# jiangzhongshi/SurfaceNetworks

Hardware: AMD Instinct MI355X
Metric: meshes/sec fwd+bwd, Dirac temporal-predict (higher is better)
Workload: dtype f32; 1 GPU; as_rigid_as_possible Dirac temporal prediction: 64 grid-cloth meshes 71x71 (V=5041,F=9800) per GPU, C=128, 15 layers, fwd+loss+bwd+allreduce+Adam; meshes_per_gpu=64, global_batch=64, parallelism=dp1 (mesh sharding, flat-bucket RCCL all-reduce), world_size=1, rccl_ranks=1, collective_backend=nccl, devices_visible=1, operator_format=q3, operators=pool, grad_bucket_bytes=4075488

## Files before the change

### include/sn_spmm.h

```cpp
#ifndef SN_SPMM_H_
#define SN_SPMM_H_

#include <stddef.h>
#include <stdint.h>

#ifdef __cplusplus
extern "C" {
#endif

#define SN_ABI_VERSION 1

#define SN_OK            0
#define SN_E_NULL       -1
#define SN_E_SHAPE      -2
#define SN_E_RANGE      -3
#define SN_E_LD         -4
#define SN_E_ALIGN      -5
#define SN_E_WORKSPACE  -6
#define SN_E_UNSUPPORTED -7

int         sn_abi_version(void);
const char *sn_status_string(int status);

int sn_spmm_csr_f32(const int32_t *rowptr, const int32_t *colind, const float *vals,
// ... 122 lines not shown
                                   void *stream);

int sn_validate_csr_i32(const int32_t *rowptr, const int32_t *colind, const float *vals, int64_t M, int64_t K, int64_t nnz,
                        int32_t *flags, void *stream);

int sn_elu_into_f32(const float *src, int64_t lds, float *dst, int64_t ldd,
                    int64_t rows, int32_t C, void *stream);
int sn_elu_bwd_acc_f32(const float *gdst, int64_t ldg, const float *gdst2, int64_t ldg2, const float *gadd, int64_t ldga,
                       const float *out, int64_t ldo, float *gsrc, int64_t ldgs, int64_t rows, int32_t C,
                       int32_t accumulate, void *stream);


size_t sn_colstats_workspace_bytes(int64_t rows, int32_t C);
int sn_colstats_f32(const float *x, int64_t ld, int64_t rows, int32_t C, double *out,
                    void *workspace, size_t workspace_bytes, void *stream);
int sn_colstats_into_f32(const float *x, int64_t ld, int64_t rows, int32_t C, double *out, int64_t out_ld, int64_t out_off,
                         void *workspace, size_t workspace_bytes, void *stream);
int sn_colstats_merge_f64(const double *part, int32_t nblk, int32_t C, double *out, int64_t out_ld, int64_t out_off,
                          void *stream);
int sn_colstats_merge2_f64(const double *part_lo, int32_t nblk_lo, int32_t C_lo, int32_t ld_lo, const double *part_hi,
                           int32_t nblk_hi, int32_t C_hi, int32_t ld_hi, double *out, void *stream);
int32_t sn_linear_fwd_stats_blocks(int64_t rows);
size_t sn_wgrad_workspace_bytes(int64_t rows, int32_t J, int32_t C);
int sn_wgrad_f32(const float *dy, int64_t lddy, const float *x, int64_t ldx, const float *center, int64_t rows,
                 int32_t J, int32_t C, float *G, double *dysum, void *workspace, size_t workspace_bytes, void *stream);
size_t sn_wgrad_seg_workspace_bytes(int64_t rows, int64_t rows_per_seg, int32_t J, int32_t C);
int sn_wgrad_seg_f32(const float *dy, int64_t lddy, const float *x, int64_t ldx, const float *center, int64_t rows,
                     int64_t rows_per_seg, int32_t J, int32_t C, float *G, double *dysum, float *seg_dysum, void *workspace,
                     size_t workspace_bytes, void *stream);
int sn_wgrad_slabs_f32(const float *dy, int64_t lddy, const float *x, int64_t ldx, const float *center, int64_t rows,
                       const int64_t *slab_off, int32_t nslab, const int64_t *seg_slab_ptr, int32_t nseg, int32_t J, int32_t C,
                       float *G, double *dysum, float *seg_dysum, void *workspace, size_t workspace_bytes, void *stream);
int sn_wgrad_bounded_f32(const float *dy, int64_t lddy, const float *x, int64_t ldx, const float *center, int64_t rows,
                         int32_t J, int32_t C, float *G, double *dysum, void *workspace, size_t workspace_bytes,
                         const float *dybound, int64_t n_dybound, const float *xinvstd, int64_t stat_rows, void *stream);
int sn_wgrad_seg_bounded_f32(const float *dy, int64_t lddy, const float *x, int64_t ldx, const float *center, int64_t rows,
                             int64_t rows_per_seg, int32_t J, int32_t C, float *G, double *dysum, float *seg_dysum,
                             void *workspace, size_t workspace_bytes, const float *dybound, int64_t n_dybound,
                             const float *xinvstd, int64_t stat_rows, void *stream);
int sn_wgrad_slabs_bounded_f32(const float *dy, int64_t lddy, const float *x, int64_t ldx, const float *center, int64_t rows,
                               const int64_t *slab_off, int32_t nslab, const int64_t *seg_slab_ptr, int32_t nseg, int32_t J,
                               int32_t C, float *G, double *dysum, float *seg_dysum, void *workspace, size_t workspace_bytes,
                               const float *dybound, int64_t n_dybound, const float *xinvstd, int64_t stat_rows, void *stream);
size_t sn_wgrad_thin_workspace_bytes(int64_t rows, int32_t J, int32_t C);
int sn_wgrad_thin_f32(const float *dy, int64_t lddy, const float *x, int64_t ldx, int64_t rows, int32_t J, int32_t C,
                      float *G, float *db, void *workspace, size_t workspace_bytes, void *stream);
size_t sn_masked_smooth_l1_workspace_bytes(int64_t rows, int32_t C);
int sn_masked_smooth_l1_fwd_f32(const float *out, int64_t ldo, const float *target, int64_t ldt, const float *rowmask,
                                int64_t rows, int32_t C, double scale, float *loss, void *workspace, size_t workspace_bytes,
                                void *stream);
int sn_masked_smooth_l1_bwd_f32(const float *out, int64_t ldo, const float *target, int64_t ldt, const float *rowmask,
                                int64_t rows, int32_t C, double scale, const float *gloss, float *gout, int64_t ldg,
                                void *stream);
int sn_gather_segments_f32(const float *src, const int64_t *base, int64_t nitems, int64_t rows_per_item, int64_t row_stride,
                           int32_t len, float *out, void *stream);
int sn_gather_segments_ragged_f32(const float *src, const int64_t *base, const int64_t *item_off, int64_t nitems,
                                  int64_t total_rows, int64_t row_stride, int32_t len, float *out, void *stream);
int sn_pair_argmin_f32(const float *GA, int64_t ldA, int64_t colsA, const int64_t *pa, const float *GB, int64_t ldB,
                       const int64_t *pb, int64_t NA, int64_t NB, int64_t *out, void *stream);
int sn_pair_ce_fwd_f32(const float *S, int64_t ld, const int64_t *target, int64_t NA, int64_t NB, float *lse, float *rowloss,
                       void *stream);
int sn_pair_ce_bwd_f32(const float *S, int64_t ld, const int64_t *target, const float *lse, const float *gloss, int64_t NA,
                       int64_t NB, int64_t rows, int64_t cols, float *dS, int64_t ldd, void *stream);
size_t sn_pair_fused_workspace_bytes(int64_t rowsA, int64_t rowsB);
int sn_pair_fused_fwd_f32(const float *FA, int64_t lda, const float *FB, int64_t ldb, const int64_t *target, int64_t NA,
                          int64_t NB, int64_t rowsA, int64_t rowsB, int32_t K, float *lse, float *rowloss, void *workspace,
                          size_t workspace_bytes, void *stream);
int sn_pair_fused_bwd_f32(const int64_t *target, const float *lse, const float *gloss, int64_t NA, int64_t NB, int64_t rowsA,
                          int64_t rowsB, int32_t K, float *dFA, int64_t ldda, float *dFB, int64_t lddb, void *workspace,
                          size_t workspace_bytes, void *stream);
size_t sn_pair_loss_workspace_bytes(int64_t rowsA, int64_t rowsB);
int sn_pair_soft_fwd_f32(const float *FA, int64_t lda, const float *FB, int64_t ldb, const int64_t *mapA, const int64_t *mapB,
                         const float *const *geo, int64_t ldgA, int64_t ldgB, int64_t NA, int64_t NB, int64_t rowsA, int64_t rowsB,
                         int32_t K, float *stats, float *rowloss, void *workspace, size_t workspace_bytes, void *stream);
int sn_pair_soft_bwd_f32(const int64_t *mapA, const int64_t *mapB, const float *const *geo, int64_t ldgA, int64_t ldgB,
                         const float *stats, const float *gloss, int64_t NA, int64_t NB, int64_t rowsA, int64_t rowsB, int32_t K,
                         float *dFA, int64_t ldda, float *dFB, int64_t lddb, void *workspace, size_t workspace_bytes, void *stream);
int sn_pair_sl1_fwd_f32(const float *FA, int64_t lda, const float *FB, int64_t ldb, const int64_t *mapA, const int64_t *mapB,
                        const float *const *geo, int64_t ldgA, int64_t ldgB, int64_t NA, int64_t NB, int64_t rowsA, int64_t rowsB,
                        int32_t K, double *rowloss, void *workspace, size_t workspace_bytes, void *stream);
int sn_pair_sl1_bwd_f32(const int64_t *mapA, const int64_t *mapB, const float *const *geo, int64_t ldgA, int64_t ldgB,
                        const float *gloss, int64_t NA, int64_t NB, int64_t rowsA, int64_t rowsB, int32_t K, float *dFA, int64_t ldda,
                        float *dFB, int64_t lddb, void *workspace, size_t workspace_bytes, void *stream);
size_t sn_pair_match_workspace_bytes(int64_t rowsA, int64_t rowsB);
int sn_pair_match_f32(const float *FA, int64_t lda, const float *FB, int64_t ldb, int64_t NA, int64_t NB, int64_t rowsA,
                      int64_t rowsB, int32_t K, int64_t *colA, float *bestA, int64_t *rowB, float *bestB, const float *geoB,
                      int64_t ldgB, const int64_t *truthA, float *errA, void *workspace, size_t workspace_bytes, void *stream);
int sn_linear_thin_fwd_f32(const float *x, int64_t ldx, const float *W, int64_t ldw, const float *bias, int64_t rows,
                           int32_t C, int32_t J, float *y, int64_t ldy, float *y_elu, int64_t lde, void *stream);
int sn_affine_cols_acc_f32(float *dx, int64_t lddx, const float *x, int64_t ldx, const float *center, const float *B,
                           const float *Cc, int64_t rows, int32_t C, void *stream);
int sn_affine_cols_elu_bwd_f32(float *dx, int64_t lddx, const float *x, int64_t ldx, const float *center, const float *B,
                               const float *Cc, int64_t rows, int32_t C, void *stream);

int sn_bn_fold_f32(const double *stats, int64_t rows, const float *gamma, const float *beta, const float *W,
                   const float *b, int32_t J, int32_t C, double eps, double momentum, int32_t training,
                   float *running_mean, float *running_var, float *mean, float *invstd, float *s, float *t,
                   float *Wf, float *bf, int64_t *num_batches_tracked, void *stream);
int32_t sn_wgrad_bounded_enabled(void);
int32_t sn_gemm_variant(void);
int32_t sn_colstats_blocks(int64_t rows);
int sn_colstats_partial_f32(const float *x, int64_t ld, int64_t rows, int32_t C, double *partial, void *stream);
int sn_bn_bwd_coeffs_f32(const float *Gc, const double *dystats, const float *W, const float *s, const float *invstd,
                         const float *beta, int64_t rows, int32_t J, int32_t C, float *dW, float *db, float *dgamma,
                         float *dbeta, float *Bc, float *Cc, void *stream);

// ... 135 lines not shown
int sn_mesh_cot_laplacian_f32(const float *V, const int32_t *F, int64_t nV, int64_t nF, int32_t phase, int32_t mass, int32_t clamp,
                              double hack, int32_t *rowptr, int32_t *colind, float *vals, int32_t *status, void *workspace,
                              size_t workspace_bytes, void *stream);

#define SN_SPGEMM_MAX_WINDOW   131072
#define SN_SPGEMM_BAD_COLUMN   1
#define SN_SPGEMM_TOO_WIDE     2
#define SN_SPGEMM_TOO_LARGE    4
#define SN_CSR_NO_OFFDIAGONAL  8
int64_t sn_csr_spgemm_max_window(void);
size_t sn_csr_spgemm_workspace_bytes(int64_t M);
int sn_csr_spgemm_f32(const int32_t *a_rowptr, const int32_t *a_colind, const float *a_vals, const int32_t *b_rowptr,
                      const int32_t *b_colind, const float *b_vals, int64_t M, int64_t K, int64_t N, int32_t phase,
                      int32_t *s_rowptr, int32_t *s_colind, float *s_vals, int32_t *rowptr, int32_t *colind, float *vals,
                      int32_t *status, void *workspace, size_t workspace_bytes, void *stream);
int sn_csr_inv_sqrt_degree_f32(const int32_t *rowptr, int64_t M, float *d, int32_t *status, void *stream);
int sn_csr_scale_sym_f32(const int32_t *a_rowptr, const int32_t *a_colind, const float *a_vals, const float *d, int64_t M,
                         int32_t phase, float *s_vals, int32_t *rowptr, int32_t *colind, float *vals, int32_t *status,
                         void *workspace, size_t workspace_bytes, void *stream);

int64_t sn_linear_small_rows(void);
int32_t sn_linear_fwd_form(int64_t rows, int32_t K, int32_t J, int32_t has_residual, int32_t has_y, int32_t has_elu,
                           int32_t has_tile_sums);
int sn_linear_fwd_f32(const float *x, int64_t ldx, const float *W, int64_t ldw, const float *bias,
                      const float *residual, int64_t ldr, float *y, int64_t ldy, float *y_elu, int64_t lde,
                      int64_t rows, int32_t K, int32_t J, double *elu_stats_part ,
                      void *stream);
int sn_linear_dgrad_f32(const float *dy, int64_t lddy, const float *W, int64_t ldw, const float *x, int64_t ldx,
                        const float *center, const float *B, const float *Cc, float *dx, int64_t lddx,
                        int64_t rows, int32_t J, int32_t C, void *stream);
int sn_linear_dgrad_elu_f32(const float *dy, int64_t lddy, const float *W, int64_t ldw, const float *x, int64_t ldx,
                            const float *center, const float *B, const float *Cc, float *dx_hi, int64_t lddx,
                            float *gact, int64_t ldga, const float *gadd, int64_t ldgadd,
                            int64_t rows, int32_t J, int32_t C, void *stream);
int32_t sn_linear_dgrad_absmax_blocks(void);
int sn_linear_dgrad_elu_absmax_f32(const float *dy, int64_t lddy, const float *W, int64_t ldw, const float *x, int64_t ldx,
                                   const float *center, const float *B, const float *Cc, float *dx_hi, int64_t lddx,
                                   float *gact, int64_t ldga, const float *gadd, int64_t ldgadd,
                                   int64_t rows, int32_t J, int32_t C, float *gact_absmax, void *stream);
int sn_linear_dgrad_elu_rawlow_f32(const float *dy, int64_t lddy, const float *W, int64_t ldw, const float *x, int64_t ldx,
                                   const float *center, const float *B, const float *Cc, float *dx_hi, int64_t lddx,
                                   float *graw, int64_t ldgr, int64_t rows, int32_t J, int32_t C, void *stream);
int sn_linear_fwd_segbias_f32(const float *x, int64_t ldx, const float *W, int64_t ldw, const float *segbias,
                              int64_t rows_per_seg, const float *residual, int64_t ldr, float *y, int64_t ldy,
                              float *y_elu, int64_t lde, int64_t rows, int32_t K, int32_t J, double *elu_stats_part,
                              void *stream);
int sn_linear_dgrad_eluseg_f32(const float *dy, int64_t lddy, const float *W, int64_t ldw, const float *x, int64_t ldx,
                               const float *center, const float *B, const float *Cc, const float *segvec,
                               int64_t rows_per_seg, const float *rowmask, float *gact, int64_t ldga, const float *gadd,
                               int64_t ldgadd, int64_t rows, int32_t J, int32_t C, void *stream);
int sn_linear_fwd_tiles_f32(const float *x, int64_t ldx, const float *W, int64_t ldw, const float *bias, const float *residual,
                            int64_t ldr, float *y, int64_t ldy, float *y_elu, int64_t lde, int64_t rows, int32_t K, int32_t J,
                            double *elu_stats_part, float *tile_sums, void *stream);
int sn_linear_fwd_segbias_tiles_f32(const float *x, int64_t ldx, const float *W, int64_t ldw, const float *segbias,
                                    int64_t rows_per_seg, const float *residual, int64_t ldr, float *y, int64_t ldy, float *y_elu,
                                    int64_t lde, int64_t rows, int32_t K, int32_t J, double *elu_stats_part, float *tile_sums,
                                    void *stream);
int sn_avg_stats_from_tiles_f32(const float *tile_sums, const double *stats_part, int32_t nblk, const float *e, int64_t ld,
                                const float *mask, const float *inv_count, int64_t rows_per_seg, int64_t nseg, int32_t C,
                                float *m, double *stats, float *workspace, void *stream);
int sn_avg_stats_from_tiles_ragged_f32(const float *tile_sums, const double *stats_part, int32_t nblk, const float *e, int64_t ld,
                                       const int64_t *segoff, const float *inv_count, int64_t nseg, int32_t C, float *m,
                                       double *stats, float *workspace, void *stream);
int sn_linear_fwd_segbias_ragged_tiles_f32(const float *x, int64_t ldx, const float *W, int64_t ldw, const float *segbias,
                                           const int64_t *segoff, int32_t nseg, const float *residual, int64_t ldr, float *y,
                                           int64_t ldy, float *y_elu, int64_t lde, int64_t rows, int32_t K, int32_t J,
                                           double *elu_stats_part, float *tile_sums, void *stream);
int sn_linear_fwd_segbias_ragged_f32(const float *x, int64_t ldx, const float *W, int64_t ldw, const float *segbias,
                                     const int64_t *segoff, int32_t nseg, const float *residual, int64_t ldr, float *y,
                                     int64_t ldy, float *y_elu, int64_t lde, int64_t rows, int32_t K, int32_t J,
                                     double *elu_stats_part, void *stream);
int sn_linear_dgrad_eluseg_ragged_f32(const float *dy, int64_t lddy, const float *W, int64_t ldw, const float *x, int64_t ldx,
                                      const float *center, const float *B, const float *Cc, const float *segvec,
                                      const int64_t *segoff, int32_t nseg, float *gact, int64_t ldga, const float *gadd,
                                      int64_t ldgadd, int64_t rows, int32_t J, int32_t C, void *stream);
int sn_linear_dgrad_eluseg_absmax_f32(const float *dy, int64_t lddy, const float *W, int64_t ldw, const float *x, int64_t ldx,
                                      const float *center, const float *B, const float *Cc, const float *segvec,
                                      int64_t rows_per_seg, const float *rowmask, float *gact, int64_t ldga, const float *gadd,
                                      int64_t ldgadd, int64_t rows, int32_t J, int32_t C, float *gact_absmax, void *stream);
int sn_linear_dgrad_eluseg_ragged_absmax_f32(const float *dy, int64_t lddy, const float *W, int64_t ldw, const float *x,
                                             int64_t ldx, const float *center, const float *B, const float *Cc,
                                             const float *segvec, const int64_t *segoff, int32_t nseg, float *gact, int64_t ldga,
                                             const float *gadd, int64_t ldgadd, int64_t rows, int32_t J, int32_t C,
                                             float *gact_absmax, void *stream);

typedef struct sn_plan sn_plan;
int sn_plan_create(sn_plan **out);
int sn_plan_destroy(sn_plan *plan);
int32_t sn_plan_lookup(const char *entry_point_name);
int32_t sn_plan_entry_count(void);
const char *sn_plan_entry_name(int32_t fn);
const char *sn_plan_entry_signature(int32_t fn);
int64_t sn_plan_length(const sn_plan *plan);
int sn_plan_add_call(sn_plan *plan, int32_t fn, int32_t nargs, const int32_t *kind, const int32_t *slot, const int64_t *ival,
                     const double *dval);
int sn_plan_add_memset(sn_plan *plan, int32_t slot, int64_t offset, int32_t byte_value, int64_t pitch, int64_t width_bytes,
                       int64_t rows);
int sn_plan_add_copy(sn_plan *plan, int32_t dst_slot, int64_t dst_offset, int64_t dst_pitch, int32_t src_slot, int64_t src_offset,
                     int64_t src_pitch, int64_t width_bytes, int64_t rows);
int sn_plan_run(const sn_plan *plan, const uint64_t *slot_base, int32_t nslots, void *stream, int32_t *failed_node);

typedef struct sn_plan_exec sn_plan_exec;
int sn_plan_instantiate(const sn_plan *plan, const uint64_t *slot_base, int32_t nslots, sn_plan_exec **out, int32_t *failed_node);
int sn_plan_exec_launch(const sn_plan_exec *exec, const sn_plan *plan, const uint64_t *slot_base, int32_t nslots, void *stream,
                        int32_t *failed_node);
int sn_plan_exec_destroy(sn_plan_exec *exec);
// ... 6 lines not shown
```

### surfacenetworks_amd/_lib.py

```python
from __future__ import annotations

import ctypes as C
import os
import threading

_HERE = os.path.dirname(os.path.abspath(__file__))
LIB_PATH = os.path.join(_HERE, "libsn_hip.so")

_vp, _i64, _i32, _sz = C.c_void_p, C.c_int64, C.c_int32, C.c_size_t

SIGNATURES = {
    "sn_abi_version": (C.c_int, []),
    "sn_status_string": (C.c_char_p, [C.c_int]),
    "sn_spmm_csr_f32": (C.c_int, [_vp, _vp, _vp, _i64, _i64, _i64, _vp, _i64, _i32, _i32, _vp, _i64, _i32, _vp]),
    "sn_spmm_csr_stats_workspace_bytes": (_sz, [_i64]),
    "sn_spmm_csr_stats_f32": (C.c_int, [_vp, _vp, _vp, _i64, _i64, _i64, _vp, _i64, _i32, _i32, _vp, _i64, _i32, _vp, _vp, _sz, _vp]),
    "sn_spmm_bsr4_f32": (C.c_int, [_vp, _vp, _vp, _i64, _i64, _i64, _vp, _i64, _i32, _i32, _vp, _i64, _i32, _vp]),
    "sn_spmm_csr_elubwd_f32": (C.c_int, [_vp, _vp, _vp, _i64, _i64, _i64, _vp, _i64, _i32, _i32, _vp, _i64, _vp, _i64, _vp, _i64,
                                         _i32, _vp]),
    "sn_spmm_bsr4_elubwd_f32": (C.c_int, [_vp, _vp, _vp, _i64, _i64, _i64, _vp, _i64, _i32, _i32, _vp, _i64, _vp, _i64, _vp, _i64,
                                          _i32, _vp]),
    "sn_spmm_q3_f32": (C.c_int, [_vp, _vp, _i64, _i64, _i64, _vp, _i64, _i32, _i32, _vp, _i64, _i32, _vp]),
    "sn_spmm_q3_stats_workspace_bytes": (_sz, [_i64]),
    "sn_spmm_q3_stats_blocks": (_i32, []),
# ... 16 lines not shown
    "sn_spmm_rb4_stats_f32": (C.c_int, [_vp, _vp, _vp, _i64, _i64, _i64, _vp, _i64, _i32, _vp, _i64, _vp, _vp, _sz, _vp]),
    "sn_spmm_csr_ring_f32": (C.c_int, [_vp, _vp, _vp, _i64, _i64, _i64, _vp, _i64, _i32, _vp, _i64, _vp]),
    "sn_spmm_csr_ring_elubwd_f32": (C.c_int, [_vp, _vp, _vp, _i64, _i64, _i64, _vp, _i64, _i32, _vp, _i64, _vp, _i64, _vp, _i64, _vp]),
    "sn_spmm_csr_ring_absmax_blocks": (_i64, [_i64, _i32]),
    "sn_spmm_csr_ring_elubwd_absmax_f32": (C.c_int, [_vp, _vp, _vp, _i64, _i64, _i64, _vp, _i64, _i32, _vp, _i64, _vp, _i64, _vp, _i64, _vp,
                                                     _vp]),
    "sn_spmm_csr_ring_stats_workspace_bytes": (_sz, [_i64]),
    "sn_spmm_csr_ring_stats_f32": (C.c_int, [_vp, _vp, _vp, _i64, _i64, _i64, _vp, _i64, _i32, _vp, _i64, _vp, _vp, _sz, _vp]),
    "sn_spmm_csr_ring_half_window": (_i32, []),
    "sn_csr_band_i32": (C.c_int, [_vp, _vp, _i64, _i64, _vp, _vp]),
    "sn_blockdiag_concat_i32": (C.c_int, [_vp, _vp, _vp, _vp, _i64, _i64, _i64, _i64, _i32, _vp, _vp, _vp, _vp]),
    "sn_blockdiag_concat_ragged_i32": (C.c_int, [_vp, _vp, _vp, _vp, _i64, _i64, _i64, _i64, _i32, _vp, _vp, _vp, _vp]),
    "sn_validate_csr_i32": (C.c_int, [_vp, _vp, _vp, _i64, _i64, _i64, _vp, _vp]),
    "sn_elu_into_f32": (C.c_int, [_vp, _i64, _vp, _i64, _i64, _i32, _vp]),
    "sn_elu_bwd_acc_f32": (C.c_int, [_vp, _i64, _vp, _i64, _vp, _i64, _vp, _i64, _vp, _i64, _i64, _i32, _i32, _vp]),
    "sn_colstats_workspace_bytes": (_sz, [_i64, _i32]),
    "sn_colstats_f32": (C.c_int, [_vp, _i64, _i64, _i32, _vp, _vp, _sz, _vp]),
    "sn_wgrad_workspace_bytes": (_sz, [_i64, _i32, _i32]),
    "sn_wgrad_f32": (C.c_int, [_vp, _i64, _vp, _i64, _vp, _i64, _i32, _i32, _vp, _vp, _vp, _sz, _vp]),
    "sn_wgrad_seg_workspace_bytes": (_sz, [_i64, _i64, _i32, _i32]),
    "sn_wgrad_seg_f32": (C.c_int, [_vp, _i64, _vp, _i64, _vp, _i64, _i64, _i32, _i32, _vp, _vp, _vp, _vp, _sz, _vp]),
    "sn_wgrad_slabs_f32": (C.c_int, [_vp, _i64, _vp, _i64, _vp, _i64, _vp, _i32, _vp, _i32, _i32, _i32, _vp, _vp, _vp, _vp, _sz, _vp]),
    "sn_wgrad_bounded_f32": (C.c_int, [_vp, _i64, _vp, _i64, _vp, _i64, _i32, _i32, _vp, _vp, _vp, _sz, _vp, _i64, _vp, _i64, _vp]),
    "sn_wgrad_seg_bounded_f32": (C.c_int, [_vp, _i64, _vp, _i64, _vp, _i64, _i64, _i32, _i32, _vp, _vp, _vp, _vp, _sz, _vp, _i64, _vp,
                                           _i64, _vp]),
    "sn_wgrad_slabs_bounded_f32": (C.c_int, [_vp, _i64, _vp, _i64, _vp, _i64, _vp, _i32, _vp, _i32, _i32, _i32, _vp, _vp, _vp, _vp, _sz,
                                             _vp, _i64, _vp, _i64, _vp]),
    "sn_avg_prep_ragged_f32": (C.c_int, [_vp, _vp, _i64, _i32, _vp, _i32, _vp, _vp]),
    "sn_bn_fold_seg_f32": (C.c_int, [_vp, _i64, _vp, _vp, _vp, _vp, _i32, _i32, C.c_double, C.c_double, _vp, _vp, _vp, _vp, _vp, _vp, _vp,
                                     _vp, _vp, _vp, _i64, _vp, _vp]),
    "sn_avg_bn_bwd_f32": (C.c_int, [_vp, _vp, _vp, _vp, _vp, _vp, _vp, _vp, _vp, _i64, _i32, _i32, _i64, _vp, _i64, _vp, _i64, _vp, _vp,
                                    _vp, _vp, _vp, _vp, _vp, _vp, _vp]),
    "sn_linear_dgrad_absmax_blocks": (_i32, []),
    "sn_linear_dgrad_elu_absmax_f32": (C.c_int, [_vp, _i64, _vp, _i64, _vp, _i64, _vp, _vp, _vp, _vp, _i64, _vp, _i64, _vp, _i64, _i64,
                                                 _i32, _i32, _vp, _vp]),
    "sn_linear_dgrad_eluseg_absmax_f32": (C.c_int, [_vp, _i64, _vp, _i64, _vp, _i64, _vp, _vp, _vp, _vp, _i64, _vp, _vp, _i64, _vp,
                                                    _i64, _i64, _i32, _i32, _vp, _vp]),
    "sn_linear_dgrad_eluseg_ragged_absmax_f32": (C.c_int, [_vp, _i64, _vp, _i64, _vp, _i64, _vp, _vp, _vp, _vp, _vp, _i32, _vp, _i64,
                                                           _vp, _i64, _i64, _i32, _i32, _vp, _vp]),
    "sn_spmm_q3_absmax_blocks": (_i64, [_i64, _i32]),
    "sn_spmm_q3_elubwd_absmax_f32": (C.c_int, [_vp, _vp, _i64, _i64, _i64, _vp, _i64, _i32, _i32, _vp, _i64, _vp, _i64, _vp, _i64, _i32,
                                               _vp, _vp]),
    "sn_spmm_q3_tail_supported": (_i32, [_i32, _i32]),
    "sn_spmm_q3_elubwd_tail_absmax_f32": (C.c_int, [_vp, _vp, _i64, _i64, _i64, _vp, _i64, _i32, _i32, _vp, _i64, _vp, _i64, _vp, _vp, _vp,
                                                    _vp, _i64, _i32, _vp, _vp]),
    "sn_elu_tail_finish_f32": (C.c_int, [_vp, _i64, _vp, _i64, _vp, _vp, _vp, _i64, _i32, _vp]),
    "sn_linear_dgrad_elu_rawlow_f32": (C.c_int, [_vp, _i64, _vp, _i64, _vp, _i64, _vp, _vp, _vp, _vp, _i64, _vp, _i64, _i64, _i32, _i32,
                                                 _vp]),
    "sn_wgrad_thin_workspace_bytes": (_sz, [_i64, _i32, _i32]),
    "sn_wgrad_thin_f32": (C.c_int, [_vp, _i64, _vp, _i64, _i64, _i32, _i32, _vp, _vp, _vp, _sz, _vp]),
    "sn_masked_smooth_l1_workspace_bytes": (_sz, [_i64, _i32]),
    "sn_masked_smooth_l1_fwd_f32": (C.c_int, [_vp, _i64, _vp, _i64, _vp, _i64, _i32, C.c_double, _vp, _vp, _sz, _vp]),
    "sn_masked_smooth_l1_bwd_f32": (C.c_int, [_vp, _i64, _vp, _i64, _vp, _i64, _i32, C.c_double, _vp, _vp, _i64, _vp]),
    "sn_pair_argmin_f32": (C.c_int, [_vp, _i64, _i64, _vp, _vp, _i64, _vp, _i64, _i64, _vp, _vp]),
    "sn_pair_ce_fwd_f32": (C.c_int, [_vp, _i64, _vp, _i64, _i64, _vp, _vp, _vp]),
    "sn_pair_ce_bwd_f32": (C.c_int, [_vp, _i64, _vp, _vp, _vp, _i64, _i64, _i64, _i64, _vp, _i64, _vp]),
    "sn_pair_fused_workspace_bytes": (C.c_size_t, [_i64, _i64]),
    "sn_pair_fused_fwd_f32": (C.c_int, [_vp, _i64, _vp, _i64, _vp, _i64, _i64, _i64, _i64, C.c_int32, _vp, _vp, _vp, C.c_size_t, _vp]),
    "sn_pair_fused_bwd_f32": (C.c_int, [_vp, _vp, _vp, _i64, _i64, _i64, _i64, C.c_int32, _vp, _i64, _vp, _i64, _vp, C.c_size_t, _vp]),
    "sn_pair_loss_workspace_bytes": (C.c_size_t, [_i64, _i64]),
    "sn_pair_soft_fwd_f32": (C.c_int, [_vp, _i64, _vp, _i64, _vp, _vp, _vp, _i64, _i64, _i64, _i64, _i64, _i64, C.c_int32, _vp, _vp, _vp, C.c_size_t, _vp]),
    "sn_pair_soft_bwd_f32": (C.c_int, [_vp, _vp, _vp, _i64, _i64, _vp, _vp, _i64, _i64, _i64, _i64, C.c_int32, _vp, _i64, _vp, _i64, _vp, C.c_size_t, _vp]),
    "sn_pair_sl1_fwd_f32": (C.c_int, [_vp, _i64, _vp, _i64, _vp, _vp, _vp, _i64, _i64, _i64, _i64, _i64, _i64, C.c_int32, _vp, _vp, C.c_size_t, _vp]),
    "sn_pair_sl1_bwd_f32": (C.c_int, [_vp, _vp, _vp, _i64, _i64, _vp, _i64, _i64, _i64, _i64, C.c_int32, _vp, _i64, _vp, _i64, _vp, C.c_size_t, _vp]),
    "sn_pair_match_workspace_bytes": (C.c_size_t, [_i64, _i64]),
    "sn_pair_match_f32": (C.c_int, [_vp, _i64, _vp, _i64, _i64, _i64, _i64, _i64, C.c_int32, _vp, _vp, _vp, _vp, _vp, _i64, _vp, _vp, _vp,
                                    C.c_size_t, _vp]),
    "sn_gather_segments_f32": (C.c_int, [_vp, _vp, _i64, _i64, _i64, _i32, _vp, _vp]),
    "sn_gather_segments_ragged_f32": (C.c_int, [_vp, _vp, _vp, _i64, _i64, _i64, _i32, _vp, _vp]),
    "sn_linear_thin_fwd_f32": (C.c_int, [_vp, _i64, _vp, _i64, _vp, _i64, _i32, _i32, _vp, _i64, _vp, _i64, _vp]),
    "sn_bn_fold_f32": (C.c_int, [_vp, _i64, _vp, _vp, _vp, _vp, _i32, _i32, C.c_double, C.c_double, _i32, _vp, _vp, _vp,
                                 _vp, _vp, _vp, _vp, _vp, _vp, _vp]),
    "sn_colstats_blocks": (C.c_int32, [_i64]),
    "sn_wgrad_bounded_enabled": (C.c_int32, []),
    "sn_gemm_variant": (C.c_int32, []),
    "sn_colstats_merge2_f64": (C.c_int, [_vp, C.c_int32, C.c_int32, C.c_int32, _vp, C.c_int32, C.c_int32, C.c_int32, _vp, _vp]),
    "sn_colstats_partial_f32": (C.c_int, [_vp, _i64, _i64, C.c_int32, _vp, _vp]),
    "sn_bn_bwd_coeffs_f32": (C.c_int, [_vp, _vp, _vp, _vp, _vp, _vp, _i64, _i32, _i32, _vp, _vp, _vp, _vp, _vp, _vp, _vp]),
    "sn_segment_colsum_ragged_workspace_bytes": (_sz, [_i64, _i32]),
    "sn_segment_colsum_ragged_f32": (C.c_int, [_vp, _i64, _vp, _i64, _vp, _i64, _i32, _vp, _vp, _vp, _sz, _vp]),
    "sn_bcast_rows_ragged_f32": (C.c_int, [_vp, _vp, _i64, _vp, _i64, _i32, _vp]),
    "sn_segment_colsum_workspace_bytes": (_sz, [_i64, _i64, _i32]),
    "sn_segment_colsum_f32": (C.c_int, [_vp, _i64, _vp, _i64, _i64, _i32, _vp, _vp, _sz, _vp]),
    "sn_bcast_rows_f32": (C.c_int, [_vp, _vp, _i64, _i64, _i64, _i32, _vp]),
    "sn_elu_bwd_bcast_f32": (C.c_int, [_vp, _i64, _vp, _i64, _vp, _vp, _vp, _i64, _vp, _i64, _i64, _i64, _i32, _vp]),
    "sn_dirac_workspace_bytes": (_sz, [_i64, _i64]),
    "sn_dirac_bsr4_from_mesh": (C.c_int, [_vp, _vp, _i64, _i64, _vp, _vp, _vp, _vp, _vp, _vp, _vp, _vp, _vp, _sz, _vp]),
    "sn_timing_enable": (C.c_int, [_i32]),
    "sn_timing_count": (_i64, []),
    "sn_timing_drain": (C.c_int, [_vp, _vp, _i64, _vp]),
    "sn_laplacian_workspace_bytes": (_sz, [_i64, _i64]),
    "sn_laplacian_csr_from_mesh": (C.c_int, [_vp, _vp, _i64, _i64, _i32, _vp, _vp, _vp, _vp, _vp, _sz, _vp]),
    "sn_edge_lengths_csr_f32": (C.c_int, [_vp, _vp, _vp, _i64, _vp, _vp]),
    "sn_graph_apsp_max_vertices": (_i64, []),
    "sn_graph_apsp_group": (_i32, [_i64]),
    "sn_graph_apsp_threads": (_i32, [_i64]),
    "sn_graph_apsp_f32": (C.c_int, [_vp, _vp, _vp, _i64, _i64, _i64, _vp, _i64, _vp, _vp]),
    "sn_graph_apsp_sweeps_f32": (C.c_int, [_vp, _vp, _vp, _i64, _i64, _i64, _vp, _i64, _vp, _vp, _vp]),
    "sn_symmetrize_min_f32": (C.c_int, [_vp, _i64, _i64, _vp]),
    "sn_mesh_corners_workspace_bytes": (_sz, [_i64]),
    "sn_mesh_corners_f32": (C.c_int, [_vp, _vp, _i64, _i64, _vp, _vp, _vp, _vp, _sz, _vp]),
    "sn_mesh_geodesics_f32": (C.c_int, [_vp, _vp, _i64, _i64, _i64, _vp, _i64, _vp, _vp]),
    "sn_mesh_geodesics_sweeps_f32": (C.c_int, [_vp, _vp, _i64, _i64, _i64, _vp, _i64, _vp, _vp, _vp]),
    "sn_mesh_glue_workspace_bytes": (_sz, [_i64, _i64]),
    "sn_mesh_glue_i32": (C.c_int, [_vp, _vp, _i64, _i64, _vp, _vp, _vp, _vp, _sz, _vp]),
    "sn_mesh_idt_workspace_bytes": (_sz, [_i64]),
    "sn_mesh_idt_rounds_f64": (C.c_int, [_vp, _vp, _vp, _i64, _i32, _i32, _i32, _vp, _vp, _vp, _sz, _vp]),
    "sn_mesh_idt_laplacian_items": (_i64, [_i64, _i64]),
    "sn_mesh_idt_laplacian_workspace_bytes": (_sz, [_i64, _i64]),
    "sn_mesh_idt_laplacian_f32": (C.c_int, [_vp, _vp, _i64, _i64, _i32, _vp, _vp, _vp, _vp, _vp, _vp, _vp, _sz, _vp]),
    "sn_mesh_components_workspace_bytes": (_sz, [_i64, _i64, _i32]),
    "sn_mesh_components_i32": (C.c_int, [_vp, _i64, _i64, _i32, _vp, _vp, _vp, _vp, _vp, _vp, _sz, _vp]),
    "sn_mesh_label_mask_i32": (C.c_int, [_vp, _i64, _vp, _vp, _vp]),
    "sn_mesh_compact_workspace_bytes": (_sz, [_i64, _i64]),
    "sn_mesh_compact_i32": (C.c_int, [_vp, _vp, _vp, _i64, _i64, _vp, _vp, _vp, _vp, _vp, _vp, _vp, _sz, _vp]),
    "sn_mesh_weld_workspace_bytes": (_sz, [_i64]),
    "sn_mesh_weld_f32": (C.c_int, [_vp, _vp, _i64, _i64, C.c_double, _i32, _vp, _vp, _vp, _vp, _vp, _sz, _vp]),
    "sn_mesh_unique_faces_workspace_bytes": (_sz, [_i64]),
    "sn_mesh_unique_faces_i32": (C.c_int, [_vp, _vp, _i64, _i64, _i32, _vp, _vp, _vp, _vp, _sz, _vp]),
    "sn_mesh_orient_workspace_bytes": (_sz, [_i64, _i64]),
    "sn_mesh_orient_i32": (C.c_int, [_vp, _vp, _i64, _i64, _vp, _vp, _vp, _vp, _vp, _vp, _sz, _vp]),
    "sn_mesh_descriptors_workspace_bytes": (_sz, [_i64, _i64]),
    "sn_mesh_descriptors_f32": (C.c_int, [_vp, _vp, _i64, _i64, _vp, _vp, _vp, _vp, _vp, _vp, _vp, _vp, _vp, _vp, _vp, _sz, _vp]),
    "sn_mesh_cot_laplacian_workspace_bytes": (_sz, [_i64, _i64]),
    "sn_mesh_cot_laplacian_f32": (C.c_int, [_vp, _vp, _i64, _i64, _i32, _i32, _i32, C.c_double, _vp, _vp, _vp, _vp, _vp, _sz, _vp]),
    "sn_csr_spgemm_max_window": (_i64, []),
    "sn_csr_spgemm_workspace_bytes": (_sz, [_i64]),
    "sn_csr_spgemm_f32": (C.c_int, [_vp, _vp, _vp, _vp, _vp, _vp, _i64, _i64, _i64, _i32, _vp, _vp, _vp, _vp, _vp, _vp, _vp, _vp, _sz, _vp]),
    "sn_csr_inv_sqrt_degree_f32": (C.c_int, [_vp, _i64, _vp, _vp, _vp]),
    "sn_csr_scale_sym_f32": (C.c_int, [_vp, _vp, _vp, _vp, _i64, _i32, _vp, _vp, _vp, _vp, _vp, _vp, _sz, _vp]),
    "sn_linear_fwd_f32": (C.c_int, [_vp, _i64, _vp, _i64, _vp, _vp, _i64, _vp, _i64, _vp, _i64, _i64, _i32, _i32, _vp, _vp]),
    "sn_linear_fwd_stats_blocks": (_i32, [_i64]),
    "sn_linear_small_rows": (_i64, []),
    "sn_linear_fwd_form": (_i32, [_i64, _i32, _i32, _i32, _i32, _i32, _i32]),
    "sn_linear_fwd_tiles_f32": (C.c_int, [_vp, _i64, _vp, _i64, _vp, _vp, _i64, _vp, _i64, _vp, _i64, _i64, _i32, _i32, _vp, _vp, _vp]),
    "sn_linear_fwd_segbias_tiles_f32": (C.c_int, [_vp, _i64, _vp, _i64, _vp, _i64, _vp, _i64, _vp, _i64, _vp, _i64, _i64, _i32, _i32,
                                                  _vp, _vp, _vp]),
    "sn_avg_stats_from_tiles_ragged_f32": (C.c_int, [_vp, _vp, _i32, _vp, _i64, _vp, _vp, _i64, _i32, _vp, _vp, _vp, _vp]),
    "sn_linear_fwd_segbias_ragged_tiles_f32": (C.c_int, [_vp, _i64, _vp, _i64, _vp, _vp, _i32, _vp, _i64, _vp, _i64, _vp, _i64, _i64, _i32,
                                                         _i32, _vp, _vp, _vp]),
    "sn_avg_stats_from_tiles_f32": (C.c_int, [_vp, _vp, _i32, _vp, _i64, _vp, _vp, _i64, _i64, _i32, _vp, _vp, _vp, _vp]),
    "sn_colstats_into_f32": (C.c_int, [_vp, _i64, _i64, _i32, _vp, _i64, _i64, _vp, _sz, _vp]),
    "sn_colstats_merge_f64": (C.c_int, [_vp, _i32, _i32, _vp, _i64, _i64, _vp]),
    "sn_linear_dgrad_f32": (C.c_int, [_vp, _i64, _vp, _i64, _vp, _i64, _vp, _vp, _vp, _vp, _i64, _i64, _i32, _i32, _vp]),
    "sn_linear_dgrad_elu_f32": (C.c_int, [_vp, _i64, _vp, _i64, _vp, _i64, _vp, _vp, _vp, _vp, _i64, _vp, _i64, _vp, _i64, _i64,
                                          _i32, _i32, _vp]),
    "sn_linear_fwd_segbias_f32": (C.c_int, [_vp, _i64, _vp, _i64, _vp, _i64, _vp, _i64, _vp, _i64, _vp, _i64, _i64, _i32, _i32, _vp,
                                            _vp]),
    "sn_linear_dgrad_eluseg_f32": (C.c_int, [_vp, _i64, _vp, _i64, _vp, _i64, _vp, _vp, _vp, _vp, _i64, _vp, _vp, _i64, _vp, _i64,
                                             _i64, _i32, _i32, _vp]),
    "sn_avg_fwd_prep_f32": (C.c_int, [_vp, _vp, _i64, _i32, _i64, _vp, _vp, _vp, _vp]),
    "sn_avg_stats_workspace_bytes": (_sz, [_i64, _i64, _i32]),
    "sn_avg_stats_f32": (C.c_int, [_vp, _i64, _vp, _vp, _i64, _i64, _i32, _vp, _vp, _vp, _sz, _vp]),
    "sn_seg_affine_f32": (C.c_int, [_vp, _i64, _i32, _vp, _i64, _vp, _i32, _vp, _vp]),
    "sn_avg_bwd_gc_f32": (C.c_int, [_vp, _vp, _vp, _vp, _i64, _i32, _i32, _vp, _vp]),
    "sn_avg_bwd_segvec_f32": (C.c_int, [_vp, _vp, _i64, _vp, _vp, _vp, _vp, _vp, _i64, _i64, _i32, _i32, _vp, _vp]),
    "sn_avg_bwd_segvec_ragged_f32": (C.c_int, [_vp, _vp, _i64, _vp, _vp, _vp, _vp, _vp, _vp, _i64, _i32, _i32, _vp, _vp]),
    "sn_linear_fwd_segbias_ragged_f32": (C.c_int, [_vp, _i64, _vp, _i64, _vp, _vp, _i32, _vp, _i64, _vp, _i64, _vp, _i64, _i64, _i32,
                                                   _i32, _vp, _vp]),
    "sn_linear_dgrad_eluseg_ragged_f32": (C.c_int, [_vp, _i64, _vp, _i64, _vp, _i64, _vp, _vp, _vp, _vp, _vp, _i32, _vp, _i64, _vp,
                                                    _i64, _i64, _i32, _i32, _vp]),
    "sn_affine_cols_acc_f32": (C.c_int, [_vp, _i64, _vp, _i64, _vp, _vp, _vp, _i64, _i32, _vp]),
    "sn_affine_cols_elu_bwd_f32": (C.c_int, [_vp, _i64, _vp, _i64, _vp, _vp, _vp, _i64, _i32, _vp]),
    "sn_plan_create": (C.c_int, [C.POINTER(_vp)]),
    "sn_plan_destroy": (C.c_int, [_vp]),
    "sn_plan_lookup": (_i32, [C.c_char_p]),
    "sn_plan_entry_count": (_i32, []),
    "sn_plan_entry_name": (C.c_char_p, [_i32]),
    "sn_plan_entry_signature": (C.c_char_p, [_i32]),
    "sn_plan_length": (_i64, [_vp]),
    "sn_plan_add_call": (C.c_int, [_vp, _i32, _i32, _vp, _vp, _vp, _vp]),
    "sn_plan_add_memset": (C.c_int, [_vp, _i32, _i64, _i32, _i64, _i64, _i64]),
    "sn_plan_add_copy": (C.c_int, [_vp, _i32, _i64, _i64, _i32, _i64, _i64, _i64, _i64]),
    "sn_plan_run": (C.c_int, [_vp, _vp, _i32, _vp, _vp]),
    "sn_plan_instantiate": (C.c_int, [_vp, _vp, _i32, _vp, _vp]),
    "sn_plan_exec_launch": (C.c_int, [_vp, _vp, _vp, _i32, _vp, _vp]),
    "sn_plan_exec_destroy": (C.c_int, [_vp]),
}

_lib = None


class SnError(RuntimeError):
    """A C-ABI call returned non-zero (negative: SN_E_* argument error, positive: hipError_t)."""


def load() -> C.CDLL:
    global _lib
# ... 44 lines not shown
```

### surfacenetworks_amd/arap.py

```python
from __future__ import annotations

from dataclasses import dataclass
from typing import List, Optional

import numpy as np
import torch
import torch.nn as nn
import torch.nn.functional as F

from . import kernels, mesh_ops
from . import utils_pt as utils
from .operators import OperatorPool, PackedSegments, h2d_async

INPUT_FRAMES = 2
OUTPUT_FRAMES = 40


def _num_faces(Di, DiA, batch_size):
    return DiA.size(2) // 4 if len(Di.size()) == 3 else DiA.size(1) // 4 // batch_size



def _add_last_frame(x, inputs, frames):
    B, V, _ = x.shape
    return (x.reshape(B, V, frames, 3) + inputs[:, :, None, -3:]).reshape(B, V, 3 * frames)


class Model(nn.Module):

    def __init__(self, layer=15, dense=False):
        super().__init__()
        self.conv1 = utils.GraphConv1x1(6, 128, batch_norm=None)
        self.layer = layer
        for i in range(layer):
            if i % 2 == 0:
                blk = utils.DenseLapResNet2(128) if dense else utils.LapResNet2(128)
            else:
                blk = utils.AvgResNet2(128)
            self.add_module("rn{}".format(i), blk)
        self.conv2 = utils.GraphConv1x1(128, 120, batch_norm="pre")

    def forward(self, L, mask, inputs):
        x = self.conv1(inputs)
        for i in range(self.layer):
            blk = self._modules["rn{}".format(i)]
            if i % 2 == 0 and isinstance(blk, utils.LapResNet2):
                x = blk(L, mask, x, avg_next=i + 1 < self.layer)
            else:
                x = blk(L, mask, x)
        x = utils.elu_conv1x1(self.conv2, x)
        return _add_last_frame(x, inputs, OUTPUT_FRAMES)


class AvgModel(nn.Module):

    def __init__(self):
        super().__init__()
        self.conv1 = utils.GraphConv1x1(6, 128, batch_norm=None)
        for i in range(15):
            self.add_module("rn{}".format(i), utils.AvgResNet2(128))
        self.conv2 = utils.GraphConv1x1(128, 120, batch_norm="pre")

    def forward(self, L, mask, inputs):
        x = self.conv1(inputs)
        for i in range(15):
            x = self._modules["rn{}".format(i)](L, mask, x)
        x = utils.elu_conv1x1(self.conv2, x)
        return _add_last_frame(x, inputs, OUTPUT_FRAMES)


class MlpModel(nn.Module):

    def __init__(self):
        super().__init__()
        self.conv1 = utils.GraphConv1x1(6, 128, batch_norm=None)
        for i in range(15):
            self.add_module("rn{}".format(i), utils.MlpResNet2(128))
        self.bn = utils.GraphBatchNorm(128)
        self.conv2 = utils.GraphConv1x1(128, 120, batch_norm=None)

    def forward(self, L, mask, inputs):
        x = self.conv1(inputs)
        for i in range(15):
            x = self._modules["rn{}".format(i)](L, mask, x)
        x = self.conv2(F.elu(self.bn(x)))
        return _add_last_frame(x, inputs, OUTPUT_FRAMES)


class DirModel(nn.Module):

    def __init__(self):
        super().__init__()
        self.conv1 = utils.GraphConv1x1(6, 128, batch_norm=None)
        for i in range(15):
            self.add_module("rn{}".format(i), utils.DirResNet2(128) if i % 2 == 0 else utils.AvgResNet2(128))
        self.do = nn.Dropout2d()
        self.conv2 = utils.GraphConv1x1(128, 120, batch_norm="pre")

    def forward(self, Di, DiA, mask, inputs):
        batch_size = inputs.size(0)
        v = self.conv1(inputs)
        f = None
        nf = _num_faces(Di, DiA, batch_size)
        for i in range(15):
            blk = self._modules["rn{}".format(i)]
            if i % 2 == 0:
                v, f = blk(Di, DiA, v, f, f_out_needed=False, num_faces=nf,
                           avg_next=i + 1 < 15)
            else:
                v = blk(None, mask, v)
        x = utils.elu_conv1x1(self.conv2, v)
        return _add_last_frame(x, inputs, OUTPUT_FRAMES)


class _MaskedSmoothL1(torch.autograd.Function):

    @staticmethod
    def forward(ctx, out2d, tgt2d, rowmask, scale):
        ctx.save_for_backward(out2d, tgt2d, rowmask)
        ctx.scale = scale
        return kernels.masked_smooth_l1_fwd(out2d, tgt2d, rowmask, scale)

    @staticmethod
    def backward(ctx, gloss):
        out2d, tgt2d, rowmask = ctx.saved_tensors
        return kernels.masked_smooth_l1_bwd(out2d, tgt2d, rowmask, ctx.scale, gloss.contiguous()), None, None, None


def loss_fn(outputs, targets, mask, batch_size):
    if isinstance(mask, PackedSegments):
        mask = torch.ones(outputs.shape[0] * outputs.shape[1], dtype=torch.float32, device=outputs.device)
    if outputs.dim() == 3 and outputs.dtype == torch.float32 and targets.dtype == torch.float32 and \
            not targets.requires_grad and mask.numel() == outputs.shape[0] * outputs.shape[1]:
        C = outputs.shape[2]
        out = _MaskedSmoothL1.apply(outputs.reshape(-1, C), targets.reshape(-1, C).contiguous(),
                                    mask.reshape(-1).to(torch.float32).contiguous(), 1.0 / batch_size)
        return out
    outputs = outputs * mask.expand_as(outputs)
    return F.smooth_l1_loss(outputs, targets, reduction="sum") / batch_size


def make_adam(model):
    params = list(model.parameters())
    fused = len(params) > 0 and all(p.is_cuda and p.dtype == torch.float32 for p in params)
    return torch.optim.Adam(params, 1e-3, weight_decay=1e-5, fused=fused)


def make_optimizer(model):
    return make_adam(model)


def halve_lr(optimizer, epoch: int, after: int = 50, every: int = 10) -> bool:
    if not (epoch > after and epoch % every == 0):
        return False
    for group in optimizer.param_groups:
        group["lr"] *= 0.5
    return True


@dataclass
class Batch:
    inputs: torch.Tensor
    targets: torch.Tensor
    mask: torch.Tensor
    L: Optional[object]
    Di: Optional[object]
    DiA: Optional[object]
    num_meshes: int


class ClothSequences:

    def __init__(self, grids, frames=50, op_frames=2, seed=3, device="cuda", model="dir", permute=False,
                 operators="pool", reorder="auto"):
        rng = np.random.default_rng(seed)
        self.device = torch.device(device)
        self.frames, self.op_frames, self.kind = frames, op_frames, model
        self.operators = operators
        if operators not in ("pool", "device"):
            raise ValueError(operators)
        if operators == "device" and (model != "dir" or len(set(grids)) != 1):
            raise ValueError("on-device operator construction supports the Dirac model on equally sized meshes")
        assert frames >= INPUT_FRAMES + OUTPUT_FRAMES + 1 and 1 <= op_frames
        Vs, Fs, mats = [], [], {"L": [], "Di": [], "DiA": []}
        coords, faces_all, orders = [], [], []
        for (n, m) in grids:
            V0, F_ = mesh_ops.grid_cloth(n, m, rng, permute=permute)
            order = mesh_ops.MeshOrder.of_mesh(F_, V0.shape[0], reorder)
            V0, F_ = order.mesh(V0, F_)
# ... 165 lines not shown
```

### surfacenetworks_amd/blocks.py

```python
from __future__ import annotations

import weakref

import torch

from . import kernels, plans
from .functional import (SpmmTimer, _launch, _rows2d, product_form, avg_stage_backward, avg_stage_backward_ragged, avg_stage_forward,
                         avg_stage_forward_ragged, bn_prepare, bnlin_backward,
                         bnlin_backward_elu_input, bnlin_backward_zero_first, bnlin_forward, bnlin_forward_zero_first, stash, unstash,
                         zero_first_supported)
from .graphs import active_capture
from .operators import as_operator

__all__ = ["lap_block", "dirac_block", "avg_block", "avg_block_ragged", "avg_block_ragged_ok", "take_activated", "attach_activated", "zero_faces_ok", "elu_conv", "elu_conv_ok"]


DEFER_FACE_TAIL = True


def _version_of(t: torch.Tensor):
    return None if t.is_inference() else t._version


def attach_activated(t: torch.Tensor, cat: torch.Tensor) -> torch.Tensor:
    t._sn_cat = (cat, _version_of(t))
    return t


def take_activated(t: torch.Tensor, rows: int, C: int):
    d = getattr(t, "__dict__", None)
    entry = d.pop("_sn_cat", None) if d is not None else None
    if entry is None:
        return None
    cat, version = entry
    if version != _version_of(t) or tuple(cat.shape) != (rows, 2 * C) or cat.device != t.device or cat.dtype != torch.float32:
        return None
    return cat


def _new_cat(rows, C, device):
    return torch.empty((rows, 2 * C), dtype=torch.float32, device=device)


def _new_part(rows, C, device, narrow=False):
    if not (C == 128 or (narrow and C == 64 and kernels.linear_fwd_supported(2 * C, C))) or not kernels.elu_stats_supported():
        return None
    return kernels.new_elu_stats_part(rows, device)


def _attach_part(cat, part, tiles=None):
    if part is not None:
        cat._sn_part = part
        if tiles is not None:
            cat._sn_tiles = tiles


_TILE_SUMS_MIN_ROWS = 32768


def _new_tiles(rows, C, device, part, wanted):
    if not wanted or part is None or C != 128 or rows < _TILE_SUMS_MIN_ROWS or not kernels.tile_sums_supported():
        return None
    return kernels.new_tile_sums(rows, device)


def _wants_tiles(mod, avg_next) -> bool:
    if avg_next is None:
# ... 125 lines not shown
        g0 = 2 + len(kept)
        plan = plans.record(site, (id(fplan), key), impl, (saved, *[o for o, _ in ops], *grads, *consts), ext,
                            grads_device(grads, big, small), range(g0, g0 + len(grads)))
        fplan.bwd[key] = plan
        if plan is None:
            plans.renote(grads, maxima, tails)
            return impl(saved, *[o for o, _ in ops], *grads, *consts)
        for g in grads:
            if g is not None:
                kernels.take_absmax(g)
                kernels.take_tail(g)
    timer = SpmmTimer.active
    if timer is not None:
        if plan.tags is None:
            fext = [None] * fplan.n_ext
            for j, t in zip(fplan.saved_ext, kept):
                fext[j] = t
            plans.renote(grads, maxima, tails)
            return impl(plans._Builder(big, small, fext)(fplan.result[1]), *[o for o, _ in ops], *grads, *consts)
        timer.tags.extend(plan.tags)
    b2, s2 = plan.new_arenas(grads_device(grads, big, small))
    plan.run(b2, s2, ext)
    site.replayed += 1
    build = plans._Builder(b2, s2, ext)
    out = build(plan.result)
    if plan.effects or plan.tail_effects:
        plans.apply_effects(plan, build)
    return out


def grads_device(grads, *others):
    for t in (*grads, *others):
        if t is not None:
            return t.device
    raise ValueError("no tensor to take the device from")


_SITES = {name: plans.Site(name) for name in ("dirac_fwd", "dirac_bwd", "propagate_fwd", "propagate_bwd", "avg_fwd", "avg_bwd",
                                              "avg_ragged_fwd", "avg_ragged_bwd", "elu_conv_fwd", "elu_conv_bwd")}


_NAN = {}


def _nan_placeholder(device):
    t = _NAN.get(device)
    if t is None:
        t = torch.full((1, 1), float("nan"), dtype=torch.float32, device=device)
        if device.type != "cuda" or not torch.cuda.is_current_stream_capturing():
            _NAN[device] = t
    return t


def _dirac_fwd(v, f, pre_v, pre_f, g0, b0, W0, c0, rm0, rv0, g1, b1, W1, c1, rm1, rv1, opDi, opDiA, need_f, avg_next, tr0, mo0,
               ep0, tr1, mo1, ep1):
    rv, C = v.shape
    rf = opDi.shape[0] // 4
    cat1 = _activated(v, pre_v)
    nxt_f = _new_cat(rf, C, v.device)
    pf = _new_part(rf, C, v.device, narrow=True)
    if f is None:
        cat0 = torch.empty((rf, C), dtype=torch.float32, device=v.device)
        _attach_hi(cat0, _launch(opDi, cat1[:, :C], cat0, 4, "fwd", stats=tr0))
        f_out, st0 = bnlin_forward_zero_first(cat0, g0, b0, W0, c0, rm0, rv0, tr0, mo0, ep0, nxt_f[:, :C], need_f, pf)
    else:
        cat0 = pre_f if pre_f is not None else _activated(f, None)
        _attach_hi(cat0, _launch(opDi, cat1[:, :C], cat0[:, C:], 4, "fwd", stats=tr0))
        f_out, st0 = bnlin_forward(cat0, g0, b0, W0, c0, rm0, rv0, tr0, mo0, ep0, None, nxt_f[:, :C], want_y=need_f,
                                   elu_stats=pf)
    _attach_part(nxt_f, pf)
    _attach_hi(cat1, _launch(opDiA, nxt_f[:, :C], cat1[:, C:], 4, "fwd", stats=tr1))
    nxt_v = _new_cat(rv, C, v.device)
    pv = _new_part(rv, C, v.device, narrow=True)
    tv = _new_tiles(rv, C, v.device, pv, avg_next)
    v_new, st1 = bnlin_forward(cat1, g1, b1, W1, c1, rm1, rv1, tr1, mo1, ep1, v, nxt_v[:, :C], elu_stats=pv, tile_sums=tv)
    _attach_part(nxt_v, pv, tv)
    return (v_new, f_out, nxt_v, nxt_f), ((cat0, cat1, nxt_f), st0, st1)


def _dirac_bwd(saved, opDi, opDiA, g_vnew, g_fo, f_zero, need_gv, need_gf, defer=False, expect_raw=False):
    (cat0, cat1, nxt_f), st0, st1 = saved
    C = cat1.shape[1] // 2
    dev = cat1.device
    tail = kernels.take_tail(g_fo) if g_fo is not None else None
    if expect_raw and g_fo is not None and tail is None:
        raise RuntimeError("dirac_block: a raw face gradient without its tail")
    gp1 = (None,) * 4
    h1 = None
    if g_vnew is not None:
        (dx1_hi, h1), dg1, db1, dW1, dc1 = bnlin_backward(st1, g_vnew, through_elu=(g_vnew,))
        gp1 = (dg1, db1, dW1, dc1)
        g_sum = torch.empty((nxt_f.shape[0], C), dtype=torch.float32, device=dev)
        _launch(opDiA.t(), dx1_hi, g_sum, 4, "bwd", elubwd=(nxt_f[:, :C], g_fo) if tail is None else (nxt_f[:, :C], g_fo, tail))
        g_fo = g_sum
    elif tail is not None:
        kernels.elu_tail_finish(g_fo, nxt_f[:, :C], tail)
    gp0 = (None,) * 4
    g_v = g_f = None
    dx0_hi = None
    if g_fo is not None and f_zero:
        dx0_hi, dg0, db0, dW0, dc0 = bnlin_backward_zero_first(st0, g_fo)
        gp0 = (dg0, db0, dW0, dc0)
    elif g_fo is not None and defer and need_gf:
        (dx0_hi, g_f), dg0, db0, dW0, dc0, tail_f = bnlin_backward(st0, g_fo, through_elu=(None,), raw_low=True)
        kernels.note_tail(g_f, tail_f)
        gp0 = (dg0, db0, dW0, dc0)
    elif g_fo is not None:
        (dx0_hi, g_f), dg0, db0, dW0, dc0 = bnlin_backward(st0, g_fo, through_elu=(None,))
        gp0 = (dg0, db0, dW0, dc0)
    if need_gv:
        if dx0_hi is not None:
            g_v = torch.empty((cat1.shape[0], C), dtype=torch.float32, device=dev)
            _launch(opDi.t(), dx0_hi, g_v, 4, "bwd", elubwd=(cat1[:, :C], h1))
        else:
            g_v = h1
    if f_zero or not need_gf:
        g_f = None
    return (g_v, g_f) + gp0 + gp1


class _DiracBlock(torch.autograd.Function):

    @staticmethod
    def forward(ctx, v, f, opDi, opDiA, pre_v, pre_f, need_f, avg_next, g0, b0, W0, c0, rm0, rv0, tr0, mo0, ep0, g1, b1, W1, c1,
                rm1, rv1, tr1, mo1, ep1):
        v = _rows2d(v)
        if f is not None and pre_f is None:
            f = _rows2d(f)
        ctx.f_zero = f is None
        ctx.ops = (opDi, opDiA)
        box = pre_f.__dict__.get("_sn_rawbox") if pre_f is not None else None
        ctx.defer = bool(DEFER_FACE_TAIL and box is not None and tr0 and v.is_cuda and
                         kernels.linear_dgrad_elu_supported(W0.shape[0], W0.shape[1]) and W0.shape[1] == 2 * v.shape[1])
        if ctx.defer:
            box[0] = True
        ctx.rawbox = [False] if not need_f else None
        tensors = (v, f, pre_v, pre_f, g0, b0, W0, c0, rm0, rv0, g1, b1, W1, c1, rm1, rv1)
        consts = (need_f, avg_next, tr0, mo0, ep0, tr1, mo1, ep1)
        outs = None
        ctx._sn_plan = None
        if plans.usable(v):
            outs = _plan_forward(ctx, _SITES["dirac_fwd"], _dirac_fwd, tensors, ((opDi, 4), (opDiA, 4)), consts, v.shape[1], 4, (2, 3, 8, 14))
            if outs is not None:
                _drop_counters(rm0, rm1)
        ctx._sn_planned = outs is not None
        if outs is None:
            outs, saved = _dirac_fwd(*tensors, opDi, opDiA, *consts)
            stash(ctx, *saved)
        v_new, f_out, nxt_v, nxt_f = outs
        if f_out is None:
            f_out = _nan_placeholder(v.device).expand(nxt_f.shape[0], v.shape[1])
            if ctx.rawbox is not None:
                nxt_f._sn_rawbox = ctx.rawbox
        ctx.mark_non_differentiable(nxt_v, nxt_f)
        ctx.set_materialize_grads(False)
        return v_new, f_out, nxt_v, nxt_f

    @staticmethod
    def backward(ctx, g_vnew, g_fout, _gv, _gf):
        if g_vnew is None and g_fout is None:
            return (None,) * 26
        opDi, opDiA = ctx.ops
        g_vnew = g_vnew.contiguous() if g_vnew is not None else None
        g_fout = g_fout.contiguous() if g_fout is not None else None
        consts = (ctx.f_zero, bool(ctx.needs_input_grad[0]), bool(ctx.needs_input_grad[1]), ctx.defer,
                  bool(ctx.rawbox is not None and ctx.rawbox[0]))
        if consts[4] and g_fout is not None and not kernels.has_tail(g_fout):
            raise RuntimeError("dirac_block: the gradient of the face output was left raw by the next Dirac block (DEFER_FACE_TAIL), but "
                               "what finishes it is gone — the gradient was copied, edited in place, or kernels.clear_absmax() ran "
                               "between the two backward calls")
        if ctx._sn_planned:
            r = _plan_backward(ctx, _SITES["dirac_bwd"], _dirac_bwd, (g_vnew, g_fout), consts)
        else:
            r = _dirac_bwd(unstash(ctx), opDi, opDiA, g_vnew, g_fout, *consts)
        none5 = (None,) * 5
        return (r[0], r[1], None, None, None, None, None, None) + r[2:6] + none5 + r[6:10] + none5


def _drop_counters(*running_means) -> None:
    for rm in running_means:
        d = getattr(rm, "__dict__", None)
        if d is not None:
            d.pop("_sn_nbt", None)


def dirac_block(mod, Di, DiA, v, f, need_f=True, num_faces=None, avg_next=None):
    B, V, C = v.shape
    F_ = f.shape[1] if f is not None else int(num_faces)
    rv, rf = B * V, B * F_
    opDi, opDiA = as_operator(Di), as_operator(DiA)
    if opDi.shape != (4 * rf, 4 * rv) or opDiA.shape != (4 * rv, 4 * rf):
        raise ValueError(f"DirResNet2: Di {tuple(opDi.shape)} / DiA {tuple(opDiA.shape)} do not match v rows {rv}, f rows {rf}")
    v_new, f_out, nxt_v, nxt_f = _DiracBlock.apply(v.reshape(rv, C), f.reshape(rf, C) if f is not None else None, opDi, opDiA,
                                                  take_activated(v, rv, C),
                                                  take_activated(f, rf, C) if f is not None else None, bool(need_f),
                                                  _wants_tiles(mod, avg_next), *_bn_args(mod._modules["bn_fc0"]), *_bn_args(mod._modules["bn_fc1"]))
    _mark_producer(nxt_v, mod, avg_next)
    return attach_activated(v_new.view(B, V, C), nxt_v), attach_activated(f_out.view(B, F_, C), nxt_f)


def zero_faces_ok(mod, C: int) -> bool:
    return zero_first_supported(C, mod.bn_fc0.fc.weight.shape[0]) and mod.bn_fc0.fc.weight.shape[1] == 2 * C


def _propagate_fwd(x, pre, mask_rows, inv_count, g0, b0, W0, c0, rm0, rv0, g1, b1, W1, c1, rm1, rv1, op, nseg, avg_next, tr0, mo0,
                   ep0, tr1, mo1, ep1):
    rows, C = x.shape
    per = rows // nseg if nseg else 0

    def propagate(cat, training):
        if op is not None:
            _attach_hi(cat, _launch(op, cat[:, :C], cat[:, C:], 1, "fwd", stats=training))
        else:
            mean = kernels.segment_colsum(cat[:, :C], mask_rows, per, nseg) * inv_count
            kernels.bcast_rows(mean, cat[:, C:], per)

    cat_a = _activated(x, pre)
    propagate(cat_a, tr0)
    cat_b = _new_cat(rows, C, x.device)
    pb = _new_part(rows, C, x.device)
    _, st0 = bnlin_forward(cat_a, g0, b0, W0, c0, rm0, rv0, tr0, mo0, ep0, None, cat_b[:, :C],
                           want_y=False, elu_stats=pb)
    _attach_part(cat_b, pb)
    propagate(cat_b, tr1)
    nxt = _new_cat(rows, C, x.device)
    pn = _new_part(rows, C, x.device)
    tn = _new_tiles(rows, C, x.device, pn, avg_next)
    out, st1 = bnlin_forward(cat_b, g1, b1, W1, c1, rm1, rv1, tr1, mo1, ep1, x, nxt[:, :C], elu_stats=pn, tile_sums=tn)
    _attach_part(nxt, pn, tn)
    return (out, nxt), ((cat_a, cat_b), st0, st1, (mask_rows, inv_count))


def _propagate_bwd(saved, op, g_out, nseg, need_gx):
    (cat_a, cat_b), st0, st1, (mask_rows, inv_count) = saved
    C = cat_a.shape[1] // 2
    per = cat_a.shape[0] // nseg if nseg else 0

    def stage_backward(st, g_in, cat, gadd):
        if op is not None:
            (d_hi, h), dg, db, dW, dc = bnlin_backward(st, g_in, through_elu=(gadd,))
            g = torch.empty((cat.shape[0], C), dtype=torch.float32, device=cat.device)
            _launch(op.t(), d_hi, g, 1, "bwd", elubwd=(cat[:, :C], h))
        else:
            dcat, dg, db, dW, dc = bnlin_backward(st, g_in)
            g = torch.empty((cat.shape[0], C), dtype=torch.float32, device=cat.device)
            gm = (kernels.segment_colsum(dcat[:, C:], None, per, nseg) * inv_count).contiguous()
            kernels.elu_bwd_bcast(dcat[:, :C], cat[:, :C], gm, mask_rows, g, per, gadd)
        return g, dg, db, dW, dc
# ... 165 lines not shown
        if g_out is None:
            return (None,) * 21
        g_out = g_out.contiguous()
        seg = ctx.seg
        seg_t, seg_key = _seg_tensors(seg)
        need = bool(ctx.needs_input_grad[0])
        if ctx._sn_planned:
            r = _plan_backward(ctx, _SITES["avg_ragged_bwd"], _avg_ragged_bwd_u, (g_out, *seg_t), (_Opaque(seg), seg_key, need))
        else:
            r = _avg_ragged_bwd(unstash(ctx), g_out, *seg_t, seg, seg_key, need)
        none5 = (None,) * 5
        return (r[0], None, None) + r[1:5] + none5 + r[5:9] + none5


class _Opaque:
    __slots__ = ("v",)

    def __init__(self, v):
        self.v = v

    def __hash__(self):
        return 0

    def __eq__(self, other):
        return isinstance(other, _Opaque)


def _avg_ragged_fwd_u(*a):
    return _avg_ragged_fwd(*a[:21], a[21].v, *a[22:])


def _avg_ragged_bwd_u(saved, g_out, *a):
    return _avg_ragged_bwd(saved, g_out, *a[:7], a[7].v, *a[8:])


def avg_block_ragged_ok(mod, seg, inputs) -> bool:
    C = inputs.shape[-1]
    a0, a1 = _bn_args(mod._modules["bn_fc0"]), _bn_args(mod._modules["bn_fc1"])
    return bool(a0[6] and a1[6]) and inputs.dtype == torch.float32 and mod.bn_fc0.fc.weight.shape == (C, 2 * C) and \
        mod.bn_fc1.fc.weight.shape == (C, 2 * C) and kernels.avg_stage_ragged_supported(C, C, seg) and \
        seg.rows == inputs.shape[0] * inputs.shape[1]


def avg_block_ragged(mod, seg, inputs):
    B, V, C = inputs.shape
    rows = B * V
    pre = take_activated(inputs, rows, C)
    _learn_avg_next(pre, rows)
    out, nxt = _AvgBlockRagged.apply(inputs.reshape(rows, C), seg, pre, *_bn_args(mod.bn_fc0),
                                     *_bn_args(mod.bn_fc1))
    return attach_activated(out.view(B, V, C), nxt)


def _elu_conv_fwd(v, pre, g0, b0, W0, c0, rm0, rv0, tr0, mo0, ep0):
    C = v.shape[1]
    cat = _activated(v, pre)
    part = getattr(cat, "_sn_part", None)
    pre_stats = kernels.colstats_from_part(part, v.shape[0]) if (part is not None and tr0 and C == 128) else None
    y, st = bnlin_forward(cat[:, :C], g0, b0, W0, c0, rm0, rv0, tr0, mo0, ep0, pre_stats=pre_stats)
    return (y,), (st,)


def _elu_conv_bwd(saved, dy, need_gv):
    (st,) = saved
    g_v, dg, db, dW, dc = bnlin_backward_elu_input(st, dy)
    return (g_v if need_gv else None, dg, db, dW, dc)


class _EluConv(torch.autograd.Function):

    @staticmethod
    def forward(ctx, v, pre, g0, b0, W0, c0, rm0, rv0, tr0, mo0, ep0):
        v = _rows2d(v)
        tensors = (v, pre, g0, b0, W0, c0, rm0, rv0)
        consts = (tr0, mo0, ep0)
        ctx._sn_plan = None
        outs = None
        if plans.usable(v):
            outs = _plan_forward(ctx, _SITES["elu_conv_fwd"], _elu_conv_fwd, tensors, (), consts, v.shape[1], 2, (1, 6))
            if outs is not None:
                _drop_counters(rm0)
        ctx._sn_planned = outs is not None
        if outs is None:
            outs, saved = _elu_conv_fwd(*tensors, *consts)
            stash(ctx, *saved)
        return outs[0]

    @staticmethod
    def backward(ctx, dy):
        dy = dy.contiguous()
        need = bool(ctx.needs_input_grad[0])
        if ctx._sn_planned:
            r = _plan_backward(ctx, _SITES["elu_conv_bwd"], _elu_conv_bwd, (dy,), (need,))
        else:
            r = _elu_conv_bwd(unstash(ctx), dy, need)
        return (r[0], None) + r[1:5] + (None,) * 5


def elu_conv(conv, v):
    B, N, C = v.shape
    rows = B * N
    y = _EluConv.apply(v.reshape(rows, C), take_activated(v, rows, C), *_bn_args(conv))
    return y.view(B, N, conv.num_outputs)


def elu_conv_ok(conv, v) -> bool:
    c = v.shape[-1]
    return getattr(conv, "batch_norm", None) == "pre" and v.dtype == torch.float32 and c % 4 == 0 and 256 % (c // 4) == 0 and \
        conv.bn.affine and conv.bn.momentum is not None and conv.bn.track_running_stats


def lap_block(mod, L, inputs, avg_next=None):
    B, V, C = inputs.shape
    rows = B * V
    op = as_operator(L)
    if op.shape != (rows, rows):
        raise ValueError(f"LapResNet2: operator {tuple(op.shape)} vs {rows} rows")
    out, nxt = _PropagateBlock.apply(inputs.reshape(rows, C), op, None, None, 0, take_activated(inputs, rows, C),
                                     _wants_tiles(mod, avg_next), *_bn_args(mod._modules["bn_fc0"]), *_bn_args(mod._modules["bn_fc1"]))
    _mark_producer(nxt, mod, avg_next)
    return attach_activated(out.view(B, V, C), nxt)


def avg_block(mod, mask, inputs):
    B, V, C = inputs.shape
    rows = B * V
    capturing = mask.is_cuda and torch.cuda.is_current_stream_capturing()
    gen = active_capture() if capturing else None
    slot = "_sn_avg" if not capturing else ("_sn_avg_cap" if gen is not None else None)
    cached = getattr(mask, slot, None) if slot else None
    key = (B, V, _version_of(mask), gen)
    if cached is None or cached[0] != key:
        cached = (key, mask.reshape(rows).contiguous(), 1.0 / mask.reshape(B, V).sum(1, keepdim=True))
        if slot:
            try:
                setattr(mask, slot, cached)
            except AttributeError:
                pass
    _, mask_rows, inv_count = cached
    a0, a1 = _bn_args(mod._modules["bn_fc0"]), _bn_args(mod._modules["bn_fc1"])
    if a0[6] and a1[6] and kernels.avg_stage_supported(C, a0[2].shape[0], V) and a0[2].shape[1] == 2 * C and a1[2].shape[0] == C:
        pre = take_activated(inputs, rows, C)
        _learn_avg_next(pre, rows)
        out, nxt = _AvgBlock.apply(inputs.reshape(rows, C), mask_rows, inv_count, B, pre, *a0, *a1)
    else:
        out, nxt = _PropagateBlock.apply(inputs.reshape(rows, C), None, mask_rows, inv_count, B, take_activated(inputs, rows, C),
                                         False, *a0, *a1)
    return attach_activated(out.view(B, V, C), nxt)
```

### surfacenetworks_amd/csrc/sn_dense.hip

```cpp

#include <hip/hip_runtime.h>
#include <hip/hip_ext.h>
#include <limits.h>
#include <stdint.h>
#include <stdlib.h>

#include "sn_dense_common.h"

namespace {

#define kCUs sn_internal_cu_count()

__device__ __forceinline__ f4 ld4_s(const float *p, int nt) {
  return nt ? __builtin_nontemporal_load(reinterpret_cast<const f4 *>(p)) : *reinterpret_cast<const f4 *>(p);
}
__device__ __forceinline__ void st4_s(float *p, f4 v, int nt) {
  if (nt) __builtin_nontemporal_store(v, reinterpret_cast<f4 *>(p));
  else *reinterpret_cast<f4 *>(p) = v;
}
__device__ __forceinline__ f4 ld4_stat(const float *p) { return ld4_s(p, 0); }

constexpr int kStreamNT = 1;

constexpr int kStatBlocks = 512;

template <bool VEC>
__global__ __launch_bounds__(kWG) void colstats_k(const float *__restrict__ x, int64_t ld, int64_t rows, int C,
                                                  double *__restrict__ partial ) {
  extern __shared__ double sm[];
  const int cw = VEC ? C / 4 : C;
  const int lanes_r = kWG / cw;
  const int cg = threadIdx.x % cw, rl = threadIdx.x / cw;
  const int64_t per = (rows + gridDim.x - 1) / gridDim.x;
  const int64_t r0 = (int64_t)blockIdx.x * per;
  const int64_t r1 = r0 + per < rows ? r0 + per : rows;
  if constexpr (VEC) {
    double s0 = 0, s1 = 0, s2 = 0, s3 = 0, q0 = 0, q1 = 0, q2 = 0, q3 = 0;
    if (rl < lanes_r) {
      const float *p = x + cg * 4;
      int64_t r = r0 + rl;
      for (; r + 3 * lanes_r < r1; r += 4 * lanes_r) {
        const f4 a = ld4_stat(p + r * ld);
        const f4 b = ld4_stat(p + (r + lanes_r) * ld);
        const f4 c = ld4_stat(p + (r + 2 * lanes_r) * ld);
        const f4 d = ld4_stat(p + (r + 3 * lanes_r) * ld);
#define SN_ACC(v)                                                                    \
  s0 += (double)v.x; s1 += (double)v.y; s2 += (double)v.z; s3 += (double)v.w;        \
  q0 += (double)v.x * v.x; q1 += (double)v.y * v.y; q2 += (double)v.z * v.z; q3 += (double)v.w * v.w;
        SN_ACC(a) SN_ACC(b) SN_ACC(c) SN_ACC(d)
      }
      for (; r < r1; r += lanes_r) {
        const f4 a = ld4_stat(p + r * ld);
        SN_ACC(a)
#undef SN_ACC
      }
      double *o = sm + (int64_t)rl * 2 * C;
      o[cg * 4] = s0; o[cg * 4 + 1] = s1; o[cg * 4 + 2] = s2; o[cg * 4 + 3] = s3;
      o[C + cg * 4] = q0; o[C + cg * 4 + 1] = q1; o[C + cg * 4 + 2] = q2; o[C + cg * 4 + 3] = q3;
// ... 525 lines not shown
constexpr int kLossBlocks = 1024;

__device__ __forceinline__ double sl1(float d) {
  const float a = fabsf(d);
  return a < 1.f ? 0.5 * (double)d * (double)d : (double)a - 0.5;
}

template <bool VEC>
__global__ __launch_bounds__(kWG) void masked_sl1_fwd_k(const float *__restrict__ o, int64_t ldo,
                                                        const float *__restrict__ t, int64_t ldt,
                                                        const float *__restrict__ mask, int64_t rows, int C,
                                                        double *__restrict__ partial) {
  __shared__ double red[kWG];
  constexpr int W = VEC ? 4 : 1;
  const int cw = C / W;
  const int64_t total = rows * cw;
  double acc = 0;
  for (int64_t i = (int64_t)blockIdx.x * kWG + threadIdx.x; i < total; i += (int64_t)gridDim.x * kWG) {
    const int64_t r = i / cw;
    const int c = (int)(i - r * cw) * W;
    const float m = mask ? mask[r] : 1.f;
    if constexpr (VEC) {
      const f4 ov = ld4_s(o + r * ldo + c, 1), tv = ld4_s(t + r * ldt + c, 1);
      acc += sl1(ov.x * m - tv.x) + sl1(ov.y * m - tv.y) + sl1(ov.z * m - tv.z) + sl1(ov.w * m - tv.w);
    } else {
      acc += sl1(o[r * ldo + c] * m - t[r * ldt + c]);
    }
  }
  red[threadIdx.x] = acc;
  __syncthreads();
  for (int s = kWG / 2; s > 0; s >>= 1) {
    if (threadIdx.x < s) red[threadIdx.x] += red[threadIdx.x + s];
    __syncthreads();
  }
  if (threadIdx.x == 0) partial[blockIdx.x] = red[0];
}

__global__ __launch_bounds__(kWG) void masked_sl1_final_k(const double *__restrict__ partial, int nblk, double scale,
                                                          float *__restrict__ loss) {
  __shared__ double red[kWG];
  double acc = 0;
  for (int i = threadIdx.x; i < nblk; i += kWG) acc += partial[i];
  red[threadIdx.x] = acc;
  __syncthreads();
  for (int s = kWG / 2; s > 0; s >>= 1) {
    if (threadIdx.x < s) red[threadIdx.x] += red[threadIdx.x + s];
    __syncthreads();
  }
  if (threadIdx.x == 0) loss[0] = (float)(red[0] * scale);
}

__device__ __forceinline__ float sl1_grad(float d) { return d < -1.f ? -1.f : (d > 1.f ? 1.f : d); }

template <bool VEC>
__global__ __launch_bounds__(kWG) void masked_sl1_bwd_k(const float *__restrict__ o, int64_t ldo,
                                                        const float *__restrict__ t, int64_t ldt,
                                                        const float *__restrict__ mask, int64_t rows, int C, float scale,
                                                        const float *__restrict__ gloss, float *__restrict__ g,
                                                        int64_t ldg) {
  constexpr int W = VEC ? 4 : 1;
  const int cw = C / W;
  const int64_t total = rows * cw;
  const float gs = gloss[0] * scale;
  for (int64_t i = (int64_t)blockIdx.x * kWG + threadIdx.x; i < total; i += (int64_t)gridDim.x * kWG) {
    const int64_t r = i / cw;
    const int c = (int)(i - r * cw) * W;
    const float m = mask ? mask[r] : 1.f;
    const float gm = gs * m;
    if constexpr (VEC) {
      const f4 ov = ld4_s(o + r * ldo + c, 1), tv = ld4_s(t + r * ldt + c, 1);
      st4_s(g + r * ldg + c, f4{gm * sl1_grad(ov.x * m - tv.x), gm * sl1_grad(ov.y * m - tv.y),
                                gm * sl1_grad(ov.z * m - tv.z), gm * sl1_grad(ov.w * m - tv.w)}, 1);
    } else {
      g[r * ldg + c] = gm * sl1_grad(o[r * ldo + c] * m - t[r * ldt + c]);
    }
  }
}

template <int W>
__global__ __launch_bounds__(kWG) void gather_segments_k(const float *__restrict__ src, const int64_t *__restrict__ base,
                                                         int64_t rows_per_item, int64_t row_stride, int len,
                                                         int64_t total, float *__restrict__ out) {
  const int lw = len / W;
  const int64_t per_item = rows_per_item * lw;
  for (int64_t i = (int64_t)blockIdx.x * kWG + threadIdx.x; i < total; i += (int64_t)gridDim.x * kWG) {
    const int64_t item = i / per_item, w = i - item * per_item;
    const int64_t r = w / lw;
    const int c = (int)(w - r * lw) * W;
    const float *p = src + base[item] + r * row_stride + c;
    if constexpr (W == 4) {
      __builtin_nontemporal_store(f4{p[0], p[1], p[2], p[3]}, reinterpret_cast<f4 *>(out) + i);
    } else {
      __builtin_nontemporal_store(p[0], out + i);
    }
  }
}

template <int W>
__global__ __launch_bounds__(kWG) void gather_segments_ragged_k(const float *__restrict__ src, const int64_t *__restrict__ base,
                                                                const int64_t *__restrict__ item_off, int nitems,
                                                                int64_t row_stride, int len, int64_t total,
                                                                float *__restrict__ out) {
  const int lw = len / W;
  for (int64_t i = (int64_t)blockIdx.x * kWG + threadIdx.x; i < total; i += (int64_t)gridDim.x * kWG) {
    const int64_t row = i / lw;
    const int c = (int)(i - row * lw) * W;
    int lo = 0, hi = nitems - 1;
    while (lo < hi) {
      const int mid = (lo + hi + 1) >> 1;
      if (item_off[mid] <= row) lo = mid;
      else hi = mid - 1;
    }
    const float *p = src + base[lo] + (row - item_off[lo]) * row_stride + c;
    if constexpr (W == 4) {
      __builtin_nontemporal_store(f4{p[0], p[1], p[2], p[3]}, reinterpret_cast<f4 *>(out) + i);
    } else {
      __builtin_nontemporal_store(p[0], out + i);
    }
  }
}

template <int C>
__global__ __launch_bounds__(kWG) void linear_thin_fwd_k(const float *__restrict__ x, int64_t ldx,
                                                         const float *__restrict__ W, int64_t ldw,
                                                         const float *__restrict__ b, int64_t rows, int J,
                                                         float *__restrict__ y, int64_t ldy, float *__restrict__ ye,
                                                         int64_t lde) {
  const int cw = J / 4, lanes_r = kWG / cw;
  const int cg = threadIdx.x % cw, rl = threadIdx.x / cw;
// ... 1705 lines not shown
  return launch_status();
}

int sn_elu_bwd_bcast_f32(const float *gdst, int64_t ldg, const float *out, int64_t ldo, const float *bias,
                         const float *mask, const float *gadd, int64_t ldga, float *gsrc, int64_t ldgs,
                         int64_t rows_per_seg, int64_t nseg, int32_t C, void *stream) {
  (void)hipGetLastError();
  if (rows_per_seg < 0 || nseg < 0 || C < 1 || ldg < C || ldo < C || ldgs < C || (gadd && ldga < C)) return SN_E_SHAPE;
  if ((C % 4) || (ldg % 4) || (ldo % 4) || (ldgs % 4) || (gadd && (ldga % 4))) return SN_E_UNSUPPORTED;
  const int64_t rows = rows_per_seg * nseg;
  if (rows == 0) return SN_OK;
  if (!gdst || !out || !bias || !gsrc) return SN_E_NULL;
  if (!aligned16(gdst) || !aligned16(out) || !aligned16(bias) || !aligned16(gsrc) || (gadd && !aligned16(gadd))) return SN_E_ALIGN;
  hipLaunchKernelGGL(elu_bwd_bcast_k, dim3(ew_grid(rows * (C / 4))), dim3(kWG), 0, static_cast<hipStream_t>(stream), gdst,
                     ldg, out, ldo, bias, mask, gadd, ldga, gsrc, ldgs, rows_per_seg, rows, (int)C, kStreamNT);
  return launch_status();
}

static int loss_blocks(int64_t items) {
  int64_t b = (items + kWG - 1) / kWG;
  if (b > kLossBlocks) b = kLossBlocks;
  return b < 1 ? 1 : (int)b;
}

size_t sn_masked_smooth_l1_workspace_bytes(int64_t rows, int32_t C) {
  (void)rows; (void)C;
  return (size_t)kLossBlocks * sizeof(double);
}

int sn_masked_smooth_l1_fwd_f32(const float *out, int64_t ldo, const float *target, int64_t ldt, const float *rowmask,
                                int64_t rows, int32_t C, double scale, float *loss, void *workspace, size_t workspace_bytes,
                                void *stream) {
  (void)hipGetLastError();
  if (rows < 0 || C < 1 || ldo < C || ldt < C) return SN_E_SHAPE;
  if (!loss) return SN_E_NULL;
  hipStream_t s = static_cast<hipStream_t>(stream);
  if (rows == 0) {
    const hipError_t e = sn_internal_fill(loss, 0, sizeof(float), s);
    return e == hipSuccess ? SN_OK : (int)e;
  }
  if (!out || !target || !workspace) return SN_E_NULL;
  if (workspace_bytes < (size_t)kLossBlocks * sizeof(double)) return SN_E_WORKSPACE;
  const bool vec = (C % 4 == 0) && (ldo % 4 == 0) && (ldt % 4 == 0) && aligned16(out) && aligned16(target);
  const int nblk = loss_blocks(rows * (vec ? C / 4 : C));
  double *partial = static_cast<double *>(workspace);
  if (vec)
    hipLaunchKernelGGL((masked_sl1_fwd_k<true>), dim3(nblk), dim3(kWG), 0, s, out, ldo, target, ldt, rowmask, rows, (int)C, partial);
  else
    hipLaunchKernelGGL((masked_sl1_fwd_k<false>), dim3(nblk), dim3(kWG), 0, s, out, ldo, target, ldt, rowmask, rows, (int)C, partial);
  hipLaunchKernelGGL(masked_sl1_final_k, dim3(1), dim3(kWG), 0, s, partial, nblk, scale, loss);
  return launch_status();
}

int sn_masked_smooth_l1_bwd_f32(const float *out, int64_t ldo, const float *target, int64_t ldt, const float *rowmask,
                                int64_t rows, int32_t C, double scale, const float *gloss, float *gout, int64_t ldg,
                                void *stream) {
  (void)hipGetLastError();
  if (rows < 0 || C < 1 || ldo < C || ldt < C || ldg < C) return SN_E_SHAPE;
  if (rows == 0) return SN_OK;
  if (!out || !target || !gloss || !gout) return SN_E_NULL;
  hipStream_t s = static_cast<hipStream_t>(stream);
  const bool vec = (C % 4 == 0) && (ldo % 4 == 0) && (ldt % 4 == 0) && (ldg % 4 == 0) && aligned16(out) &&
                   aligned16(target) && aligned16(gout);
  const int64_t items = rows * (vec ? C / 4 : C);
  int64_t blocks = (items + kWG - 1) / kWG;
  if (blocks > 16 * 1024) blocks = 16 * 1024;
  if (vec)
    hipLaunchKernelGGL((masked_sl1_bwd_k<true>), dim3((unsigned)blocks), dim3(kWG), 0, s, out, ldo, target, ldt, rowmask, rows, (int)C,
                       (float)scale, gloss, gout, ldg);
  else
    hipLaunchKernelGGL((masked_sl1_bwd_k<false>), dim3((unsigned)blocks), dim3(kWG), 0, s, out, ldo, target, ldt, rowmask, rows, (int)C,
                       (float)scale, gloss, gout, ldg);
  return launch_status();
}

int sn_gather_segments_f32(const float *src, const int64_t *base, int64_t nitems, int64_t rows_per_item, int64_t row_stride,
                           int32_t len, float *out, void *stream) {
  (void)hipGetLastError();
  if (nitems < 0 || rows_per_item < 0 || len < 1 || row_stride < 0) return SN_E_SHAPE;
  if (nitems * rows_per_item * len == 0) return SN_OK;
  if (!src || !base || !out) return SN_E_NULL;
  const bool vec = (len % 4 == 0) && aligned16(out);
  const int64_t total = nitems * rows_per_item * (vec ? len / 4 : len);
  int64_t blocks = (total + kWG - 1) / kWG;
  if (blocks > 64 * 1024) blocks = 64 * 1024;
  if (vec)
    hipLaunchKernelGGL((gather_segments_k<4>), dim3((unsigned)blocks), dim3(kWG), 0, static_cast<hipStream_t>(stream), src, base,
                       rows_per_item, row_stride, (int)len, total, out);
  else
    hipLaunchKernelGGL((gather_segments_k<1>), dim3((unsigned)blocks), dim3(kWG), 0, static_cast<hipStream_t>(stream), src, base,
                       rows_per_item, row_stride, (int)len, total, out);
  return launch_status();
}

int sn_gather_segments_ragged_f32(const float *src, const int64_t *base, const int64_t *item_off, int64_t nitems,
                                  int64_t total_rows, int64_t row_stride, int32_t len, float *out, void *stream) {
  (void)hipGetLastError();
  if (nitems < 0 || nitems > INT_MAX || total_rows < 0 || len < 1 || row_stride < 0) return SN_E_SHAPE;
  if (nitems == 0 || total_rows == 0) return SN_OK;
  if (!src || !base || !item_off || !out) return SN_E_NULL;
  const bool vec = (len % 4 == 0) && aligned16(out);
  const int64_t total = total_rows * (vec ? len / 4 : len);
  int64_t blocks = (total + kWG - 1) / kWG;
  if (blocks > 64 * 1024) blocks = 64 * 1024;
  if (vec)
    hipLaunchKernelGGL((gather_segments_ragged_k<4>), dim3((unsigned)blocks), dim3(kWG), 0, static_cast<hipStream_t>(stream), src,
                       base, item_off, (int)nitems, row_stride, (int)len, total, out);
  else
    hipLaunchKernelGGL((gather_segments_ragged_k<1>), dim3((unsigned)blocks), dim3(kWG), 0, static_cast<hipStream_t>(stream), src,
                       base, item_off, (int)nitems, row_stride, (int)len, total, out);
  return launch_status();
}

int sn_pair_ce_fwd_f32(const float *S, int64_t ld, const int64_t *target, int64_t NA, int64_t NB, float *lse, float *rowloss,
                       void *stream) {
  (void)hipGetLastError();
  if (NA < 0 || NB < 1 || ld < NB) return SN_E_SHAPE;
  if (NA > INT_MAX || NB > INT_MAX) return SN_E_RANGE;
  if (NA == 0) return SN_OK;
  if (!S || !target || !lse || !rowloss) return SN_E_NULL;
  hipStream_t s = static_cast<hipStream_t>(stream);
  if (aligned16(S) && (ld % 4) == 0)
    hipLaunchKernelGGL((pair_ce_fwd_k<true>), dim3((unsigned)NA), dim3(kWG), 0, s, S, ld, target, (int)NB, lse, rowloss);
  else
    hipLaunchKernelGGL((pair_ce_fwd_k<false>), dim3((unsigned)NA), dim3(kWG), 0, s, S, ld, target, (int)NB, lse, rowloss);
  return launch_status();
// ... 66 lines not shown
```

### surfacenetworks_amd/csrc/sn_gemm.hip

```cpp
#include <hip/hip_runtime.h>
#include <hip/hip_ext.h>
#include <stdint.h>
#include <stdlib.h>

#include "sn_spmm.h"

int sn_internal_cu_count();
hipError_t sn_internal_fill(void *dst, int value, size_t bytes, hipStream_t s);
hipError_t sn_internal_copy2d(void *dst, int64_t dpitch, const void *src, int64_t spitch, int64_t width, int64_t rows, hipStream_t s);
bool sn_internal_timing_slot(int kind, int64_t rows, int64_t width, int64_t bytes, int outw, hipEvent_t *s, hipEvent_t *e);

namespace {

constexpr int kWG = 256;
#define kCUs sn_internal_cu_count()
typedef float f4 __attribute__((ext_vector_type(4)));
typedef float f16v __attribute__((ext_vector_type(16)));

inline int launch_status() {
  const hipError_t e = hipGetLastError();
  return e == hipSuccess ? SN_OK : (int)e;
}
inline bool aligned16(const void *p) { return (reinterpret_cast<uintptr_t>(p) & 15u) == 0; }
inline bool ld32(int64_t a, int64_t b = 0, int64_t c = 0, int64_t d = 0, int64_t e = 0) {
  const int64_t lim = (int64_t)1 << 24;
  return a < lim && b < lim && c < lim && d < lim && e < lim;
}
__device__ __forceinline__ float elu1(float x) { return x > 0.f ? x : __expf(x) - 1.0f; }

enum { EPI_FWD = 0, EPI_DGRAD = 1, EPI_DGRAD_ELU = 2 };

struct EpiArgs {
  const float *v0, *v1, *v2, *v3;
  float *o2;
  int64_t ld1, ld2;
  const float *v4;
  int64_t ld3;
  int half;
  const float *segv;
  int64_t period, ldseg;
  const float *rowmask;
  double *stats;
  int stats_blocks;
  int jv;
  const int64_t *segoff;
  int nseg;
  float *absmax;
  int interleave;
  float *tile_sums;
};
constexpr int kAbsmaxBlocks = 512;

template <int K, int NT, bool TRANSW, int EPI>
__global__ __launch_bounds__(kWG, 1) void gemm_rows_k(const float *__restrict__ In, int64_t ldi,
                                                      const float *__restrict__ W, int64_t ldw,
                                                      float *__restrict__ Out, int64_t ldo, int64_t rows, EpiArgs ep) {
  constexpr int STEPS = K / 2;
  constexpr int LOADS = K / 8;
  const int wave = threadIdx.x >> 6, lane = threadIdx.x & 63;
  const int n = lane & 31, h = lane >> 5;
  float a[NT][STEPS];
#pragma unroll
  for (int t = 0; t < NT; ++t) {
    const int col = 32 * (wave * NT + t) + n;
#pragma unroll
    for (int t8 = 0; t8 < LOADS; ++t8) {
      if constexpr (!TRANSW) {
        const f4 w4 = *reinterpret_cast<const f4 *>(W + (int64_t)col * ldw + 8 * t8 + 4 * h);
        a[t][4 * t8 + 0] = w4.x; a[t][4 * t8 + 1] = w4.y; a[t][4 * t8 + 2] = w4.z; a[t][4 * t8 + 3] = w4.w;
      } else {
#pragma unroll
        for (int s = 0; s < 4; ++s) a[t][4 * t8 + s] = W[(int64_t)(8 * t8 + 4 * h + s) * ldw + col];
      }
    }
  }
  const int64_t ntiles = (rows + 31) / 32;
  const int64_t per = (ntiles + gridDim.x - 1) / gridDim.x;
  int64_t tile = (int64_t)blockIdx.x * per;
  const int64_t tend = tile + per < ntiles ? tile + per : ntiles;
  if (tile >= tend) return;
  f4 e0[NT][4], e1[NT][4], e2[NT][4];
  const bool affine = (EPI == EPI_DGRAD) && ep.v2 != nullptr;
#pragma unroll
  for (int t = 0; t < NT; ++t)
#pragma unroll
    for (int g = 0; g < 4; ++g) {
      const int c = 32 * (wave * NT + t) + 4 * h + 8 * g;
      const f4 z = {0.f, 0.f, 0.f, 0.f};
      if constexpr (EPI == EPI_FWD) {
        e0[t][g] = *reinterpret_cast<const f4 *>(ep.v0 + c);
        e1[t][g] = z;
        e2[t][g] = z;
      } else {
        e0[t][g] = (affine && ep.v1) ? *reinterpret_cast<const f4 *>(ep.v1 + c) : z;
        e1[t][g] = affine ? *reinterpret_cast<const f4 *>(ep.v2 + c) : z;
        e2[t][g] = affine ? *reinterpret_cast<const f4 *>(ep.v3 + c) : z;
      }
    }
  const bool side = (EPI == EPI_FWD) ? (ep.v1 != nullptr) : affine;
  const float *side_p = (EPI == EPI_FWD) ? ep.v1 : ep.v0;

  f4 b0[LOADS], b1[LOADS];
// ... 115 lines not shown
}
__device__ __forceinline__ unsigned row16_umax(unsigned v) {
  v = dpp_umax<0xB1>(v);
  v = dpp_umax<0x4E>(v);
  v = dpp_umax<0x141>(v);
  v = dpp_umax<0x140>(v);
  return v;
}

template <int I>
struct IC {
  static constexpr int value = I;
};
template <int I, int N, class F>
__device__ __forceinline__ void static_for(F &&f) {
  if constexpr (I < N) {
    f(IC<I>{});
    static_for<I + 1, N>(f);
  }
}

#define SN_LDS_BARRIER() asm volatile("s_waitcnt lgkmcnt(0)\n\ts_barrier" ::: "memory")

typedef __amdgpu_buffer_rsrc_t rsrc_t;
struct RowWindow {
  const char *p;
  int step;
  int n_full, n_last;
  __device__ __forceinline__ void init(const float *base, int64_t ld, int64_t row0, int last_rows, int span) {
    step = 128 * (int)ld;
    p = reinterpret_cast<const char *>(base + row0 * ld);
    n_full = 4 * (31 * (int)ld + span);
    n_last = 4 * ((last_rows - 1) * (int)ld + span);
  }
  __device__ __forceinline__ void init_empty() {
    step = 0;
    p = nullptr;
    n_full = n_last = 0;
  }
  __device__ __forceinline__ void next() { p += step; }
  __device__ __forceinline__ void stride(int g) { step *= g; }
  __device__ __forceinline__ rsrc_t rsrc(int to_last) const {
    const int n = to_last > 0 ? n_full : (to_last == 0 ? n_last : 0);
    return __builtin_amdgcn_make_buffer_rsrc(const_cast<char *>(p), 0, n, 0x00020000);
  }
};
__device__ __forceinline__ f4 bld4(rsrc_t r, int voff) {
  return __builtin_bit_cast(f4, __builtin_amdgcn_raw_buffer_load_b128(r, voff, 0, 0));
}
__device__ __forceinline__ void bst4(rsrc_t r, int voff, const f4 &v) {
  __builtin_amdgcn_raw_buffer_store_b128(__builtin_bit_cast(u4, v), r, voff, 0, 2);
}

template <int PC, int K, int NT, bool TRANSW, int EPI, bool SIDE, bool ELU, bool SMALL = false, int WV = 4, bool RAWLOW = false>
__global__ __launch_bounds__(64 * WV, (PC == 2 && K == 128 && NT == 1 && WV == 4) ? 2 : 1) void gemm_rows_split_k(const float *__restrict__ In, int64_t ldi,
                                                         const float *__restrict__ W, int64_t ldw,
                                                         float *__restrict__ Out, int64_t ldo, int64_t rows, EpiArgs ep) {
  constexpr int KS = K / 16;
  constexpr int RS = 2 * K + 16;
  constexpr int PART = 32 * RS;
  constexpr int SEG = K / 64;
  constexpr int NCH = 8 / WV;
  constexpr int NL = NCH * SEG;
  constexpr int CSTEP = KS / 2;
  constexpr int NOUT = 32 * WV * NT;
  constexpr int CPR = 8 * NT;
  constexpr int SROW = 16 * CPR + 16;
  constexpr int RPI = 64 / CPR;
  constexpr int NST = 32 / RPI;
  static_assert(PC == 2, "two fp16 pieces");
  __shared__ __attribute__((aligned(16))) unsigned char img[2][PC][PART];
  __shared__ __attribute__((aligned(16))) unsigned char stg[WV][32 * SROW];
  __shared__ float s_rs[2][32];
  __shared__ float s_amax[WV];
  __shared__ __attribute__((aligned(16))) float s_cs[NOUT];
  const int wave = __builtin_amdgcn_readfirstlane(threadIdx.x >> 6), lane = threadIdx.x & 63;
  const int n = lane & 31, h = lane >> 5;
  u4 wh[NT][KS], wl[NT][KS];
  constexpr int kOob = 0x7fffff00;
  const f4 zero4 = {0.f, 0.f, 0.f, 0.f};
  auto load_w = [&](int col, int ks, f4 &p, f4 &q) {
    if constexpr (!TRANSW) {
      p = q = zero4;
      if (col < ep.jv) {
        p = *reinterpret_cast<const f4 *>(W + (int64_t)col * ldw + 16 * ks + 8 * h);
        q = *reinterpret_cast<const f4 *>(W + (int64_t)col * ldw + 16 * ks + 8 * h + 4);
      }
    } else {
      const int k0w = 16 * ks + 8 * h;
      const float *w0 = W + (int64_t)k0w * ldw + col;
      p = q = zero4;
      if (k0w < ep.jv) p = f4{w0[0], w0[ldw], w0[2 * ldw], w0[3 * ldw]};
      if (k0w + 4 < ep.jv) q = f4{w0[4 * ldw], w0[5 * ldw], w0[6 * ldw], w0[7 * ldw]};
    }
  };
#pragma unroll
  for (int t = 0; t < NT; ++t) {
    const int col = 32 * (wave * NT + t) + n;
    float cup = 1.f;
    constexpr bool ONEPASS = SMALL && !(PC == 2 && K == 128 && NT == 1 && !TRANSW && !SIDE);
    f4 wp[ONEPASS ? KS : 1], wq[ONEPASS ? KS : 1];
    if constexpr (ONEPASS) {
#pragma unroll
      for (int ks = 0; ks < KS; ++ks) load_w(col, ks, wp[ks], wq[ks]);
    }
    {
      float cm = 0.f;
#pragma unroll
      for (int ks = 0; ks < KS; ++ks) {
        f4 p, q;
        if constexpr (ONEPASS) p = wp[ks], q = wq[ks];
        else load_w(col, ks, p, q);
        cm = fmaxf(cm, fmaxf(absmax4(p), absmax4(q)));
      }
      cm = fmaxf(cm, __shfl_xor(cm, 32));
      float cdown;
      pow2_scales(cm, cup, cdown);
      if (h == 0) s_cs[col] = cdown;
    }
#pragma unroll
    for (int ks = 0; ks < KS; ++ks) {
      f4 p, q;
      if constexpr (ONEPASS) p = wp[ks], q = wq[ks];
      else load_w(col, ks, p, q);
      split8_h2(p, q, cup, wh[t][ks], wl[t][ks]);
    }
  }
  __syncthreads();
  const int64_t ntiles = (rows + 31) / 32;
  const int64_t per = (ntiles + gridDim.x - 1) / gridDim.x;
  const int G = ep.interleave ? (int)gridDim.x : 1;
  int64_t tile = G > 1 ? (int64_t)blockIdx.x : (int64_t)blockIdx.x * per;
  const int64_t tend = G > 1 ? ntiles : (tile + per < ntiles ? tile + per : ntiles);
  constexpr bool STATS = (EPI == EPI_FWD) && ELU && NT == 1;
  if (tile >= tend) {
    if constexpr (STATS)
      if (ep.stats)
        for (int64_t b = blockIdx.x; b < ep.stats_blocks; b += gridDim.x) ep.stats[b * 256 + threadIdx.x] = 0.0;
    if constexpr (EPI == EPI_DGRAD_ELU)
      if (ep.absmax && threadIdx.x == 0)
        for (int b = blockIdx.x; b < kAbsmaxBlocks; b += gridDim.x) ep.absmax[b] = 0.f;
    return;
  }
  float amax = 0.f;
  double ssum[STATS ? 4 : 1], ssq[STATS ? 4 : 1];
#pragma unroll
  for (int i = 0; i < (STATS ? 4 : 1); ++i) ssum[i] = ssq[i] = 0.0;
  const int erow = lane / CPR;
  const int ecol = 32 * NT * wave + 4 * (lane % CPR);
  f4 k0 = {0.f, 0.f, 0.f, 0.f}, k1 = k0, k2 = k0;
  constexpr bool DGE = (EPI == EPI_DGRAD_ELU);
  static_assert(!DGE || SIDE, "the ELU variant needs the BatchNorm tail operand");
  static_assert(!RAWLOW || DGE, "the raw low half is a form of the input gradient through the activation");
  const bool lowhalf = DGE && 32 * NT * wave < ep.half;
  const bool colv = EPI != EPI_FWD || ecol < ep.jv;
  if constexpr (EPI == EPI_FWD) {
    if (colv) k0 = *reinterpret_cast<const f4 *>(ep.v0 + ecol);
  } else if constexpr (SIDE) {
    if (!(RAWLOW && lowhalf)) {
      if (ep.v1) k0 = *reinterpret_cast<const f4 *>(ep.v1 + ecol);
      k1 = *reinterpret_cast<const f4 *>(ep.v2 + ecol);
      k2 = *reinterpret_cast<const f4 *>(ep.v3 + ecol);
    }
  }
  const f4 kcs = *reinterpret_cast<const f4 *>(s_cs + ecol);
  unsigned char *const sw = &stg[wave][0] + n * SROW + 16 * h;
  const unsigned char *const sr = &stg[wave][0] + erow * SROW + 16 * (lane % CPR);
  const float *side_p = (EPI == EPI_FWD) ? ep.v1 : ep.v0;
  const bool has_out = (EPI != EPI_FWD && !DGE) || Out != nullptr;
  const bool has_ga = DGE && !RAWLOW && lowhalf && ep.v4 != nullptr;
  const int scol = RAWLOW ? ecol - ep.half : ecol;
  const int vo_side = (colv && (!RAWLOW || scol >= 0)) ? 4 * (erow * (int)ep.ld1 + scol) : kOob, js_side = 4 * RPI * (int)ep.ld1;
  const int vo_out = colv ? 4 * (erow * (int)ldo + ecol) : kOob, js_out = 4 * RPI * (int)ldo;
  const int vo_o2 = colv ? 4 * (erow * (int)ep.ld2 + ecol) : kOob, js_o2 = 4 * RPI * (int)ep.ld2;
  const int vo_ga = 4 * (erow * (int)ep.ld3 + ecol), js_ga = 4 * RPI * (int)ep.ld3;
  RowWindow w_in, w_side, w_out, w_o2, w_ga;
  const int64_t row0 = tile * 32;
  const int last_nrt = (int)(rows - (ntiles - 1) * 32);
  int to_last = (int)(ntiles - 1 - tile);
  const int ispan = EPI == EPI_FWD ? K : ep.jv;
  const int ospan = EPI == EPI_FWD ? ep.jv : NOUT;
  w_in.init(In, ldi, row0, last_nrt, ispan);
  if constexpr (SIDE) {
    if (RAWLOW && lowhalf) w_side.init_empty();
    else w_side.init(side_p, ep.ld1, row0, last_nrt, RAWLOW ? NOUT - ep.half : ospan);
  }
  if (has_out) w_out.init(Out, ldo, row0, last_nrt, ospan);
  else w_out.init_empty();
  if constexpr (DGE || (EPI == EPI_FWD && ELU)) w_o2.init(ep.o2, ep.ld2, row0, last_nrt, DGE ? ep.half : ospan);
  if constexpr (DGE) {
    if (has_ga) w_ga.init(ep.v4, ep.ld3, row0, last_nrt, ep.half);
    else w_ga.init_empty();
  }
  if (G > 1) {
    w_in.stride(G);
    if constexpr (SIDE) w_side.stride(G);
    w_out.stride(G);
    if constexpr (DGE || (EPI == EPI_FWD && ELU)) w_o2.stride(G);
    if constexpr (DGE) w_ga.stride(G);
  }
  const bool useseg = (ep.period > 0 || ep.segoff != nullptr) && (EPI == EPI_FWD || (DGE && lowhalf));
  int64_t seg_m = 0;
  int seg_left = 0;
  if (useseg) {
    if (ep.segoff) {
      int lo = 0, hi = ep.nseg - 1;
      while (lo < hi) {
        const int mid = (lo + hi + 1) >> 1;
        if (ep.segoff[mid] <= row0) lo = mid;
        else hi = mid - 1;
      }
      seg_m = lo;
      seg_left = (int)(ep.segoff[lo + 1] - row0);
    } else {
      seg_m = row0 / ep.period;
      seg_left = (int)((seg_m + 1) * ep.period - row0);
    }
  }

  const int lr = lane >> 4, lc = lane & 15;
  const int lrow = 4 * NCH * wave + lr;
  int lvo[SEG];
#pragma unroll
  for (int s = 0; s < SEG; ++s)
    lvo[s] = (EPI == EPI_FWD || 64 * s + 4 * lc < ep.jv) ? 4 * (lrow * (int)ldi + 4 * lc) + 256 * s : kOob;
  const int lps = 16 * (int)ldi;
  f4 raw[NL];
  auto load_chunk = [&](rsrc_t r, int p) {
#pragma unroll
    for (int s = 0; s < SEG; ++s) raw[p * SEG + s] = bld4(r, lvo[s] + p * lps);
  };
  auto convert_chunk = [&](int buf, int p) {
    unsigned char *d = &img[buf][0][0] + (lrow + 4 * p) * RS + 8 * lc;
    float m = absmax4(raw[p * SEG]);
#pragma unroll
    for (int s = 1; s < SEG; ++s) m = fmaxf(m, absmax4(raw[p * SEG + s]));
    float up, down;
    pow2_scales(__uint_as_float(row16_umax(__float_as_uint(m))), up, down);
#pragma unroll
    for (int s = 0; s < SEG; ++s) {
      u2 H, L;
      split4_h2(raw[p * SEG + s], up, H, L);
      *reinterpret_cast<u2 *>(d + 128 * s) = H;
      *reinterpret_cast<u2 *>(d + 128 * s + PART) = L;
    }
    if (lc == 0) s_rs[buf][lrow + 4 * p] = down;
  };
  {
    const rsrc_t r0 = w_in.rsrc(to_last);
#pragma unroll
    for (int p = 0; p < NCH; ++p) load_chunk(r0, p);
    w_in.next();
    const rsrc_t r1 = w_in.rsrc(to_last - G);
#pragma unroll
    for (int p = 0; p < NCH; ++p) {
      convert_chunk(0, p);
      load_chunk(r1, p);
    }
    w_in.next();
  }

  auto do_tile = [&](auto bufc, int64_t tl) {
    constexpr int buf = decltype(bufc)::value;
    SN_LDS_BARRIER();
    const rsrc_t r_in = w_in.rsrc(to_last - 2 * G);
    const int nrt = to_last == 0 ? last_nrt : 32;
    f4 sd[NST];
    if constexpr (SIDE) {
      if (!(RAWLOW && lowhalf)) {
        const rsrc_t r_side = w_side.rsrc(to_last);
#pragma unroll
        for (int j = 0; j < NST; ++j) sd[j] = bld4(r_side, vo_side + j * js_side);
      }
    }
    f4 sg0 = {0.f, 0.f, 0.f, 0.f}, sg1 = sg0;
    float smk[NST];
    int nb = 32;
    const bool usemask = DGE && useseg && ep.rowmask != nullptr;
    if (useseg) {
      while (seg_left <= 0) {
        ++seg_m;
        seg_left += ep.segoff ? (int)(ep.segoff[seg_m + 1] - ep.segoff[seg_m]) : (int)ep.period;
      }
      nb = seg_left < nrt ? seg_left : nrt;
      const float *s0 = ep.segv + seg_m * ep.ldseg + (colv ? ecol : 0);
      const float *s1 = nb < nrt ? s0 + ep.ldseg : s0;
      sg0 = *reinterpret_cast<const f4 *>(s0);
      sg1 = *reinterpret_cast<const f4 *>(s1);
      if constexpr (DGE) {
        if (usemask) {
          const float *mrow = ep.rowmask + tl * 32;
#pragma unroll
          for (int j = 0; j < NST; ++j) {
            const int rt = erow + RPI * j;
            smk[j] = mrow[rt < nrt ? rt : nrt - 1];
          }
        }
      }
    }
    f4 ga[NST];
    if constexpr (DGE && !RAWLOW) {
      if (lowhalf) {
        const rsrc_t r_ga = w_ga.rsrc(to_last);
#pragma unroll
        for (int j = 0; j < NST; ++j) ga[j] = bld4(r_ga, vo_ga + j * js_ga);
      }
    }
    f16v acc0[NT], acc1[NT];
    const f16v zero = {0.f, 0.f, 0.f, 0.f, 0.f, 0.f, 0.f, 0.f, 0.f, 0.f, 0.f, 0.f, 0.f, 0.f, 0.f, 0.f};
    const unsigned char *fp = &img[buf][0][0] + n * RS + 16 * h;
    constexpr int LOWP = PART;
    const float rs = s_rs[buf][n];
    u4 dh = *reinterpret_cast<const u4 *>(fp), dl = *reinterpret_cast<const u4 *>(fp + LOWP);
    static_for<0, KS>([&](auto ic) {
      constexpr int ks = decltype(ic)::value;
      __builtin_amdgcn_sched_barrier(0);
      u4 nh, nl;
      if constexpr (ks + 1 < KS) {
        nh = *reinterpret_cast<const u4 *>(fp + 32 * (ks + 1));
        nl = *reinterpret_cast<const u4 *>(fp + LOWP + 32 * (ks + 1));
      }
      if constexpr (ks % CSTEP == 0 && ks / CSTEP < NCH) {
        constexpr int p = ks / CSTEP;
        convert_chunk(buf ^ 1, p);
        load_chunk(r_in, p);
      }
#pragma unroll
      for (int t = 0; t < NT; ++t) acc1[t] = mfma_f16(wl[t][ks], dh, ks == 0 ? zero : acc1[t]);
#pragma unroll
      for (int t = 0; t < NT; ++t) acc0[t] = mfma_f16(wh[t][ks], dh, ks == 0 ? zero : acc0[t]);
#pragma unroll
      for (int t = 0; t < NT; ++t) acc1[t] = mfma_f16(wh[t][ks], dl, acc1[t]);
      if constexpr (ks + 1 < KS) {
        dh = nh; dl = nl;
      }
    });
    __builtin_amdgcn_sched_barrier(0);
#pragma unroll
    for (int t = 0; t < NT; ++t)
#pragma unroll
      for (int g = 0; g < 4; ++g)
        *reinterpret_cast<f4 *>(sw + 128 * t + 32 * g) =
            f4{__builtin_fmaf(acc1[t][4 * g], kLowDown, acc0[t][4 * g]) * rs,
               __builtin_fmaf(acc1[t][4 * g + 1], kLowDown, acc0[t][4 * g + 1]) * rs,
               __builtin_fmaf(acc1[t][4 * g + 2], kLowDown, acc0[t][4 * g + 2]) * rs,
               __builtin_fmaf(acc1[t][4 * g + 3], kLowDown, acc0[t][4 * g + 3]) * rs};
    const rsrc_t r_out = w_out.rsrc(to_last);
    rsrc_t r_o2 = r_out;
    if constexpr (DGE || (EPI == EPI_FWD && ELU)) r_o2 = w_o2.rsrc(to_last);
    auto out_row = [&](int j) {
      f4 v = *reinterpret_cast<const f4 *>(sr + RPI * j * SROW);
      v *= kcs;
      if constexpr (EPI == EPI_FWD) {
        if (useseg) v += (erow + RPI * j < nb ? sg0 : sg1);
        else v += k0;
        if constexpr (SIDE) v += sd[j];
      } else if constexpr (SIDE) {
        const f4 xv = sd[j] - k0;
        v.x += __builtin_fmaf(xv.x, k1.x, k2.x);
        v.y += __builtin_fmaf(xv.y, k1.y, k2.y);
        v.z += __builtin_fmaf(xv.z, k1.z, k2.z);
        v.w += __builtin_fmaf(xv.w, k1.w, k2.w);
      }
      return v;
    };
    if constexpr (RAWLOW) {
      if (lowhalf) {
#pragma unroll
        for (int j = 0; j < NST; ++j) {
          f4 v = *reinterpret_cast<const f4 *>(sr + RPI * j * SROW);
          v *= kcs;
          bst4(r_o2, vo_o2 + j * js_o2, v);
        }
      } else {
#pragma unroll
        for (int j = 0; j < NST; ++j) bst4(r_out, vo_out + j * js_out, out_row(j));
      }
    } else if constexpr (DGE) {
      if (lowhalf) {
#pragma unroll
        for (int j = 0; j < NST; ++j) {
          f4 v = out_row(j);
          const f4 o = sd[j];
          if (useseg) {
            f4 sv = erow + RPI * j < nb ? sg0 : sg1;
            if (usemask) sv *= smk[j];
            v += sv;
          }
          v = f4{__builtin_fmaf(v.x, fminf(o.x, 0.f), v.x), __builtin_fmaf(v.y, fminf(o.y, 0.f), v.y),
                 __builtin_fmaf(v.z, fminf(o.z, 0.f), v.z), __builtin_fmaf(v.w, fminf(o.w, 0.f), v.w)};
          v += ga[j];
          bst4(r_o2, vo_o2 + j * js_o2, v);
          const float m4 = fmaxf(fmaxf(__builtin_fabsf(v.x), __builtin_fabsf(v.y)), fmaxf(__builtin_fabsf(v.z), __builtin_fabsf(v.w)));
          amax = (erow + RPI * j < nrt) ? fmaxf(amax, m4) : amax;
        }
      } else {
#pragma unroll
        for (int j = 0; j < NST; ++j) bst4(r_out, vo_out + j * js_out, out_row(j));
      }
    } else {
      f4 tsum = {0.f, 0.f, 0.f, 0.f};
#pragma unroll
      for (int j = 0; j < NST; ++j) {
        const f4 v = out_row(j);
        bst4(r_out, vo_out + j * js_out, v);
        if constexpr (EPI == EPI_FWD && ELU) {
          const f4 ev = f4{elu1(v.x), elu1(v.y), elu1(v.z), elu1(v.w)};
          bst4(r_o2, vo_o2 + j * js_o2, ev);
          if constexpr (STATS) {
            if (erow + RPI * j < nrt) {
              const double e0 = ev.x, e1 = ev.y, e2 = ev.z, e3 = ev.w;
              ssum[0] += e0; ssum[1] += e1; ssum[2] += e2; ssum[3] += e3;
              ssq[0] = __builtin_fma(e0, e0, ssq[0]); ssq[1] = __builtin_fma(e1, e1, ssq[1]);
              ssq[2] = __builtin_fma(e2, e2, ssq[2]); ssq[3] = __builtin_fma(e3, e3, ssq[3]);
              tsum += ev;
            }
          }
        }
      }
      if constexpr (STATS) {
        if (ep.tile_sums) {
#pragma unroll
          for (int o = CPR; o < 64; o <<= 1) {
            tsum.x += __shfl_xor(tsum.x, o); tsum.y += __shfl_xor(tsum.y, o);
            tsum.z += __shfl_xor(tsum.z, o); tsum.w += __shfl_xor(tsum.w, o);
          }
          if (erow == 0) *reinterpret_cast<f4 *>(ep.tile_sums + tl * 128 + ecol) = tsum;
        }
      }
    }
    w_in.next();
    to_last -= G;
    seg_left -= 32 * G;
    if constexpr (SIDE) w_side.next();
    w_out.next();
    if constexpr (DGE || (EPI == EPI_FWD && ELU)) w_o2.next();
    if constexpr (DGE) w_ga.next();
  };
  while (true) {
    do_tile(IC<0>{}, tile);
    if ((tile += G) >= tend) break;
    do_tile(IC<1>{}, tile);
    if ((tile += G) >= tend) break;
  }
  if constexpr (EPI == EPI_DGRAD_ELU) {
    if (ep.absmax) {
      unsigned mb = __float_as_uint(amax);
#pragma unroll
      for (int o = 32; o > 0; o >>= 1) {
        const unsigned other = (unsigned)__shfl_xor((int)mb, o);
        mb = other > mb ? other : mb;
      }
      if (lane == 0) s_amax[wave] = __uint_as_float(mb);
      __syncthreads();
      if (threadIdx.x == 0) {
        float m = s_amax[0];
#pragma unroll
        for (int w = 1; w < WV; ++w) m = fmaxf(m, s_amax[w]);
        ep.absmax[blockIdx.x] = m;
        for (int b = blockIdx.x + gridDim.x; b < kAbsmaxBlocks; b += gridDim.x) ep.absmax[b] = 0.f;
      }
    }
  }
  if constexpr (STATS) {
    if (ep.stats) {
      static_assert(CPR == 8 && 32 * SROW >= 64 * 64, "statistics staging assumes the NT == 1 epilogue geometry");
      double *sl = reinterpret_cast<double *>(&stg[wave][0]);
#pragma unroll
      for (int i = 0; i < 4; ++i) {
        sl[lane * 8 + i] = ssum[i];
        sl[lane * 8 + 4 + i] = ssq[i];
      }
      const int chunk = lane >> 3, val = lane & 7;
      double tot = 0.0;
#pragma unroll
      for (int er = 0; er < 8; ++er) tot += sl[(er * 8 + chunk) * 8 + val];
      ep.stats[(int64_t)blockIdx.x * 256 + (val >> 2) * 128 + 32 * wave + 4 * chunk + (val & 3)] = tot;
      for (int64_t b = blockIdx.x + gridDim.x; b < ep.stats_blocks; b += gridDim.x) ep.stats[b * 256 + threadIdx.x] = 0.0;
    }
  }
}

typedef float f4v __attribute__((ext_vector_type(4)));
__device__ __forceinline__ f4 mfma16_f16(const u4 &a, const u4 &b, const f4 &c) {
  return __builtin_amdgcn_mfma_f32_16x16x32_f16(__builtin_bit_cast(h8v, a), __builtin_bit_cast(h8v, b), c, 0, 0, 0);
}

template <int K, bool SIDE, bool ELU>
__global__ __launch_bounds__(512, 1) void gemm_fwd_w8_k(const float *__restrict__ In, int64_t ldi, const float *__restrict__ W,
                                                        int64_t ldw, float *__restrict__ Out, int64_t ldo, int64_t rows,
// ... 279 lines not shown
}

int sn_linear_fwd_tiles_f32(const float *x, int64_t ldx, const float *W, int64_t ldw, const float *bias,
                            const float *residual, int64_t ldr, float *y, int64_t ldy, float *y_elu, int64_t lde,
                            int64_t rows, int32_t K, int32_t J, double *elu_stats_part, float *tile_sums, void *stream) {
  (void)hipGetLastError();
  if (tile_sums && (!elu_stats_part || J != 128)) return SN_E_UNSUPPORTED;
  if (rows < 0 || K < 1 || J < 1 || ldx < K || ldw < K || (y && ldy < J)) return SN_E_SHAPE;
  if (J > 128 || (J % 4) || (J != 128 && gemm_variant() == 0) || (K != 128 && K != 256) || !ld32(ldx, ldy, ldr, lde))
    return SN_E_UNSUPPORTED;
  if (rows == 0) return SN_OK;
  if (!x || !W || !bias || (!y && !(y_elu && gemm_variant() != 0))) return SN_E_NULL;
  if (!aligned16(x) || !aligned16(W) || !aligned16(bias) || (y && (!aligned16(y) || (ldy % 4))) || (ldx % 4) || (ldw % 4) ||
      (residual && (!aligned16(residual) || (ldr % 4) || ldr < J)) || (y_elu && (!aligned16(y_elu) || (lde % 4) || lde < J)))
    return SN_E_ALIGN;
  if (elu_stats_part && (!y_elu || gemm_variant() == 0)) return SN_E_UNSUPPORTED;
  EpiArgs ep{bias, residual, nullptr, nullptr, y_elu, ldr, lde, nullptr, 0, 0, nullptr, 0, 0, nullptr, elu_stats_part,
             sn_linear_fwd_stats_blocks(rows), (int)J, nullptr, 0, nullptr, 1, tile_sums};
  hipStream_t s = static_cast<hipStream_t>(stream);
  const unsigned grid = gemm_grid(rows, gemm_wgs(K, 1));
  const bool x3 = gemm_variant() != 0;
  hipEvent_t t_start = nullptr, t_stop = nullptr;
  if (x3)
    sn_internal_timing_slot(0x100 | (residual ? 2 : 0) | (y_elu ? 1 : 0) | (y ? 4 : 0), rows, K,
                            rows * 4 * ((int64_t)K + (y ? J : 0) + (residual ? J : 0) + (y_elu ? J : 0)), J, &t_start, &t_stop);
#define SN_X3_FWD(KK, RES, EL) SN_SPLIT_LAUNCH((KK, 1, false, EPI_FWD, RES, EL), x, ldx, W, ldw, y, ldy, rows, ep)
#define SN_W8_FWD(KK, RES, EL)                                                                                         \
  do {                                                                                                                 \
    if (t_start) hipExtLaunchKernelGGL((gemm_fwd_w8_k<KK, RES, EL>), dim3(grid8), dim3(512), 0, s, t_start, t_stop, 0, x, ldx, W, ldw, y, ldy, rows, ep); \
    else hipLaunchKernelGGL((gemm_fwd_w8_k<KK, RES, EL>), dim3(grid8), dim3(512), 0, s, x, ldx, W, ldw, y, ldy, rows, ep); \
  } while (0)
  if (linear_fwd_form(rows, K, J, residual != nullptr, y != nullptr, y_elu != nullptr, tile_sums != nullptr) == FWD_FORM_W8) {
    const unsigned grid8 = gemm_grid(rows, 1);
    SN_W8_FWD(256, false, true);
    return launch_status();
  }
  if (x3) {
    const int sel = (K == 256 ? 4 : 0) + (residual ? 2 : 0) + (y_elu ? 1 : 0);
    switch (sel) {
      case 0: SN_X3_FWD(128, false, false); break;
      case 1: SN_X3_FWD(128, false, true); break;
      case 2: SN_X3_FWD(128, true, false); break;
      case 3: SN_X3_FWD(128, true, true); break;
      case 4: SN_X3_FWD(256, false, false); break;
      case 5: SN_X3_FWD(256, false, true); break;
      case 6: SN_X3_FWD(256, true, false); break;
      default: SN_X3_FWD(256, true, true); break;
    }
  }
  else if (K == 256)
    hipLaunchKernelGGL((gemm_rows_k<256, 1, false, EPI_FWD>), dim3(grid), dim3(kWG), 0, s, x, ldx, W, ldw, y, ldy, rows, ep);
  else
    hipLaunchKernelGGL((gemm_rows_k<128, 1, false, EPI_FWD>), dim3(grid), dim3(kWG), 0, s, x, ldx, W, ldw, y, ldy, rows, ep);
  return launch_status();
}

int sn_linear_dgrad_f32(const float *dy, int64_t lddy, const float *W, int64_t ldw, const float *x, int64_t ldx,
                        const float *center, const float *B, const float *Cc, float *dx, int64_t lddx, int64_t rows,
                        int32_t J, int32_t C, void *stream) {
  (void)hipGetLastError();
  if (rows < 0 || J < 1 || C < 1 || lddy < J || ldw < C || lddx < C) return SN_E_SHAPE;
  if (J > 128 || (J % 4) || (J != 128 && gemm_variant() == 0) || (C != 128 && C != 256) || !ld32(lddy, ldx, lddx))
    return SN_E_UNSUPPORTED;
  if (rows == 0) return SN_OK;
  if (!dy || !W || !dx) return SN_E_NULL;
  if (B && (!x || !Cc)) return SN_E_NULL;
  if (!aligned16(dy) || !aligned16(W) || !aligned16(dx) || (lddy % 4) || (ldw % 4) || (lddx % 4)) return SN_E_ALIGN;
  if (B && (!aligned16(x) || !aligned16(B) || !aligned16(Cc) || (center && !aligned16(center)) || (ldx % 4) || ldx < C))
    return SN_E_ALIGN;
  EpiArgs ep{x, center, B, Cc, nullptr, ldx, 0, nullptr, 0, 0, nullptr, 0, 0, nullptr, nullptr, 0, (int)J, nullptr, 0, nullptr, 1, nullptr};
  hipStream_t s = static_cast<hipStream_t>(stream);
  const unsigned grid = gemm_grid(rows, gemm_wgs(128, C / 128));
  const bool x3 = gemm_variant() != 0;
  hipEvent_t t_start = nullptr, t_stop = nullptr;
  if (x3) sn_internal_timing_slot(0x200 | (B ? 1 : 0), rows, C, rows * 4 * ((int64_t)J + C + (B ? C : 0)), J, &t_start, &t_stop);
  if (C == 256 && x3 && B)
    SN_SPLIT_LAUNCH_NT2(128, EPI_DGRAD, true, dy, lddy, W, ldw, dx, lddx, rows, ep);
  else if (C == 256 && x3)
    SN_SPLIT_LAUNCH_NT2(128, EPI_DGRAD, false, dy, lddy, W, ldw, dx, lddx, rows, ep);
  else if (C == 256)
    hipLaunchKernelGGL((gemm_rows_k<128, 2, true, EPI_DGRAD>), dim3(grid), dim3(kWG), 0, s, dy, lddy, W, ldw, dx, lddx, rows, ep);
  else if (x3 && B)
    SN_SPLIT_LAUNCH((128, 1, true, EPI_DGRAD, true, false), dy, lddy, W, ldw, dx, lddx, rows, ep);
  else if (x3)
    SN_SPLIT_LAUNCH((128, 1, true, EPI_DGRAD, false, false), dy, lddy, W, ldw, dx, lddx, rows, ep);
  else
    hipLaunchKernelGGL((gemm_rows_k<128, 1, true, EPI_DGRAD>), dim3(grid), dim3(kWG), 0, s, dy, lddy, W, ldw, dx, lddx, rows, ep);
  return launch_status();
}

int32_t sn_linear_dgrad_absmax_blocks(void) { return kAbsmaxBlocks; }

int sn_linear_dgrad_elu_f32(const float *dy, int64_t lddy, const float *W, int64_t ldw, const float *x, int64_t ldx,
                            const float *center, const float *B, const float *Cc, float *dx_hi, int64_t lddx, float *gact,
                            int64_t ldga, const float *gadd, int64_t ldgadd, int64_t rows, int32_t J, int32_t C,
                            void *stream) {
  return sn_linear_dgrad_elu_absmax_f32(dy, lddy, W, ldw, x, ldx, center, B, Cc, dx_hi, lddx, gact, ldga, gadd, ldgadd, rows, J, C,
                                        nullptr, stream);
}

int sn_linear_dgrad_elu_absmax_f32(const float *dy, int64_t lddy, const float *W, int64_t ldw, const float *x, int64_t ldx,
                                   const float *center, const float *B, const float *Cc, float *dx_hi, int64_t lddx, float *gact,
                                   int64_t ldga, const float *gadd, int64_t ldgadd, int64_t rows, int32_t J, int32_t C,
                                   float *gact_absmax, void *stream) {
  (void)hipGetLastError();
  if (rows < 0 || J < 1 || C < 2 || lddy < J || ldw < C || lddx < C / 2 || ldga < C / 2 || ldx < C) return SN_E_SHAPE;
// ... 199 lines not shown
```

### surfacenetworks_amd/csrc/sn_plan_table.inc

```
SN_PLAN_FN(sn_spmm_csr_f32)
SN_PLAN_FN(sn_spmm_csr_stats_f32)
SN_PLAN_FN(sn_spmm_bsr4_f32)
SN_PLAN_FN(sn_spmm_csr_elubwd_f32)
SN_PLAN_FN(sn_spmm_bsr4_elubwd_f32)
SN_PLAN_FN(sn_spmm_q3_f32)
SN_PLAN_FN(sn_spmm_q3_stats_f32)
SN_PLAN_FN(sn_spmm_q3_elubwd_f32)
SN_PLAN_FN(sn_bsr4_to_q3_f32)
SN_PLAN_FN(sn_coo_to_csr_i32)
SN_PLAN_FN(sn_csr_transpose_f32)
SN_PLAN_FN(sn_bsr4_count)
SN_PLAN_FN(sn_bsr4_fill)
SN_PLAN_FN(sn_rb4_count)
SN_PLAN_FN(sn_rb4_fill)
SN_PLAN_FN(sn_spmm_rb4_f32)
SN_PLAN_FN(sn_spmm_rb4_elubwd_f32)
SN_PLAN_FN(sn_spmm_rb4_elubwd_absmax_f32)
SN_PLAN_FN(sn_spmm_rb4_stats_f32)
SN_PLAN_FN(sn_spmm_csr_ring_f32)
SN_PLAN_FN(sn_spmm_csr_ring_elubwd_f32)
SN_PLAN_FN(sn_spmm_csr_ring_elubwd_absmax_f32)
SN_PLAN_FN(sn_spmm_csr_ring_stats_f32)
SN_PLAN_FN(sn_csr_band_i32)
SN_PLAN_FN(sn_blockdiag_concat_i32)
SN_PLAN_FN(sn_blockdiag_concat_ragged_i32)
SN_PLAN_FN(sn_validate_csr_i32)
SN_PLAN_FN(sn_elu_into_f32)
SN_PLAN_FN(sn_elu_bwd_acc_f32)
SN_PLAN_FN(sn_colstats_f32)
SN_PLAN_FN(sn_wgrad_f32)
SN_PLAN_FN(sn_wgrad_seg_f32)
SN_PLAN_FN(sn_wgrad_slabs_f32)
SN_PLAN_FN(sn_wgrad_bounded_f32)
SN_PLAN_FN(sn_wgrad_seg_bounded_f32)
SN_PLAN_FN(sn_wgrad_slabs_bounded_f32)
SN_PLAN_FN(sn_avg_prep_ragged_f32)
SN_PLAN_FN(sn_bn_fold_seg_f32)
SN_PLAN_FN(sn_avg_bn_bwd_f32)
SN_PLAN_FN(sn_linear_dgrad_elu_absmax_f32)
SN_PLAN_FN(sn_linear_dgrad_eluseg_absmax_f32)
SN_PLAN_FN(sn_linear_dgrad_eluseg_ragged_absmax_f32)
SN_PLAN_FN(sn_spmm_q3_elubwd_absmax_f32)
SN_PLAN_FN(sn_spmm_q3_elubwd_tail_absmax_f32)
SN_PLAN_FN(sn_elu_tail_finish_f32)
SN_PLAN_FN(sn_linear_dgrad_elu_rawlow_f32)
SN_PLAN_FN(sn_wgrad_thin_f32)
SN_PLAN_FN(sn_masked_smooth_l1_fwd_f32)
SN_PLAN_FN(sn_masked_smooth_l1_bwd_f32)
SN_PLAN_FN(sn_pair_argmin_f32)
SN_PLAN_FN(sn_pair_ce_fwd_f32)
SN_PLAN_FN(sn_pair_ce_bwd_f32)
SN_PLAN_FN(sn_pair_fused_fwd_f32)
SN_PLAN_FN(sn_pair_fused_bwd_f32)
SN_PLAN_FN(sn_pair_soft_fwd_f32)
SN_PLAN_FN(sn_pair_soft_bwd_f32)
SN_PLAN_FN(sn_pair_sl1_fwd_f32)
SN_PLAN_FN(sn_pair_sl1_bwd_f32)
SN_PLAN_FN(sn_pair_match_f32)
SN_PLAN_FN(sn_gather_segments_f32)
SN_PLAN_FN(sn_gather_segments_ragged_f32)
SN_PLAN_FN(sn_linear_thin_fwd_f32)
SN_PLAN_FN(sn_bn_fold_f32)
SN_PLAN_FN(sn_colstats_merge2_f64)
SN_PLAN_FN(sn_colstats_partial_f32)
SN_PLAN_FN(sn_bn_bwd_coeffs_f32)
SN_PLAN_FN(sn_segment_colsum_ragged_f32)
SN_PLAN_FN(sn_bcast_rows_ragged_f32)
SN_PLAN_FN(sn_segment_colsum_f32)
SN_PLAN_FN(sn_bcast_rows_f32)
SN_PLAN_FN(sn_elu_bwd_bcast_f32)
SN_PLAN_FN(sn_dirac_bsr4_from_mesh)
SN_PLAN_FN(sn_laplacian_csr_from_mesh)
SN_PLAN_FN(sn_edge_lengths_csr_f32)
SN_PLAN_FN(sn_graph_apsp_f32)
SN_PLAN_FN(sn_graph_apsp_sweeps_f32)
SN_PLAN_FN(sn_symmetrize_min_f32)
SN_PLAN_FN(sn_mesh_corners_f32)
SN_PLAN_FN(sn_mesh_geodesics_f32)
SN_PLAN_FN(sn_mesh_geodesics_sweeps_f32)
SN_PLAN_FN(sn_mesh_glue_i32)
SN_PLAN_FN(sn_mesh_idt_rounds_f64)
SN_PLAN_FN(sn_mesh_idt_laplacian_f32)
SN_PLAN_FN(sn_mesh_components_i32)
SN_PLAN_FN(sn_mesh_label_mask_i32)
SN_PLAN_FN(sn_mesh_compact_i32)
SN_PLAN_FN(sn_mesh_weld_f32)
SN_PLAN_FN(sn_mesh_unique_faces_i32)
SN_PLAN_FN(sn_mesh_orient_i32)
SN_PLAN_FN(sn_mesh_descriptors_f32)
SN_PLAN_FN(sn_mesh_cot_laplacian_f32)
SN_PLAN_FN(sn_csr_spgemm_f32)
SN_PLAN_FN(sn_csr_inv_sqrt_degree_f32)
SN_PLAN_FN(sn_csr_scale_sym_f32)
SN_PLAN_FN(sn_linear_fwd_f32)
SN_PLAN_FN(sn_linear_fwd_tiles_f32)
SN_PLAN_FN(sn_linear_fwd_segbias_tiles_f32)
SN_PLAN_FN(sn_avg_stats_from_tiles_ragged_f32)
SN_PLAN_FN(sn_linear_fwd_segbias_ragged_tiles_f32)
SN_PLAN_FN(sn_avg_stats_from_tiles_f32)
SN_PLAN_FN(sn_colstats_into_f32)
SN_PLAN_FN(sn_colstats_merge_f64)
SN_PLAN_FN(sn_linear_dgrad_f32)
SN_PLAN_FN(sn_linear_dgrad_elu_f32)
SN_PLAN_FN(sn_linear_fwd_segbias_f32)
SN_PLAN_FN(sn_linear_dgrad_eluseg_f32)
SN_PLAN_FN(sn_avg_fwd_prep_f32)
SN_PLAN_FN(sn_avg_stats_f32)
SN_PLAN_FN(sn_seg_affine_f32)
SN_PLAN_FN(sn_avg_bwd_gc_f32)
SN_PLAN_FN(sn_avg_bwd_segvec_f32)
SN_PLAN_FN(sn_avg_bwd_segvec_ragged_f32)
SN_PLAN_FN(sn_linear_fwd_segbias_ragged_f32)
SN_PLAN_FN(sn_linear_dgrad_eluseg_ragged_f32)
SN_PLAN_FN(sn_affine_cols_acc_f32)
SN_PLAN_FN(sn_affine_cols_elu_bwd_f32)
```

### surfacenetworks_amd/functional.py

```python
from __future__ import annotations

import os

import torch

from . import _lib as _lib_mod
from . import kernels
from .operators import SparseOperator, as_operator

__all__ = ["spmm", "lap_propagate", "dirac_face_stage", "dirac_vert_stage", "avg_propagate", "avg_propagate_ragged", "bn_linear", "bnlin_forward",
           "bnlin_backward", "bn_prepare", "avg_stage_forward_ragged", "avg_stage_backward_ragged", "set_dirac_format", "set_laplacian_format", "SpmmTimer", "thin_linear", "thin_linear_supported"]

_DIRAC_FORMAT = "q3"
_LAPLACIAN_FORMAT = "ring"


def set_laplacian_format(fmt: str) -> None:
    global _LAPLACIAN_FORMAT
    if fmt not in ("ring", "rb4", "csr"):
        raise ValueError(fmt)
    _LAPLACIAN_FORMAT = fmt


def set_dirac_format(fmt: str) -> None:
# ... 353 lines not shown
    return buf[:k].view_as(stats).contiguous(), int(round(float(buf[k].item())))


def _sync_grad_stats(Gc, sdy):
    grp, n = _sync_world()
    if n == 1:
        return Gc, sdy, 1.0
    import torch.distributed as dist

    Gc = Gc.contiguous()
    dist.all_reduce(Gc, group=grp)
    sdy = sdy.contiguous()
    dist.all_reduce(sdy, group=grp)
    return Gc, sdy, 1.0 / n


def _scale_param_grads(scale, *grads):
    return grads if scale == 1.0 else tuple(None if g is None else g * scale for g in grads)


class _Const:
    __slots__ = ("v",)

    def __init__(self, v):
        self.v = v


def stash(ctx, *groups) -> None:
    tensors, spec = [], []
    for g in groups:
        gs = []
        for item in g:
            if isinstance(item, torch.Tensor):
                gs.append(len(tensors))
                tensors.append(item)
            else:
                gs.append(_Const(item))
        spec.append(gs)
    ctx.save_for_backward(*tensors)
    ctx._sn_spec = spec


def unstash(ctx):
    t = ctx.saved_tensors
    return [tuple(t[i] if isinstance(i, int) else i.v for i in gs) for gs in ctx._sn_spec]


def _take_counter(running_mean):
    d = getattr(running_mean, "__dict__", None)
    return d.pop("_sn_nbt", None) if d is not None else None


def bnlin_forward(x, gamma, beta, W, b, running_mean, running_var, training, momentum, eps, residual=None, elu_out=None,
                  want_y=True, elu_stats=None, pre_stats=None, tile_sums=None):
    part, part_hi = getattr(x, "_sn_part", None), getattr(x, "_sn_part_hi", None)
    x = _rows2d(x)
    rows = x.shape[0]
    nbt = _take_counter(running_mean)
    if not training:
        stats = None
    elif pre_stats is not None:
        stats = pre_stats
    elif ((part is not None or part_hi is not None) and x.shape[1] == 256) or \
            (part is not None and part_hi is not None and x.shape[1] == 128):
        stats = kernels.colstats_halves(x, part, part_hi)
    else:
        stats = kernels.colstats(x)
    rows_g = rows
    if training:
        stats, rows_g = _sync_stats(stats, rows)
    mean, invstd, s, t, Wf, bf = kernels.bn_fold(stats, rows_g, gamma, beta, W, b, eps, momentum, training, running_mean,
                                                 running_var, nbt)
    if residual is not None:
        residual = _rows2d(residual)
    if kernels.linear_fwd_supported(x.shape[1], W.shape[0]):
        y = kernels.linear_fwd(x, Wf, bf, residual, elu_out, want_y, elu_stats, tile_sums)
    else:
        if elu_stats is not None:
            raise ValueError("bnlin_forward: elu_stats needs a shape the fused GEMM covers")
        _library_gemm("the forward", x.shape[1], W.shape[0])
        y = torch.addmm(bf, x, Wf.t())
        if residual is not None:
            y += residual
        if elu_out is not None:
            kernels.elu_into(y, elu_out)
    return y, (x, W, Wf, s, mean, invstd, beta, training, b is not None, rows_g)


_STRICT = os.environ.get("SN_STRICT", "0") == "1"


def _library_gemm(what: str, K: int, J: int) -> None:
    if _STRICT:
        raise RuntimeError(f"SN_STRICT: {what} of a {K} -> {J} Linear would run on the library GEMM (no hand-written kernel for this shape)")


def _dy_bounds(dy, invstd, rows_g, training):
    if not training or not kernels.absmax_wanted():
        return None
    am = kernels.take_absmax(dy)
    if am is None:
        return None
    return am, invstd, rows_g


def _centered_wgrad(dy, x, mean, bounds=None):
    rows, C = x.shape
    J = dy.shape[1]
    if kernels.wgrad_supported(J, C):
        return kernels.wgrad(dy, x, mean, want_colsum=True, bounds=bounds)
    if C == 64 and rows % 2 == 0 and rows > 0 and x.is_contiguous() and dy.is_contiguous() and kernels.wgrad_supported(2 * J, 2 * C):
        if bounds is not None:
            bounds = (bounds[0], torch.cat([bounds[1], bounds[1]]), bounds[2])
        G2, s2 = kernels.wgrad(dy.view(rows // 2, 2 * J), x.view(rows // 2, 2 * C), torch.cat([mean, mean]), want_colsum=True,
                               bounds=bounds)
        return G2[:J, :C] + G2[J:, C:], s2[:J] + s2[J:]
    _library_gemm("the weight gradient", C, J)
    return dy.t().mm(x - mean), kernels.colstats(dy)


def _wgrad_and_coeffs(dy, x, W, s, mean, invstd, beta, training, has_bias, rows_g):
    bounds = _dy_bounds(dy, invstd, rows_g, training)
    Gc, sdy = _centered_wgrad(dy, x, mean, bounds)
    scale = 1.0
    if training:
        Gc, sdy, scale = _sync_grad_stats(Gc, sdy)
    dW, db, dgamma, dbeta, Bc, Cc = kernels.bn_bwd_coeffs(Gc, sdy, W, s, invstd, beta, rows_g, has_bias)
    dW, db, dgamma, dbeta = _scale_param_grads(scale, dW, db, dgamma, dbeta)
# ... 324 lines not shown
```

### surfacenetworks_amd/kernels.py

```python
from __future__ import annotations

import collections

import torch

from . import _lib

__all__ = [
    "note_absmax", "take_absmax", "absmax_wanted", "clear_absmax", "tile_sums_supported", "new_tile_sums", "avg_stats_from_tiles", "spmm_csr", "spmm_bsr4", "spmm_csr_elubwd", "spmm_bsr4_elubwd", "spmm_q3", "spmm_q3_stats", "spmm_q3_stats_supported", "spmm_csr_stats", "spmm_csr_stats_supported", "csr_to_rb4", "spmm_rb4", "spmm_rb4_stats", "spmm_rb4_supported", "spmm_ring", "spmm_ring_stats", "spmm_ring_supported", "ring_half_window", "csr_band", "bsr4_to_q3", "coo_to_csr", "csr_transpose", "csr_to_bsr4", "blockdiag_concat", "blockdiag_concat_ragged", "validate_csr",
    "elu_into", "elu_bwd", "colstats", "wgrad", "wgrad_supported", "affine_cols_acc", "affine_cols_elu_bwd",
    "bn_fold", "bn_bwd_coeffs", "segment_colsum", "bcast_rows", "segment_colsum_ragged", "bcast_rows_ragged", "elu_bwd_bcast", "dirac_from_mesh", "laplacian_from_mesh", "linear_fwd", "linear_fwd_supported", "linear_dgrad",
    "linear_dgrad_supported", "linear_dgrad_elu", "linear_dgrad_elu_supported",
    "avg_stage_supported", "avg_fwd_prep", "avg_stats", "seg_affine", "avg_bwd_gc", "avg_bwd_segvec", "linear_fwd_segbias", "linear_dgrad_eluseg", "wgrad_seg", "wgrad_slabs", "avg_bwd_segvec_ragged", "linear_fwd_segbias_ragged", "linear_dgrad_eluseg_ragged", "avg_stage_ragged_supported", "wgrad_thin", "wgrad_thin_supported", "linear_thin_fwd", "masked_smooth_l1_fwd", "masked_smooth_l1_bwd", "gather_segments", "pair_argmin", "pair_ce_fwd", "pair_ce_bwd", "pair_fused_fwd", "pair_fused_bwd", "colstats_partial", "linear_fwd_stats_blocks", "elu_stats_supported", "new_elu_stats_part", "colstats_halves", "colstats_into", "colstats_from_part", "colstats_merge_into",
    "avg_merged_supported", "avg_stats_ragged", "avg_stats_from_tiles_ragged", "gather_segments_ragged",
]


def _dev(*tensors) -> None:
    if _lib._recorder is not None and _lib.recorder() is not None and _lib._recorder.allow_cpu:
        return
    for t in tensors:
        if t is not None and not t.is_cuda:
            raise RuntimeError(
                "surfacenetworks_amd kernels run on the MI355X only: got a CPU tensor. There is no CPU/eager "
# ... 1176 lines not shown
_gemm_variant = None


def _split_gemm() -> bool:
    global _gemm_variant
    if _gemm_variant is None:
        _gemm_variant = int(_lib.load().sn_gemm_variant())
    return _gemm_variant != 0


def linear_fwd_supported(K: int, J: int) -> bool:
    return K in (128, 256) and (J == 128 or (_split_gemm() and 0 < J < 128 and J % 4 == 0))


def elu_stats_supported() -> bool:
    return _split_gemm()


def new_elu_stats_part(rows: int, device):
    nblk = int(_lib.load().sn_linear_fwd_stats_blocks(rows))
    return torch.empty((max(nblk, 1), 2, 128), dtype=torch.float64, device=device)


def tile_sums_supported() -> bool:
    return elu_stats_supported()


def new_tile_sums(rows: int, device):
    return torch.empty(((rows + 31) // 32, 128), dtype=torch.float32, device=device)


def linear_small_rows() -> int:
    return int(_lib.load().sn_linear_small_rows())


def linear_fwd_form(rows: int, K: int, J: int, residual: bool = False, want_y: bool = True, y_elu: bool = False,
                    tile_sums: bool = False) -> int:
    return int(_lib.load().sn_linear_fwd_form(rows, K, J, int(bool(residual)), int(bool(want_y)), int(bool(y_elu)),
                                              int(bool(tile_sums))))


def linear_fwd(x, W, bias, residual=None, y_elu=None, want_y: bool = True, elu_stats=None, tile_sums=None):
    _dev(x, W, bias, residual, y_elu, elu_stats, tile_sums)
    rows, K = x.shape
    J = W.shape[0]
    keep = want_y or y_elu is None
    y = torch.empty((rows, J), dtype=torch.float32, device=x.device) if (keep or not elu_stats_supported()) else None
    _lib.call("sn_linear_fwd_tiles_f32", _p(x), _ld(x), _p(W), _ld(W), _p(bias), _p(residual),
              _ld(residual) if residual is not None else 0, _p(y), J, _p(y_elu), _ld(y_elu) if y_elu is not None else 0,
              rows, K, J, _p(elu_stats), _p(tile_sums), _stream())
    return y if keep else None


def avg_stats_from_tiles(tile_sums, part, e, mask, inv_count, rows_per_seg: int, nseg: int):
    _dev(tile_sums, part, e, mask, inv_count)
    rows, C = e.shape
    if tile_sums.shape != ((rows + 31) // 32, 128) or part.dim() != 3 or part.shape[1:] != (2, 128) or part.dtype != torch.float64:
        raise ValueError("avg_stats_from_tiles: tile sums / statistics partials of another operand")
    nblk = int(_lib.load().sn_linear_fwd_stats_blocks(rows))
    if part.shape[0] < nblk:
        raise ValueError("avg_stats_from_tiles: partial buffer smaller than the producing launch's grid")
    m = torch.empty((nseg, C), dtype=torch.float32, device=e.device)
    stats = torch.empty((2, 2 * C), dtype=torch.float64, device=e.device)
    ws = torch.empty((nseg, C), dtype=torch.float32, device=e.device)
    _lib.call("sn_avg_stats_from_tiles_f32", _p(tile_sums), _p(part), nblk, _p(e), _ld(e), _p(mask), _p(inv_count.contiguous()),
              rows_per_seg, nseg, C, _p(m), _p(stats), _p(ws), _stream())
    return m, stats


def avg_stats_from_tiles_ragged(tile_sums, part, e, seg):
    _dev(tile_sums, part, e)
    rows, C = e.shape
    if tile_sums.shape != ((rows + 31) // 32, 128) or part.dim() != 3 or part.shape[1:] != (2, 128) or part.dtype != torch.float64:
        raise ValueError("avg_stats_from_tiles_ragged: tile sums / statistics partials of another operand")
    nblk = int(_lib.load().sn_linear_fwd_stats_blocks(rows))
    if part.shape[0] < nblk or seg.rows != rows:
        raise ValueError("avg_stats_from_tiles_ragged: partial buffer smaller than the producing launch's grid / another batch")
    m = torch.empty((seg.nseg, C), dtype=torch.float32, device=e.device)
    stats = torch.empty((2, 2 * C), dtype=torch.float64, device=e.device)
    ws = torch.empty((seg.nseg, C), dtype=torch.float32, device=e.device)
    _lib.call("sn_avg_stats_from_tiles_ragged_f32", _p(tile_sums), _p(part), nblk, _p(e), _ld(e), _p(seg.off_dev), _p(seg.inv_count),
              seg.nseg, C, _p(m), _p(stats), _p(ws), _stream())
    return m, stats


def colstats_from_part(part, rows: int):
    _dev(part)
    if part.dim() != 3 or part.shape[1:] != (2, 128) or part.dtype != torch.float64:
        raise ValueError("colstats_from_part: expected (nblk, 2, 128) float64 partials")
    nblk = int(_lib.load().sn_linear_fwd_stats_blocks(rows))
    if part.shape[0] < nblk:
        raise ValueError("colstats_from_part: partial buffer smaller than the producing launch's grid")
    out = torch.empty((2, 128), dtype=torch.float64, device=part.device)
    _lib.call("sn_colstats_merge_f64", _p(part), nblk, 128, _p(out), 128, 0, _stream())
    return out


def colstats_merge_into(part, out, offset: int) -> None:
    _dev(part, out)
    C = part.shape[2]
    if part.dim() != 3 or part.shape[1] != 2 or part.dtype != torch.float64 or out.dtype != torch.float64 or \
            not out.is_contiguous() or offset + C > out.shape[1]:
        raise ValueError("colstats_merge_into: (nblk, 2, C) float64 partials into a contiguous (2, width >= offset + C) tensor")
    _lib.call("sn_colstats_merge_f64", _p(part), int(part.shape[0]), C, _p(out), out.shape[1], offset, _stream())


# ... 437 lines not shown


def pair_match(FA, FB, NA: int, NB: int, both: bool = True, geoB=None, truthA=None):
    _dev(FA, FB, geoB, truthA)
    for t in (FA, FB):
        if t.dtype != torch.float32 or t.dim() != 2 or t.stride(1) != 1:
            raise TypeError("pair_match: row-major float32 feature matrices expected")
    if FA.shape[1] != FB.shape[1]:
        raise TypeError("pair_match: features of one width expected")
    if not (0 < NA <= FA.shape[0] and 0 < NB <= FB.shape[0]):
        raise ValueError("pair_match: NA / NB do not fit the feature matrices")
    if (geoB is None) != (truthA is None):
        raise ValueError("pair_match: geoB and truthA come together")
    if geoB is not None:
        if geoB.dtype != torch.float32 or geoB.dim() != 2 or geoB.stride(1) != 1 or truthA.dtype != torch.int64:
            raise TypeError("pair_match: a row-major float32 geodesic matrix and int64 true matches expected")
        if geoB.shape[0] < NB or geoB.shape[1] < NB or truthA.numel() != NA:
            raise ValueError("pair_match: geoB holds fewer than NB x NB entries, or truthA not NA")
        truthA = truthA.contiguous()
    dev = FA.device
    nbytes = _lib.load().sn_pair_match_workspace_bytes(FA.shape[0], FB.shape[0])
    ws = torch.empty(nbytes, dtype=torch.uint8, device=dev)
    colA = torch.empty(NA, dtype=torch.int64, device=dev)
    bestA = torch.empty(NA, dtype=torch.float32, device=dev)
    rowB = torch.empty(NB, dtype=torch.int64, device=dev) if both else None
    bestB = torch.empty(NB, dtype=torch.float32, device=dev) if both else None
    errA = torch.empty(NA, dtype=torch.float32, device=dev) if geoB is not None else None
    _lib.call("sn_pair_match_f32", _p(FA), FA.stride(0), _p(FB), FB.stride(0), NA, NB, FA.shape[0], FB.shape[0], FA.shape[1], _p(colA),
              _p(bestA), _p(rowB), _p(bestB), _p(geoB), geoB.stride(0) if geoB is not None else 0, _p(truthA), _p(errA), _p(ws), nbytes,
              _stream())
    return colA, bestA, rowB, bestB, errA


def masked_smooth_l1_fwd(out2d, target2d, rowmask, scale: float):
    _dev(out2d, target2d, rowmask)
    rows, C = out2d.shape
    loss = torch.empty((), dtype=torch.float32, device=out2d.device)
    ws_bytes = int(_lib.load().sn_masked_smooth_l1_workspace_bytes(rows, C))
    ws = torch.empty(ws_bytes, dtype=torch.uint8, device=out2d.device)
    _lib.call("sn_masked_smooth_l1_fwd_f32", _p(out2d), _ld(out2d), _p(target2d), _ld(target2d), _p(rowmask), rows, C,
              float(scale), _p(loss), _p(ws), ws_bytes, _stream())
    return loss


def masked_smooth_l1_bwd(out2d, target2d, rowmask, scale: float, gloss):
    _dev(out2d, target2d, rowmask, gloss)
    rows, C = out2d.shape
    g = torch.empty((rows, C), dtype=torch.float32, device=out2d.device)
    _lib.call("sn_masked_smooth_l1_bwd_f32", _p(out2d), _ld(out2d), _p(target2d), _ld(target2d), _p(rowmask), rows, C,
              float(scale), _p(gloss), _p(g), C, _stream())
    return g


def linear_fwd_segbias(x, W, segbias, rows_per_seg: int, residual=None, y_elu=None, want_y: bool = True, elu_stats=None,
                       tile_sums=None):
    _dev(x, W, segbias, residual, y_elu, tile_sums)
    rows, K = x.shape
    J = W.shape[0]
    y = torch.empty((rows, J), dtype=torch.float32, device=x.device) if want_y else None
    _lib.call("sn_linear_fwd_segbias_tiles_f32", _p(x), _ld(x), _p(W), _ld(W), _p(segbias), rows_per_seg, _p(residual),
              _ld(residual) if residual is not None else 0, _p(y), J, _p(y_elu), _ld(y_elu) if y_elu is not None else 0,
              rows, K, J, _p(elu_stats), _p(tile_sums), _stream())
    return y


def linear_dgrad_eluseg(dy, W, x, center, B, Cc, segvec, rows_per_seg: int, rowmask=None, gadd=None):
    _dev(dy, W, x, center, B, Cc, segvec, rowmask, gadd)
    rows, J = dy.shape
    C = x.shape[1]
    gact = torch.empty((rows, C), dtype=torch.float32, device=dy.device)
    am = _new_dgrad_absmax(dy.device)
    _lib.call("sn_linear_dgrad_eluseg_absmax_f32", _p(dy), _ld(dy), _p(W), _ld(W), _p(x), _ld(x), _p(center), _p(B), _p(Cc),
              _p(segvec), rows_per_seg, _p(rowmask), _p(gact), C, _p(gadd), _ld(gadd) if gadd is not None else 0, rows, J, C,
              _p(am), _stream())
    note_absmax(gact, am)
    return gact
```

### surfacenetworks_amd/utils_pt.py

```python
from __future__ import annotations

import numpy as np
import torch
import torch.nn as nn
import torch.nn.functional as F

from . import blocks as snB
from . import functional as snF
from .operators import PackedSegments, SparseOperator, as_operator
from .resident import LazySparse, batch_operator, reference_cat, reference_diag_cat

__all__ = [
    "sparse_cat", "sparse_diag_cat", "sp_sparse_to_pt_sparse", "to_dense_batched", "GraphConv1x1",
    "GraphBatchNorm", "global_average", "DenseLapResNet2", "LapResNet2", "DirResNet2", "AvgResNet2",
    "MlpResNet2", "SparseBMMFunc", "PackedSegments",
]


def sp_sparse_to_pt_sparse(L):
    return LazySparse.of_scipy(L)


def sparse_diag_cat(tensors, size0, size1):
    if len(tensors) and all(isinstance(t, LazySparse) for t in tensors):
# ... 17 lines not shown

def global_average(x, mask):
    if isinstance(mask, PackedSegments):
        return mask.mean(x.reshape(-1, x.shape[-1])).unsqueeze(1)
    m = mask.expand_as(x)
    return (x * m).sum(1, keepdim=True) / m.sum(1, keepdim=True)


class SparseBMMFunc:

    def __call__(self, matrix1, matrix2):
        op = as_operator(matrix1)
        B, _, N = matrix2.shape
        y = snF.spmm(op, matrix2.reshape(-1, N), 1)
        return y.view(B, -1, N)


class GraphConv1x1(nn.Module):

    def __init__(self, num_inputs, num_outputs, batch_norm=None):
        super().__init__()
        self.num_inputs, self.num_outputs, self.batch_norm = num_inputs, num_outputs, batch_norm
        if batch_norm == "pre":
            self.bn = nn.BatchNorm1d(num_inputs)
        if batch_norm == "post":
            self.bn = nn.BatchNorm1d(num_outputs)
        self.fc = nn.Linear(num_inputs, num_outputs)

    def forward2d(self, x2d, residual=None):
        if self.batch_norm == "pre":
            if x2d.dtype == torch.float32 and self.bn.affine and self.bn.momentum is not None:
                return snF.bn_linear(x2d, self.bn, self.fc, residual)
            x2d = self.bn(x2d)
        if self.batch_norm is None and snF.thin_linear_supported(x2d, self.fc):
            want_elu = residual is None and self.num_outputs % 4 == 0 and 256 % (self.num_outputs // 4) == 0
            x2d, cat = snF.thin_linear(x2d, self.fc, want_elu)
            if cat is not None:
                snB.attach_activated(x2d, cat)
        else:
            x2d = self.fc(x2d)
        if self.batch_norm == "post":
            x2d = self.bn(x2d)
        return x2d if residual is None else x2d + residual

    def forward(self, x):
        batch_size, num_nodes, num_inputs = x.size()
        assert num_inputs == self.num_inputs
        y2d = self.forward2d(x.reshape(-1, num_inputs))
        cat = snB.take_activated(y2d, y2d.shape[0], self.num_outputs)
        y = y2d.view(batch_size, num_nodes, self.num_outputs)
        return y if cat is None else snB.attach_activated(y, cat)


def elu_conv1x1(conv: GraphConv1x1, x: torch.Tensor) -> torch.Tensor:
    if USE_WHOLE_BLOCKS and snB.elu_conv_ok(conv, x):
        return snB.elu_conv(conv, x)
    return conv(F.elu(x))


class GraphBatchNorm(nn.Module):

    def __init__(self, num_inputs):
        super().__init__()
        self.bn = nn.BatchNorm1d(num_inputs)

    def forward(self, x):
        self.bn.train()
        b, n, c = x.size()
        return self.bn(x.reshape(b * n, c)).view(b, n, c)


def _blocks_ok(mod, x) -> bool:
    c = x.shape[-1]
    if not USE_WHOLE_BLOCKS or x.dtype != torch.float32 or c % 4 or 256 % (c // 4):
        return False
    mods = mod.__dict__["_modules"]
    for name in ("bn_fc0", "bn_fc1"):
        bn = mods[name].__dict__["_modules"]["bn"].__dict__
        if not (bn["affine"] and bn["momentum"] is not None and bn["track_running_stats"]):
            return False
    return True


USE_WHOLE_BLOCKS = True


class _TwoStage(nn.Module):

    def __init__(self, num_outputs):
        super().__init__()
        self.num_outputs = num_outputs
        self.bn_fc0 = GraphConv1x1(2 * num_outputs, num_outputs, batch_norm="pre")
        self.bn_fc1 = GraphConv1x1(2 * num_outputs, num_outputs, batch_norm="pre")


class DenseLapResNet2(_TwoStage):

    def forward(self, L, mask, inputs):
        x = F.elu(inputs)
        x = self.bn_fc0(torch.cat([x, torch.bmm(L, x)], 2))
        x = F.elu(x)
        x = self.bn_fc1(torch.cat([x, torch.bmm(L, x)], 2))
        return x + inputs


class LapResNet2(_TwoStage):

    def forward(self, L, mask, inputs, avg_next=None):
        if isinstance(L, torch.Tensor) and L.layout == torch.strided:
            return DenseLapResNet2.forward(self, L, mask, inputs)
        batch, node, feat = inputs.size()
        op = as_operator(L)
        if _blocks_ok(self, inputs):
            return snB.lap_block(self, op, inputs, avg_next)
        x2d = inputs.reshape(batch * node, feat)
        h = self.bn_fc0.forward2d(snF.lap_propagate(op, x2d))
        h = self.bn_fc1.forward2d(snF.lap_propagate(op, h), residual=x2d)
        return h.view(batch, node, feat)


class DirResNet2(_TwoStage):

    def __init__(self, num_outputs, res_f=False):
        super().__init__(num_outputs)
        self.res_f = res_f

    def forward(self, Di, DiA, v, f, f_out_needed=True, num_faces=None, avg_next=None):
        batch_size, num_nodes, num_inputs = v.size()
        if f is None:
            if num_faces is None:
                raise ValueError("DirResNet2: f=None needs num_faces")
            if _blocks_ok(self, v) and snB.zero_faces_ok(self, num_inputs):
                return snB.dirac_block(self, Di, DiA, v, None, f_out_needed, num_faces, avg_next)
            f = torch.zeros(batch_size, int(num_faces), num_inputs, dtype=v.dtype, device=v.device)
        _, num_faces, _ = f.size()
        if _blocks_ok(self, v):
            return snB.dirac_block(self, Di, DiA, v, f, f_out_needed, None, avg_next)
        v2d = v.reshape(batch_size * num_nodes, num_inputs)
        cat0, e_v = snF.dirac_face_stage(as_operator(Di), v2d, f.reshape(batch_size * num_faces, num_inputs))
        f_out = self.bn_fc0.forward2d(cat0)
        cat1 = snF.dirac_vert_stage(as_operator(DiA), f_out, e_v)
        v_new = self.bn_fc1.forward2d(cat1, residual=v2d)
        return v_new.view(batch_size, num_nodes, num_inputs), f_out.view(batch_size, num_faces, num_inputs)


class AvgResNet2(_TwoStage):

    def forward(self, L, mask, inputs):
        b, n, c = inputs.size()
        if isinstance(mask, PackedSegments):
            if self.training and snB.avg_block_ragged_ok(self, mask, inputs):
                return snB.avg_block_ragged(self, mask, inputs)
            x2d = inputs.reshape(b * n, c)
            h = self.bn_fc0.forward2d(snF.avg_propagate_ragged(x2d, mask))
            h = self.bn_fc1.forward2d(snF.avg_propagate_ragged(h, mask), residual=x2d)
            return h.view(b, n, c)
        if c % 4 or 256 % (c // 4) or inputs.dtype != torch.float32:
            x = F.elu(inputs)
            x = self.bn_fc0(torch.cat([x, global_average(x, mask).expand_as(x)], 2))
            x = F.elu(x)
            x = self.bn_fc1(torch.cat([x, global_average(x, mask).expand_as(x)], 2))
            return x + inputs
        if _blocks_ok(self, inputs):
            return snB.avg_block(self, mask, inputs)
        h = self.bn_fc0.forward2d(snF.avg_propagate(inputs, mask))
        h = self.bn_fc1.forward2d(snF.avg_propagate(h.view(b, n, c), mask), residual=inputs.reshape(b * n, c))
        return h.view(b, n, c)


class MlpResNet2(nn.Module):

    def __init__(self, num_outputs):
        super().__init__()
        self.num_outputs = num_outputs
        self.bn0 = GraphBatchNorm(num_outputs)
        self.fc0 = GraphConv1x1(num_outputs, num_outputs, batch_norm=None)
        self.bn1 = GraphBatchNorm(num_outputs)
        self.fc1 = GraphConv1x1(num_outputs, num_outputs, batch_norm=None)

    def forward(self, L, mask, inputs):
        x = self.fc0(F.elu(self.bn0(inputs)))
        x = self.fc1(F.elu(self.bn1(x)))
        return x + inputs
```

Before: 3427 meshes/s.

## Fuse prediction tail: frame-add epilogue, skip last-block v store, loss computes grad

Adds a GEMM epilogue that adds the last input frame to the final 1x1 conv output, removing a separate broadcast-add pass. The last Dirac block no longer writes its raw vertex output when only the activated hand-off is consumed. The smooth-L1 loss forward also writes the gradient buffer, so backward only rescales it by gloss. This saves several memory passes over the tail, at the cost of more code paths and placeholder tensors that break if a consumer reads them.

```diff
diff --git a/include/sn_spmm.h b/include/sn_spmm.h
--- a/include/sn_spmm.h
+++ b/include/sn_spmm.h
@@ -198,6 +198,12 @@
 int sn_masked_smooth_l1_bwd_f32(const float *out, int64_t ldo, const float *target, int64_t ldt, const float *rowmask,
                                 int64_t rows, int32_t C, double scale, const float *gloss, float *gout, int64_t ldg,
                                 void *stream);
+int sn_masked_smooth_l1_fwdg_f32(const float *out, int64_t ldo, const float *target, int64_t ldt, const float *rowmask,
+                                 int64_t rows, int32_t C, double scale, float *loss, float *gout, int64_t ldg, void *workspace,
+                                 size_t workspace_bytes, void *stream);
+int sn_masked_smooth_l1_bwdg_f32(const float *out, int64_t ldo, const float *target, int64_t ldt, const float *rowmask,
+                                 int64_t rows, int32_t C, double scale, const float *gloss, float *gout, int64_t ldg,
+                                 void *stream);
 int sn_gather_segments_f32(const float *src, const int64_t *base, int64_t nitems, int64_t rows_per_item, int64_t row_stride,
                            int32_t len, float *out, void *stream);
 int sn_gather_segments_ragged_f32(const float *src, const int64_t *base, const int64_t *item_off, int64_t nitems,
@@ -439,6 +445,9 @@
 int sn_linear_fwd_tiles_f32(const float *x, int64_t ldx, const float *W, int64_t ldw, const float *bias, const float *residual,
                             int64_t ldr, float *y, int64_t ldy, float *y_elu, int64_t lde, int64_t rows, int32_t K, int32_t J,
                             double *elu_stats_part, float *tile_sums, void *stream);
+int32_t sn_linear_fwd_frame_supported(int32_t K, int32_t J);
+int sn_linear_fwd_frame_f32(const float *x, int64_t ldx, const float *W, int64_t ldw, const float *bias, const float *frame,
+                            int64_t ldf, float *y, int64_t ldy, int64_t rows, int32_t K, int32_t J, void *stream);
 int sn_linear_fwd_segbias_tiles_f32(const float *x, int64_t ldx, const float *W, int64_t ldw, const float *segbias,
                                     int64_t rows_per_seg, const float *residual, int64_t ldr, float *y, int64_t ldy, float *y_elu,
                                     int64_t lde, int64_t rows, int32_t K, int32_t J, double *elu_stats_part, float *tile_sums,
diff --git a/surfacenetworks_amd/_lib.py b/surfacenetworks_amd/_lib.py
--- a/surfacenetworks_amd/_lib.py
+++ b/surfacenetworks_amd/_lib.py
@@ -92,6 +92,8 @@
     "sn_masked_smooth_l1_workspace_bytes": (_sz, [_i64, _i32]),
     "sn_masked_smooth_l1_fwd_f32": (C.c_int, [_vp, _i64, _vp, _i64, _vp, _i64, _i32, C.c_double, _vp, _vp, _sz, _vp]),
     "sn_masked_smooth_l1_bwd_f32": (C.c_int, [_vp, _i64, _vp, _i64, _vp, _i64, _i32, C.c_double, _vp, _vp, _i64, _vp]),
+    "sn_masked_smooth_l1_fwdg_f32": (C.c_int, [_vp, _i64, _vp, _i64, _vp, _i64, _i32, C.c_double, _vp, _vp, _i64, _vp, _sz, _vp]),
+    "sn_masked_smooth_l1_bwdg_f32": (C.c_int, [_vp, _i64, _vp, _i64, _vp, _i64, _i32, C.c_double, _vp, _vp, _i64, _vp]),
     "sn_pair_argmin_f32": (C.c_int, [_vp, _i64, _i64, _vp, _vp, _i64, _vp, _i64, _i64, _vp, _vp]),
     "sn_pair_ce_fwd_f32": (C.c_int, [_vp, _i64, _vp, _i64, _i64, _vp, _vp, _vp]),
     "sn_pair_ce_bwd_f32": (C.c_int, [_vp, _i64, _vp, _vp, _vp, _i64, _i64, _i64, _i64, _vp, _i64, _vp]),
@@ -174,6 +176,8 @@
     "sn_linear_small_rows": (_i64, []),
     "sn_linear_fwd_form": (_i32, [_i64, _i32, _i32, _i32, _i32, _i32, _i32]),
     "sn_linear_fwd_tiles_f32": (C.c_int, [_vp, _i64, _vp, _i64, _vp, _vp, _i64, _vp, _i64, _vp, _i64, _i64, _i32, _i32, _vp, _vp, _vp]),
+    "sn_linear_fwd_frame_supported": (_i32, [_i32, _i32]),
+    "sn_linear_fwd_frame_f32": (C.c_int, [_vp, _i64, _vp, _i64, _vp, _vp, _i64, _vp, _i64, _i64, _i32, _i32, _vp]),
     "sn_linear_fwd_segbias_tiles_f32": (C.c_int, [_vp, _i64, _vp, _i64, _vp, _i64, _vp, _i64, _vp, _i64, _vp, _i64, _i64, _i32, _i32,
                                                   _vp, _vp, _vp]),
     "sn_avg_stats_from_tiles_ragged_f32": (C.c_int, [_vp, _vp, _i32, _vp, _i64, _vp, _vp, _i64, _i32, _vp, _vp, _vp, _vp]),
diff --git a/surfacenetworks_amd/arap.py b/surfacenetworks_amd/arap.py
--- a/surfacenetworks_amd/arap.py
+++ b/surfacenetworks_amd/arap.py
@@ -15,6 +15,8 @@
 INPUT_FRAMES = 2
 OUTPUT_FRAMES = 40
 
+FUSED_TAIL = True
+
 
 def _num_faces(Di, DiA, batch_size):
     return DiA.size(2) // 4 if len(Di.size()) == 3 else DiA.size(1) // 4 // batch_size
@@ -24,6 +26,13 @@
 def _add_last_frame(x, inputs, frames):
     B, V, _ = x.shape
     return (x.reshape(B, V, frames, 3) + inputs[:, :, None, -3:]).reshape(B, V, 3 * frames)
+
+
+def _predict(conv2, x, inputs):
+    frame = inputs[:, :, -3:]
+    if FUSED_TAIL and utils.elu_conv1x1_frame_ok(conv2, x, frame):
+        return utils.elu_conv1x1(conv2, x, frame)
+    return _add_last_frame(utils.elu_conv1x1(conv2, x), inputs, OUTPUT_FRAMES)
 
 
 class Model(nn.Module):
@@ -48,8 +57,7 @@
                 x = blk(L, mask, x, avg_next=i + 1 < self.layer)
             else:
                 x = blk(L, mask, x)
-        x = utils.elu_conv1x1(self.conv2, x)
-        return _add_last_frame(x, inputs, OUTPUT_FRAMES)
+        return _predict(self.conv2, x, inputs)
 
 
 class AvgModel(nn.Module):
@@ -65,8 +73,7 @@
         x = self.conv1(inputs)
         for i in range(15):
             x = self._modules["rn{}".format(i)](L, mask, x)
-        x = utils.elu_conv1x1(self.conv2, x)
-        return _add_last_frame(x, inputs, OUTPUT_FRAMES)
+        return _predict(self.conv2, x, inputs)
 
 
 class MlpModel(nn.Module):
@@ -102,29 +109,37 @@
         v = self.conv1(inputs)
         f = None
         nf = _num_faces(Di, DiA, batch_size)
+        last_v = not (FUSED_TAIL and utils.USE_WHOLE_BLOCKS and utils.snB.elu_conv_ok(self.conv2, v))
         for i in range(15):
             blk = self._modules["rn{}".format(i)]
             if i % 2 == 0:
                 v, f = blk(Di, DiA, v, f, f_out_needed=False, num_faces=nf,
-                           avg_next=i + 1 < 15)
+                           avg_next=i + 1 < 15,
+                           v_out_needed=i + 1 < 15 or last_v)
             else:
                 v = blk(None, mask, v)
-        x = utils.elu_conv1x1(self.conv2, v)
-        return _add_last_frame(x, inputs, OUTPUT_FRAMES)
+        return _predict(self.conv2, v, inputs)
 
 
 class _MaskedSmoothL1(torch.autograd.Function):
 
     @staticmethod
-    def forward(ctx, out2d, tgt2d, rowmask, scale):
+    def forward(ctx, out2d, tgt2d, rowmask, scale, with_grad=False):
         ctx.save_for_backward(out2d, tgt2d, rowmask)
         ctx.scale = scale
+        ctx.g = None
+        if with_grad:
+            loss, ctx.g = kernels.masked_smooth_l1_fwdg(out2d, tgt2d, rowmask, scale)
+            return loss
         return kernels.masked_smooth_l1_fwd(out2d, tgt2d, rowmask, scale)
 
     @staticmethod
     def backward(ctx, gloss):
         out2d, tgt2d, rowmask = ctx.saved_tensors
-        return kernels.masked_smooth_l1_bwd(out2d, tgt2d, rowmask, ctx.scale, gloss.contiguous()), None, None, None
+        g, ctx.g = ctx.g, None
+        if g is not None:
+            return kernels.masked_smooth_l1_bwdg(out2d, tgt2d, rowmask, ctx.scale, gloss.contiguous(), g), None, None, None, None
+        return kernels.masked_smooth_l1_bwd(out2d, tgt2d, rowmask, ctx.scale, gloss.contiguous()), None, None, None, None
 
 
 def loss_fn(outputs, targets, mask, batch_size):
@@ -133,8 +148,9 @@
     if outputs.dim() == 3 and outputs.dtype == torch.float32 and targets.dtype == torch.float32 and \
             not targets.requires_grad and mask.numel() == outputs.shape[0] * outputs.shape[1]:
         C = outputs.shape[2]
+        with_grad = bool(FUSED_TAIL and outputs.is_cuda and outputs.requires_grad and torch.is_grad_enabled())
         out = _MaskedSmoothL1.apply(outputs.reshape(-1, C), targets.reshape(-1, C).contiguous(),
-                                    mask.reshape(-1).to(torch.float32).contiguous(), 1.0 / batch_size)
+                                    mask.reshape(-1).to(torch.float32).contiguous(), 1.0 / batch_size, with_grad)
         return out
     outputs = outputs * mask.expand_as(outputs)
     return F.smooth_l1_loss(outputs, targets, reduction="sum") / batch_size
diff --git a/surfacenetworks_amd/blocks.py b/surfacenetworks_amd/blocks.py
--- a/surfacenetworks_amd/blocks.py
+++ b/surfacenetworks_amd/blocks.py
@@ -12,7 +12,8 @@
 from .graphs import active_capture
 from .operators import as_operator
 
-__all__ = ["lap_block", "dirac_block", "avg_block", "avg_block_ragged", "avg_block_ragged_ok", "take_activated", "attach_activated", "zero_faces_ok", "elu_conv", "elu_conv_ok"]
+__all__ = ["lap_block", "dirac_block", "avg_block", "avg_block_ragged", "avg_block_ragged_ok", "take_activated", "attach_activated", "zero_faces_ok", "elu_conv", "elu_conv_ok",
+           "elu_conv_frame_ok"]
 
 
 DEFER_FACE_TAIL = True
@@ -244,8 +245,8 @@
     return t
 
 
-def _dirac_fwd(v, f, pre_v, pre_f, g0, b0, W0, c0, rm0, rv0, g1, b1, W1, c1, rm1, rv1, opDi, opDiA, need_f, avg_next, tr0, mo0,
-               ep0, tr1, mo1, ep1):
+def _dirac_fwd(v, f, pre_v, pre_f, g0, b0, W0, c0, rm0, rv0, g1, b1, W1, c1, rm1, rv1, opDi, opDiA, need_f, need_v, avg_next, tr0,
+               mo0, ep0, tr1, mo1, ep1):
     rv, C = v.shape
     rf = opDi.shape[0] // 4
     cat1 = _activated(v, pre_v)
@@ -265,7 +266,8 @@
     nxt_v = _new_cat(rv, C, v.device)
     pv = _new_part(rv, C, v.device, narrow=True)
     tv = _new_tiles(rv, C, v.device, pv, avg_next)
-    v_new, st1 = bnlin_forward(cat1, g1, b1, W1, c1, rm1, rv1, tr1, mo1, ep1, v, nxt_v[:, :C], elu_stats=pv, tile_sums=tv)
+    v_new, st1 = bnlin_forward(cat1, g1, b1, W1, c1, rm1, rv1, tr1, mo1, ep1, v, nxt_v[:, :C], want_y=need_v, elu_stats=pv,
+                               tile_sums=tv)
     _attach_part(nxt_v, pv, tv)
     return (v_new, f_out, nxt_v, nxt_f), ((cat0, cat1, nxt_f), st0, st1)
 
@@ -314,8 +316,8 @@
 class _DiracBlock(torch.autograd.Function):
 
     @staticmethod
-    def forward(ctx, v, f, opDi, opDiA, pre_v, pre_f, need_f, avg_next, g0, b0, W0, c0, rm0, rv0, tr0, mo0, ep0, g1, b1, W1, c1,
-                rm1, rv1, tr1, mo1, ep1):
+    def forward(ctx, v, f, opDi, opDiA, pre_v, pre_f, need_f, need_v, avg_next, g0, b0, W0, c0, rm0, rv0, tr0, mo0, ep0, g1, b1, W1,
+                c1, rm1, rv1, tr1, mo1, ep1):
         v = _rows2d(v)
         if f is not None and pre_f is None:
             f = _rows2d(f)
@@ -328,7 +330,7 @@
             box[0] = True
         ctx.rawbox = [False] if not need_f else None
         tensors = (v, f, pre_v, pre_f, g0, b0, W0, c0, rm0, rv0, g1, b1, W1, c1, rm1, rv1)
-        consts = (need_f, avg_next, tr0, mo0, ep0, tr1, mo1, ep1)
+        consts = (need_f, need_v, avg_next, tr0, mo0, ep0, tr1, mo1, ep1)
         outs = None
         ctx._sn_plan = None
         if plans.usable(v):
@@ -344,6 +346,8 @@
             f_out = _nan_placeholder(v.device).expand(nxt_f.shape[0], v.shape[1])
             if ctx.rawbox is not None:
                 nxt_f._sn_rawbox = ctx.rawbox
+        if v_new is None:
+            v_new = _nan_placeholder(v.device).expand(v.shape[0], v.shape[1])
         ctx.mark_non_differentiable(nxt_v, nxt_f)
         ctx.set_materialize_grads(False)
         return v_new, f_out, nxt_v, nxt_f
@@ -351,7 +355,7 @@
     @staticmethod
     def backward(ctx, g_vnew, g_fout, _gv, _gf):
         if g_vnew is None and g_fout is None:
-            return (None,) * 26
+            return (None,) * 27
         opDi, opDiA = ctx.ops
         g_vnew = g_vnew.contiguous() if g_vnew is not None else None
         g_fout = g_fout.contiguous() if g_fout is not None else None
@@ -366,7 +370,7 @@
         else:
             r = _dirac_bwd(unstash(ctx), opDi, opDiA, g_vnew, g_fout, *consts)
         none5 = (None,) * 5
-        return (r[0], r[1], None, None, None, None, None, None) + r[2:6] + none5 + r[6:10] + none5
+        return (r[0], r[1], None, None, None, None, None, None, None) + r[2:6] + none5 + r[6:10] + none5
 
 
 def _drop_counters(*running_means) -> None:
@@ -376,7 +380,7 @@
             d.pop("_sn_nbt", None)
 
 
-def dirac_block(mod, Di, DiA, v, f, need_f=True, num_faces=None, avg_next=None):
+def dirac_block(mod, Di, DiA, v, f, need_f=True, num_faces=None, avg_next=None, need_v=True):
     B, V, C = v.shape
     F_ = f.shape[1] if f is not None else int(num_faces)
     rv, rf = B * V, B * F_
@@ -385,7 +389,7 @@
         raise ValueError(f"DirResNet2: Di {tuple(opDi.shape)} / DiA {tuple(opDiA.shape)} do not match v rows {rv}, f rows {rf}")
     v_new, f_out, nxt_v, nxt_f = _DiracBlock.apply(v.reshape(rv, C), f.reshape(rf, C) if f is not None else None, opDi, opDiA,
                                                   take_activated(v, rv, C),
-                                                  take_activated(f, rf, C) if f is not None else None, bool(need_f),
+                                                  take_activated(f, rf, C) if f is not None else None, bool(need_f), bool(need_v),
                                                   _wants_tiles(mod, avg_next), *_bn_args(mod._modules["bn_fc0"]), *_bn_args(mod._modules["bn_fc1"]))
     _mark_producer(nxt_v, mod, avg_next)
     return attach_activated(v_new.view(B, V, C), nxt_v), attach_activated(f_out.view(B, F_, C), nxt_f)
@@ -657,12 +661,12 @@
     return attach_activated(out.view(B, V, C), nxt)
 
 
-def _elu_conv_fwd(v, pre, g0, b0, W0, c0, rm0, rv0, tr0, mo0, ep0):
+def _elu_conv_fwd(v, pre, frame, g0, b0, W0, c0, rm0, rv0, tr0, mo0, ep0):
     C = v.shape[1]
     cat = _activated(v, pre)
     part = getattr(cat, "_sn_part", None)
     pre_stats = kernels.colstats_from_part(part, v.shape[0]) if (part is not None and tr0 and C == 128) else None
-    y, st = bnlin_forward(cat[:, :C], g0, b0, W0, c0, rm0, rv0, tr0, mo0, ep0, pre_stats=pre_stats)
+    y, st = bnlin_forward(cat[:, :C], g0, b0, W0, c0, rm0, rv0, tr0, mo0, ep0, pre_stats=pre_stats, frame=frame)
     return (y,), (st,)
 
 
@@ -675,14 +679,15 @@
 class _EluConv(torch.autograd.Function):
 
     @staticmethod
-    def forward(ctx, v, pre, g0, b0, W0, c0, rm0, rv0, tr0, mo0, ep0):
-        v = _rows2d(v)
-        tensors = (v, pre, g0, b0, W0, c0, rm0, rv0)
+    def forward(ctx, v, pre, frame, g0, b0, W0, c0, rm0, rv0, tr0, mo0, ep0):
+        if pre is None:
+            v = _rows2d(v)
+        tensors = (v, pre, frame, g0, b0, W0, c0, rm0, rv0)
         consts = (tr0, mo0, ep0)
         ctx._sn_plan = None
         outs = None
         if plans.usable(v):
-            outs = _plan_forward(ctx, _SITES["elu_conv_fwd"], _elu_conv_fwd, tensors, (), consts, v.shape[1], 2, (1, 6))
+            outs = _plan_forward(ctx, _SITES["elu_conv_fwd"], _elu_conv_fwd, tensors, (), consts, v.shape[1], 3, (1, 7))
             if outs is not None:
                 _drop_counters(rm0)
         ctx._sn_planned = outs is not None
@@ -699,14 +704,36 @@
             r = _plan_backward(ctx, _SITES["elu_conv_bwd"], _elu_conv_bwd, (dy,), (need,))
         else:
             r = _elu_conv_bwd(unstash(ctx), dy, need)
-        return (r[0], None) + r[1:5] + (None,) * 5
-
-
-def elu_conv(conv, v):
+        return (r[0], None, None) + r[1:5] + (None,) * 5
+
+
+def _unwritten(t: torch.Tensor) -> bool:
+    return t.numel() > 1 and not any(t.stride())
+
+
+def elu_conv(conv, v, frame=None):
     B, N, C = v.shape
     rows = B * N
-    y = _EluConv.apply(v.reshape(rows, C), take_activated(v, rows, C), *_bn_args(conv))
+    pre = take_activated(v, rows, C)
+    if pre is None and _unwritten(v):
+        raise RuntimeError("elu_conv: the vertex features are the placeholder of a block that ran with v_out_needed=False, and the "
+                           "activated hand-off that stands for them is gone (taken by another consumer, or the tensor was copied)")
+    if frame is not None:
+        frame = frame.detach().reshape(rows, 3)
+    y = _EluConv.apply(v.reshape(rows, C), pre, frame, *_bn_args(conv))
     return y.view(B, N, conv.num_outputs)
+
+
+def elu_conv_frame_ok(conv, v, frame) -> bool:
+    B, N, C = v.shape
+    J = conv.num_outputs
+    if not (v.is_cuda and frame.is_cuda and frame.dtype == torch.float32 and tuple(frame.shape) == (B, N, 3)) or \
+            (frame.requires_grad and torch.is_grad_enabled()):
+        return False
+    if not (kernels.linear_fwd_supported(C, J) and kernels.linear_fwd_frame_supported(C, J)):
+        return False
+    s = frame.stride()
+    return s[2] == 1 and s[1] >= 3 and (B == 1 or s[0] == N * s[1]) and frame.data_ptr() % 4 == 0
 
 
 def elu_conv_ok(conv, v) -> bool:
diff --git a/surfacenetworks_amd/csrc/sn_dense.hip b/surfacenetworks_amd/csrc/sn_dense.hip
--- a/surfacenetworks_amd/csrc/sn_dense.hip
+++ b/surfacenetworks_amd/csrc/sn_dense.hip
@@ -4,6 +4,8 @@
 #include <limits.h>
 #include <stdint.h>
 #include <stdlib.h>
+
+#include <type_traits>
 
 #include "sn_dense_common.h"
 
@@ -635,7 +637,7 @@
 
 __device__ __forceinline__ float sl1_grad(float d) { return d < -1.f ? -1.f : (d > 1.f ? 1.f : d); }
 
-template <bool VEC>
+template <bool VEC, bool SKIP1 = false>
 __global__ __launch_bounds__(kWG) void masked_sl1_bwd_k(const float *__restrict__ o, int64_t ldo,
                                                         const float *__restrict__ t, int64_t ldt,
                                                         const float *__restrict__ mask, int64_t rows, int C, float scale,
@@ -644,6 +646,8 @@
   constexpr int W = VEC ? 4 : 1;
   const int cw = C / W;
   const int64_t total = rows * cw;
+  if constexpr (SKIP1)
+    if (gloss[0] == 1.0f) return;
   const float gs = gloss[0] * scale;
   for (int64_t i = (int64_t)blockIdx.x * kWG + threadIdx.x; i < total; i += (int64_t)gridDim.x * kWG) {
     const int64_t r = i / cw;
@@ -658,6 +662,81 @@
       g[r * ldg + c] = gm * sl1_grad(o[r * ldo + c] * m - t[r * ldt + c]);
     }
   }
+}
+
+template <bool VEC>
+__global__ __launch_bounds__(kWG) void masked_sl1_fwdg_k(const float *__restrict__ o, int64_t ldo,
+                                                         const float *__restrict__ t, int64_t ldt,
+                                                         const float *__restrict__ mask, int64_t rows, int C, float scale,
+                                                         double *__restrict__ partial, float *__restrict__ g, int64_t ldg) {
+  __shared__ double red[kWG];
+  constexpr int W = VEC ? 4 : 1;
+  constexpr int U = 4;
+  typedef typename std::conditional<VEC, f4, float>::type item_t;
+  const int cw = C / W;
+  const int64_t total = rows * cw;
+  const int64_t stride = (int64_t)gridDim.x * kWG;
+  const int64_t dr = stride / cw;
+  const int dc = (int)(stride - dr * cw);
+  const float gs = 1.0f * scale;
+  int64_t i = (int64_t)blockIdx.x * kWG + threadIdx.x;
+  int64_t r = i / cw;
+  int ci = (int)(i - r * cw);
+  auto load = [&](const float *p) {
+    if constexpr (VEC) return ld4_s(p, 1);
+    else return *p;
+  };
+  auto consume = [&](const item_t &ov, const item_t &tv, float m, float *gp, double &acc) {
+    const float gm = gs * m;
+    if constexpr (VEC) {
+      const float dx = ov.x * m - tv.x, dy = ov.y * m - tv.y, dz = ov.z * m - tv.z, dw = ov.w * m - tv.w;
+      acc += sl1(dx) + sl1(dy) + sl1(dz) + sl1(dw);
+      st4_s(gp, f4{gm * sl1_grad(dx), gm * sl1_grad(dy), gm * sl1_grad(dz), gm * sl1_grad(dw)}, 1);
+    } else {
+      const float d = ov * m - tv;
+      acc += sl1(d);
+      *gp = gm * sl1_grad(d);
+    }
+  };
+  double acc = 0;
+  for (; i + (U - 1) * stride < total; i += U * stride) {
+    item_t ov[U], tv[U];
+    float m[U];
+    float *gp[U];
+#pragma unroll
+    for (int u = 0; u < U; ++u) {
+      const int c = ci * W;
+      m[u] = mask ? mask[r] : 1.f;
+      ov[u] = load(o + r * ldo + c);
+      tv[u] = load(t + r * ldt + c);
+      gp[u] = g + r * ldg + c;
+      r += dr;
+      ci += dc;
+      if (ci >= cw) {
+        ci -= cw;
+        ++r;
+      }
+    }
+#pragma unroll
+    for (int u = 0; u < U; ++u) consume(ov[u], tv[u], m[u], gp[u], acc);
+  }
+  for (; i < total; i += stride) {
+    const int c = ci * W;
+    consume(load(o + r * ldo + c), load(t + r * ldt + c), mask ? mask[r] : 1.f, g + r * ldg + c, acc);
+    r += dr;
+    ci += dc;
+    if (ci >= cw) {
+      ci -= cw;
+      ++r;
+    }
+  }
+  red[threadIdx.x] = acc;
+  __syncthreads();
+  for (int s = kWG / 2; s > 0; s >>= 1) {
+    if (threadIdx.x < s) red[threadIdx.x] += red[threadIdx.x + s];
+    __syncthreads();
+  }
+  if (threadIdx.x == 0) partial[blockIdx.x] = red[0];
 }
 
 template <int W>
@@ -2469,9 +2548,36 @@
   return launch_status();
 }
 
-int sn_masked_smooth_l1_bwd_f32(const float *out, int64_t ldo, const float *target, int64_t ldt, const float *rowmask,
-                                int64_t rows, int32_t C, double scale, const float *gloss, float *gout, int64_t ldg,
-                                void *stream) {
+int sn_masked_smooth_l1_fwdg_f32(const float *out, int64_t ldo, const float *target, int64_t ldt, const float *rowmask,
+                                 int64_t rows, int32_t C, double scale, float *loss, float *gout, int64_t ldg, void *workspace,
+                                 size_t workspace_bytes, void *stream) {
+  (void)hipGetLastError();
+  if (rows < 0 || C < 1 || ldo < C || ldt < C || ldg < C) return SN_E_SHAPE;
+  if (!loss) return SN_E_NULL;
+  hipStream_t s = static_cast<hipStream_t>(stream);
+  if (rows == 0) {
+    const hipError_t e = sn_internal_fill(loss, 0, sizeof(float), s);
+    return e == hipSuccess ? SN_OK : (int)e;
+  }
+  if (!out || !target || !gout || !workspace) return SN_E_NULL;
+  if (workspace_bytes < (size_t)kLossBlocks * sizeof(double)) return SN_E_WORKSPACE;
+  const bool vec = (C % 4 == 0) && (ldo % 4 == 0) && (ldt % 4 == 0) && aligned16(out) && aligned16(target);
+  if (vec && ((ldg % 4) || !aligned16(gout))) return SN_E_ALIGN;
+  const int nblk = loss_blocks(rows * (vec ? C / 4 : C));
+  double *partial = static_cast<double *>(workspace);
+  if (vec)
+    hipLaunchKernelGGL((masked_sl1_fwdg_k<true>), dim3(nblk), dim3(kWG), 0, s, out, ldo, target, ldt, rowmask, rows, (int)C,
+                       (float)scale, partial, gout, ldg);
+  else
+    hipLaunchKernelGGL((masked_sl1_fwdg_k<false>), dim3(nblk), dim3(kWG), 0, s, out, ldo, target, ldt, rowmask, rows, (int)C,
+                       (float)scale, partial, gout, ldg);
+  hipLaunchKernelGGL(masked_sl1_final_k, dim3(1), dim3(kWG), 0, s, partial, nblk, scale, loss);
+  return launch_status();
+}
+
+static int masked_sl1_bwd_launch(const float *out, int64_t ldo, const float *target, int64_t ldt, const float *rowmask,
+                                 int64_t rows, int32_t C, double scale, const float *gloss, float *gout, int64_t ldg,
+                                 bool skip1, void *stream) {
   (void)hipGetLastError();
   if (rows < 0 || C < 1 || ldo < C || ldt < C || ldg < C) return SN_E_SHAPE;
   if (rows == 0) return SN_OK;
@@ -2482,13 +2588,30 @@
   const int64_t items = rows * (vec ? C / 4 : C);
   int64_t blocks = (items + kWG - 1) / kWG;
   if (blocks > 16 * 1024) blocks = 16 * 1024;
-  if (vec)
-    hipLaunchKernelGGL((masked_sl1_bwd_k<true>), dim3((unsigned)blocks), dim3(kWG), 0, s, out, ldo, target, ldt, rowmask, rows, (int)C,
-                       (float)scale, gloss, gout, ldg);
-  else
-    hipLaunchKernelGGL((masked_sl1_bwd_k<false>), dim3((unsigned)blocks), dim3(kWG), 0, s, out, ldo, target, ldt, rowmask, rows, (int)C,
-                       (float)scale, gloss, gout, ldg);
-  return launch_status();
+#define SN_SL1_BWD(VEC_, SKIP_)                                                                                          \
+  hipLaunchKernelGGL((masked_sl1_bwd_k<VEC_, SKIP_>), dim3((unsigned)blocks), dim3(kWG), 0, s, out, ldo, target, ldt, rowmask, rows, \
+                     (int)C, (float)scale, gloss, gout, ldg)
+  if (skip1) {
+    if (vec) SN_SL1_BWD(true, true);
+    else SN_SL1_BWD(false, true);
+  } else {
+    if (vec) SN_SL1_BWD(true, false);
+    else SN_SL1_BWD(false, false);
+  }
+#undef SN_SL1_BWD
+  return launch_status();
+}
+
+int sn_masked_smooth_l1_bwd_f32(const float *out, int64_t ldo, const float *target, int64_t ldt, const float *rowmask,
+                                int64_t rows, int32_t C, double scale, const float *gloss, float *gout, int64_t ldg,
+                                void *stream) {
+  return masked_sl1_bwd_launch(out, ldo, target, ldt, rowmask, rows, C, scale, gloss, gout, ldg, false, stream);
+}
+
+int sn_masked_smooth_l1_bwdg_f32(const float *out, int64_t ldo, const float *target, int64_t ldt, const float *rowmask,
+                                 int64_t rows, int32_t C, double scale, const float *gloss, float *gout, int64_t ldg,
+                                 void *stream) {
+  return masked_sl1_bwd_launch(out, ldo, target, ldt, rowmask, rows, C, scale, gloss, gout, ldg, true, stream);
 }
 
 int sn_gather_segments_f32(const float *src, const int64_t *base, int64_t nitems, int64_t rows_per_item, int64_t row_stride,
diff --git a/surfacenetworks_amd/csrc/sn_gemm.hip b/surfacenetworks_amd/csrc/sn_gemm.hip
--- a/surfacenetworks_amd/csrc/sn_gemm.hip
+++ b/surfacenetworks_amd/csrc/sn_gemm.hip
@@ -48,6 +48,8 @@
   float *absmax;
   int interleave;
   float *tile_sums;
+  const float *frame;
+  int64_t ldf;
 };
 constexpr int kAbsmaxBlocks = 512;
 
@@ -269,7 +271,8 @@
   __builtin_amdgcn_raw_buffer_store_b128(__builtin_bit_cast(u4, v), r, voff, 0, 2);
 }
 
-template <int PC, int K, int NT, bool TRANSW, int EPI, bool SIDE, bool ELU, bool SMALL = false, int WV = 4, bool RAWLOW = false>
+template <int PC, int K, int NT, bool TRANSW, int EPI, bool SIDE, bool ELU, bool SMALL = false, int WV = 4, bool RAWLOW = false,
+          bool FRAME = false>
 __global__ __launch_bounds__(64 * WV, (PC == 2 && K == 128 && NT == 1 && WV == 4) ? 2 : 1) void gemm_rows_split_k(const float *__restrict__ In, int64_t ldi,
                                                          const float *__restrict__ W, int64_t ldw,
                                                          float *__restrict__ Out, int64_t ldo, int64_t rows, EpiArgs ep) {
@@ -369,6 +372,7 @@
   constexpr bool DGE = (EPI == EPI_DGRAD_ELU);
   static_assert(!DGE || SIDE, "the ELU variant needs the BatchNorm tail operand");
   static_assert(!RAWLOW || DGE, "the raw low half is a form of the input gradient through the activation");
+  static_assert(!FRAME || (EPI == EPI_FWD && !SIDE && !ELU && NT == 1), "the frame epilogue is a form of the plain forward");
   const bool lowhalf = DGE && 32 * NT * wave < ep.half;
   const bool colv = EPI != EPI_FWD || ecol < ep.jv;
   if constexpr (EPI == EPI_FWD) {
@@ -391,7 +395,10 @@
   const int vo_out = colv ? 4 * (erow * (int)ldo + ecol) : kOob, js_out = 4 * RPI * (int)ldo;
   const int vo_o2 = colv ? 4 * (erow * (int)ep.ld2 + ecol) : kOob, js_o2 = 4 * RPI * (int)ep.ld2;
   const int vo_ga = 4 * (erow * (int)ep.ld3 + ecol), js_ga = 4 * RPI * (int)ep.ld3;
-  RowWindow w_in, w_side, w_out, w_o2, w_ga;
+  const int fph = ecol % 3;
+  const int vo_fr = FRAME ? 4 * erow * (int)ep.ldf : 0, js_fr = FRAME ? 4 * RPI * (int)ep.ldf : 0;
+  const int fo0 = 4 * fph, fo1 = 4 * ((fph + 1) % 3), fo2 = 4 * ((fph + 2) % 3);
+  RowWindow w_in, w_side, w_out, w_o2, w_ga, w_fr;
   const int64_t row0 = tile * 32;
   const int last_nrt = (int)(rows - (ntiles - 1) * 32);
   int to_last = (int)(ntiles - 1 - tile);
@@ -408,6 +415,10 @@
   if constexpr (DGE) {
     if (has_ga) w_ga.init(ep.v4, ep.ld3, row0, last_nrt, ep.half);
     else w_ga.init_empty();
+  }
+  if constexpr (FRAME) {
+    w_fr.init(ep.frame, ep.ldf, row0, last_nrt, 3);
+    if (G > 1) w_fr.stride(G);
   }
   if (G > 1) {
     w_in.stride(G);
@@ -513,6 +524,16 @@
             smk[j] = mrow[rt < nrt ? rt : nrt - 1];
           }
         }
+      }
+    }
+    float fr[FRAME ? NST : 1][3];
+    if constexpr (FRAME) {
+      const rsrc_t r_fr = w_fr.rsrc(to_last);
+#pragma unroll
+      for (int j = 0; j < NST; ++j) {
+        fr[j][0] = __builtin_bit_cast(float, __builtin_amdgcn_raw_buffer_load_b32(r_fr, vo_fr + j * js_fr + fo0, 0, 0));
+        fr[j][1] = __builtin_bit_cast(float, __builtin_amdgcn_raw_buffer_load_b32(r_fr, vo_fr + j * js_fr + fo1, 0, 0));
+        fr[j][2] = __builtin_bit_cast(float, __builtin_amdgcn_raw_buffer_load_b32(r_fr, vo_fr + j * js_fr + fo2, 0, 0));
       }
     }
     f4 ga[NST];
@@ -572,6 +593,7 @@
         if (useseg) v += (erow + RPI * j < nb ? sg0 : sg1);
         else v += k0;
         if constexpr (SIDE) v += sd[j];
+        if constexpr (FRAME) v += f4{fr[j][0], fr[j][1], fr[j][2], fr[j][0]};
       } else if constexpr (SIDE) {
         const f4 xv = sd[j] - k0;
         v.x += __builtin_fmaf(xv.x, k1.x, k2.x);
@@ -653,6 +675,7 @@
     w_out.next();
     if constexpr (DGE || (EPI == EPI_FWD && ELU)) w_o2.next();
     if constexpr (DGE) w_ga.next();
+    if constexpr (FRAME) w_fr.next();
   };
   while (true) {
     do_tile(IC<0>{}, tile);
@@ -1038,6 +1061,42 @@
     hipLaunchKernelGGL((gemm_rows_k<256, 1, false, EPI_FWD>), dim3(grid), dim3(kWG), 0, s, x, ldx, W, ldw, y, ldy, rows, ep);
   else
     hipLaunchKernelGGL((gemm_rows_k<128, 1, false, EPI_FWD>), dim3(grid), dim3(kWG), 0, s, x, ldx, W, ldw, y, ldy, rows, ep);
+  return launch_status();
+}
+
+int32_t sn_linear_fwd_frame_supported(int32_t K, int32_t J) {
+  return gemm_variant() != 0 && (K == 128 || K == 256) && J >= 12 && J <= 128 && J % 12 == 0;
+}
+
+int sn_linear_fwd_frame_f32(const float *x, int64_t ldx, const float *W, int64_t ldw, const float *bias, const float *frame,
+                            int64_t ldf, float *y, int64_t ldy, int64_t rows, int32_t K, int32_t J, void *stream) {
+  (void)hipGetLastError();
+  if (rows < 0 || K < 1 || J < 1 || ldx < K || ldw < K || ldy < J || ldf < 3) return SN_E_SHAPE;
+  if (!sn_linear_fwd_frame_supported(K, J) || !ld32(ldx, ldy, ldf)) return SN_E_UNSUPPORTED;
+  if (rows == 0) return SN_OK;
+  if (!x || !W || !bias || !frame || !y) return SN_E_NULL;
+  if (!aligned16(x) || !aligned16(W) || !aligned16(bias) || !aligned16(y) || (ldy % 4) || (ldx % 4) || (ldw % 4) ||
+      (reinterpret_cast<uintptr_t>(frame) & 3u))
+    return SN_E_ALIGN;
+  EpiArgs ep{bias, nullptr, nullptr, nullptr, nullptr, 0, 0, nullptr, 0, 0, nullptr, 0, 0, nullptr, nullptr,
+             sn_linear_fwd_stats_blocks(rows), (int)J, nullptr, 0, nullptr, 1, nullptr, frame, ldf};
+  hipStream_t s = static_cast<hipStream_t>(stream);
+  const unsigned grid = gemm_grid(rows, gemm_wgs(K, 1));
+  hipEvent_t t_start = nullptr, t_stop = nullptr;
+  sn_internal_timing_slot(0x100 | 4, rows, K, rows * 4 * ((int64_t)K + J + 3), J, &t_start, &t_stop);
+#define SN_FRAME_FWD(KK, SM)                                                                                           \
+  do {                                                                                                                 \
+    if (t_start) hipExtLaunchKernelGGL((gemm_rows_split_k<2, KK, 1, false, EPI_FWD, false, false, SM, 4, false, true>), dim3(grid), dim3(kWG), 0, s, t_start, t_stop, 0, x, ldx, W, ldw, y, ldy, rows, ep); \
+    else hipLaunchKernelGGL((gemm_rows_split_k<2, KK, 1, false, EPI_FWD, false, false, SM, 4, false, true>), dim3(grid), dim3(kWG), 0, s, x, ldx, W, ldw, y, ldy, rows, ep); \
+  } while (0)
+  if (K == 256) {
+    if (small_operand(rows)) SN_FRAME_FWD(256, true);
+    else SN_FRAME_FWD(256, false);
+  } else {
+    if (small_operand(rows)) SN_FRAME_FWD(128, true);
+    else SN_FRAME_FWD(128, false);
+  }
+#undef SN_FRAME_FWD
   return launch_status();
 }
 
diff --git a/surfacenetworks_amd/csrc/sn_plan_table.inc b/surfacenetworks_amd/csrc/sn_plan_table.inc
--- a/surfacenetworks_amd/csrc/sn_plan_table.inc
+++ b/surfacenetworks_amd/csrc/sn_plan_table.inc
@@ -47,6 +47,8 @@
 SN_PLAN_FN(sn_wgrad_thin_f32)
 SN_PLAN_FN(sn_masked_smooth_l1_fwd_f32)
 SN_PLAN_FN(sn_masked_smooth_l1_bwd_f32)
+SN_PLAN_FN(sn_masked_smooth_l1_fwdg_f32)
+SN_PLAN_FN(sn_masked_smooth_l1_bwdg_f32)
 SN_PLAN_FN(sn_pair_argmin_f32)
 SN_PLAN_FN(sn_pair_ce_fwd_f32)
 SN_PLAN_FN(sn_pair_ce_bwd_f32)
@@ -94,6 +96,7 @@
 SN_PLAN_FN(sn_csr_scale_sym_f32)
 SN_PLAN_FN(sn_linear_fwd_f32)
 SN_PLAN_FN(sn_linear_fwd_tiles_f32)
+SN_PLAN_FN(sn_linear_fwd_frame_f32)
 SN_PLAN_FN(sn_linear_fwd_segbias_tiles_f32)
 SN_PLAN_FN(sn_avg_stats_from_tiles_ragged_f32)
 SN_PLAN_FN(sn_linear_fwd_segbias_ragged_tiles_f32)
diff --git a/surfacenetworks_amd/functional.py b/surfacenetworks_amd/functional.py
--- a/surfacenetworks_amd/functional.py
+++ b/surfacenetworks_amd/functional.py
@@ -429,7 +429,7 @@
 
 
 def bnlin_forward(x, gamma, beta, W, b, running_mean, running_var, training, momentum, eps, residual=None, elu_out=None,
-                  want_y=True, elu_stats=None, pre_stats=None, tile_sums=None):
+                  want_y=True, elu_stats=None, pre_stats=None, tile_sums=None, frame=None):
     part, part_hi = getattr(x, "_sn_part", None), getattr(x, "_sn_part_hi", None)
     x = _rows2d(x)
     rows = x.shape[0]
@@ -450,7 +450,11 @@
                                                  running_var, nbt)
     if residual is not None:
         residual = _rows2d(residual)
-    if kernels.linear_fwd_supported(x.shape[1], W.shape[0]):
+    if frame is not None:
+        if residual is not None or elu_out is not None or not want_y:
+            raise ValueError("bnlin_forward: the frame epilogue belongs to the plain forward")
+        y = kernels.linear_fwd_frame(x, Wf, bf, frame)
+    elif kernels.linear_fwd_supported(x.shape[1], W.shape[0]):
         y = kernels.linear_fwd(x, Wf, bf, residual, elu_out, want_y, elu_stats, tile_sums)
     else:
         if elu_stats is not None:
diff --git a/surfacenetworks_amd/kernels.py b/surfacenetworks_amd/kernels.py
--- a/surfacenetworks_amd/kernels.py
+++ b/surfacenetworks_amd/kernels.py
@@ -1252,6 +1252,21 @@
     return y if keep else None
 
 
+def linear_fwd_frame_supported(K: int, J: int) -> bool:
+    return bool(_lib.load().sn_linear_fwd_frame_supported(int(K), int(J)))
+
+
+def linear_fwd_frame(x, W, bias, frame):
+    _dev(x, W, bias, frame)
+    rows, K = x.shape
+    J = W.shape[0]
+    if frame.shape != (rows, 3) or frame.dtype != torch.float32:
+        raise ValueError(f"linear_fwd_frame: frame must be a ({rows}, 3) float32 view, got {tuple(frame.shape)} {frame.dtype}")
+    y = torch.empty((rows, J), dtype=torch.float32, device=x.device)
+    _lib.call("sn_linear_fwd_frame_f32", _p(x), _ld(x), _p(W), _ld(W), _p(bias), _p(frame), _ld(frame), _p(y), J, rows, K, J, _stream())
+    return y
+
+
 def avg_stats_from_tiles(tile_sums, part, e, mask, inv_count, rows_per_seg: int, nseg: int):
     _dev(tile_sums, part, e, mask, inv_count)
     rows, C = e.shape
@@ -1795,6 +1810,28 @@
     return g
 
 
+def masked_smooth_l1_fwdg(out2d, target2d, rowmask, scale: float):
+    _dev(out2d, target2d, rowmask)
+    rows, C = out2d.shape
+    loss = torch.empty((), dtype=torch.float32, device=out2d.device)
+    g = torch.empty((rows, C), dtype=torch.float32, device=out2d.device)
+    ws_bytes = int(_lib.load().sn_masked_smooth_l1_workspace_bytes(rows, C))
+    ws = torch.empty(ws_bytes, dtype=torch.uint8, device=out2d.device)
+    _lib.call("sn_masked_smooth_l1_fwdg_f32", _p(out2d), _ld(out2d), _p(target2d), _ld(target2d), _p(rowmask), rows, C,
+              float(scale), _p(loss), _p(g), C, _p(ws), ws_bytes, _stream())
+    return loss, g
+
+
+def masked_smooth_l1_bwdg(out2d, target2d, rowmask, scale: float, gloss, g):
+    _dev(out2d, target2d, rowmask, gloss, g)
+    rows, C = out2d.shape
+    if g.shape != (rows, C) or g.dtype != torch.float32 or not g.is_contiguous():
+        raise ValueError("masked_smooth_l1_bwdg: g must be the contiguous (rows, C) float32 buffer of masked_smooth_l1_fwdg")
+    _lib.call("sn_masked_smooth_l1_bwdg_f32", _p(out2d), _ld(out2d), _p(target2d), _ld(target2d), _p(rowmask), rows, C,
+              float(scale), _p(gloss), _p(g), C, _stream())
+    return g
+
+
 def linear_fwd_segbias(x, W, segbias, rows_per_seg: int, residual=None, y_elu=None, want_y: bool = True, elu_stats=None,
                        tile_sums=None):
     _dev(x, W, segbias, residual, y_elu, tile_sums)
diff --git a/surfacenetworks_amd/utils_pt.py b/surfacenetworks_amd/utils_pt.py
--- a/surfacenetworks_amd/utils_pt.py
+++ b/surfacenetworks_amd/utils_pt.py
@@ -93,10 +93,18 @@
         return y if cat is None else snB.attach_activated(y, cat)
 
 
-def elu_conv1x1(conv: GraphConv1x1, x: torch.Tensor) -> torch.Tensor:
+def elu_conv1x1(conv: GraphConv1x1, x: torch.Tensor, frame=None) -> torch.Tensor:
+    if frame is not None:
+        if not elu_conv1x1_frame_ok(conv, x, frame):
+            raise ValueError("elu_conv1x1: this layer / frame is not covered by the fused store (ask elu_conv1x1_frame_ok first)")
+        return snB.elu_conv(conv, x, frame)
     if USE_WHOLE_BLOCKS and snB.elu_conv_ok(conv, x):
         return snB.elu_conv(conv, x)
     return conv(F.elu(x))
+
+
+def elu_conv1x1_frame_ok(conv: GraphConv1x1, x: torch.Tensor, frame: torch.Tensor) -> bool:
+    return bool(USE_WHOLE_BLOCKS and snB.elu_conv_ok(conv, x) and snB.elu_conv_frame_ok(conv, x, frame))
 
 
 class GraphBatchNorm(nn.Module):
@@ -166,17 +174,17 @@
         super().__init__(num_outputs)
         self.res_f = res_f
 
-    def forward(self, Di, DiA, v, f, f_out_needed=True, num_faces=None, avg_next=None):
+    def forward(self, Di, DiA, v, f, f_out_needed=True, num_faces=None, avg_next=None, v_out_needed=True):
         batch_size, num_nodes, num_inputs = v.size()
         if f is None:
             if num_faces is None:
                 raise ValueError("DirResNet2: f=None needs num_faces")
             if _blocks_ok(self, v) and snB.zero_faces_ok(self, num_inputs):
-                return snB.dirac_block(self, Di, DiA, v, None, f_out_needed, num_faces, avg_next)
+                return snB.dirac_block(self, Di, DiA, v, None, f_out_needed, num_faces, avg_next, v_out_needed)
             f = torch.zeros(batch_size, int(num_faces), num_inputs, dtype=v.dtype, device=v.device)
         _, num_faces, _ = f.size()
         if _blocks_ok(self, v):
-            return snB.dirac_block(self, Di, DiA, v, f, f_out_needed, None, avg_next)
+            return snB.dirac_block(self, Di, DiA, v, f, f_out_needed, None, avg_next, v_out_needed)
         v2d = v.reshape(batch_size * num_nodes, num_inputs)
         cat0, e_v = snF.dirac_face_stage(as_operator(Di), v2d, f.reshape(batch_size * num_faces, num_inputs))
         f_out = self.bn_fc0.forward2d(cat0)
```

Measured after the change: 3462 meshes/s (median of 6 runs). 1.0% higher.
